# ZhenlongYuan/DVP-MVS

Measured on AMD Instinct MI355X. Metric: Mpixels/sec/PatchMatch-iteration, higher is better.
Workload: dtype f32

## Files before the change

__graft_entry__.py:

```python
import importlib
import os
import subprocess
import sys

ROOT = os.path.dirname(os.path.abspath(__file__))
if ROOT not in sys.path:
    sys.path.insert(0, ROOT)


def build() -> None:
    subprocess.check_call(["make", "-s", "-C", os.path.join(ROOT, "dvp-mvs_amd", "csrc")])
    host = os.path.join(ROOT, "dvp-mvs_amd", "host")
    if os.path.exists(os.path.join(host, "Makefile")):
        subprocess.check_call(["make", "-s", "-C", host])
    subprocess.check_call(["make", "-s", "-C", os.path.join(ROOT, "oracle")])
    subprocess.check_call(["make", "-s", "-C", os.path.join(ROOT, "tests", "emul")])
    subprocess.check_call(["make", "-s", "-C", os.path.join(ROOT, "tests", "host")])
    subprocess.check_call(["make", "-s", "-C", os.path.join(ROOT, "tests", "half16")])
    subprocess.check_call(["make", "-s", "-C", os.path.join(ROOT, "tests", "jpeg_host")])
    subprocess.check_call(["make", "-s", "-C", os.path.join(ROOT, "tests", "edges_host")])
    subprocess.check_call(["make", "-s", "-C", os.path.join(ROOT, "tests", "viewclean_host")])
    subprocess.check_call(["make", "-s", "-C", os.path.join(ROOT, "tests", "labels_host")])
    pkg = importlib.import_module("dvp-mvs_amd")
    lib = pkg.get_capi().lib()
    missing = [s for s in pkg.get_capi().EXPORTS if not hasattr(lib, s)]
    if missing:
        raise RuntimeError("libdvp_mvs_hip.so lacks symbols: %s" % missing)


def smoke() -> None:
    import numpy as np
    pkg = importlib.import_module("dvp-mvs_amd")
    synth, capi = pkg.synth, pkg.get_capi()
    from oracle import oracle as O
    W, H, S = 96, 64, 3
    sc = synth.make_scene(W, H, S)
    p = synth.default_params(S + 1, max_iterations=1, state=synth.FIRST_INIT, use_APD=0)
    p["depth_min"] = np.float32(2.5) * np.float32(0.6)
    p["depth_max"] = np.float32(6.5) * np.float32(1.2)
    state = dict(planes=np.zeros((H * W, 4), np.float32), edge=sc["edge"], label=sc["label"],
                 radius=np.full(H * W, 5, np.int32))
    g = capi.from_scene(sc, p, device=0)
    g.upload_state(**state)
    g.run_patchmatch()
    o = O.from_scene(sc, p)
    o.upload_state(**state)
    o.run_patchmatch()
    pg, po = g.get("planes"), o.get("planes")
    same = (pg.view(np.uint32) == po.view(np.uint32)) | (np.isnan(pg) & np.isnan(po))
    if not same.all():
        raise AssertionError("smoke: HIP planes differ from the oracle in %d values" % int((~same).sum()))
    for n in ("selected_views", "weak_info", "radius"):
        if not (g.get(n) == o.get(n)).all():
            raise AssertionError("smoke: %s differs from the oracle" % n)
    print("smoke ok: %dx%d S=%d bit-exact vs oracle; total %.2f ms" % (W, H, S, g.timings()["total_ms"]))


if __name__ == "__main__":
    build()
    if os.path.exists("/dev/kfd"):
        smoke()
```

dvp-mvs_amd/csrc/dvp_dev.hpp:

```cpp
#ifndef DVP_DEV_HPP_
#define DVP_DEV_HPP_

#include <stdint.h>
#include <math.h>
#include <float.h>
#include <string.h>
#include "../../include/dvp_mvs.h"

#if defined(__HIPCC__)
#include <hip/hip_runtime.h>
#define DVP_HD __host__ __device__ __forceinline__
#define DVP_HD_NOINLINE __host__ __device__ __noinline__
#else
#define DVP_HD inline
#define DVP_HD_NOINLINE inline
#endif
#ifndef DVP_STREAM_HINTS
#define DVP_STREAM_HINTS 3
#endif
#if defined(__HIP_DEVICE_COMPILE__)
#define DVP_NT_STORE(bit, p, v) do { if ((DVP_STREAM_HINTS) & (bit)) __builtin_nontemporal_store((v), (p)); else *(p) = (v); } while (0)
#define DVP_NT_LOAD(bit, p) (((DVP_STREAM_HINTS) & (bit)) ? __builtin_nontemporal_load(p) : *(p))
#else
#define DVP_NT_STORE(bit, p, v) (*(p) = (v))
#define DVP_NT_LOAD(bit, p) (*(p))
#endif

namespace dvp {

struct f4 { float x, y, z, w; };
struct f3 { float x, y, z; };
struct f2 { float x, y; };
struct i2 { int x, y; };
struct s2 { short x, y; };

DVP_HD f4 mk4(float x, float y, float z, float w) { f4 r; r.x = x; r.y = y; r.z = z; r.w = w; return r; }
DVP_HD f3 mk3(float x, float y, float z) { f3 r; r.x = x; r.y = y; r.z = z; return r; }
DVP_HD f2 mk2(float x, float y) { f2 r; r.x = x; r.y = y; return r; }
DVP_HD i2 mki2(int x, int y) { i2 r; r.x = x; r.y = y; return r; }
DVP_HD s2 mks2(int x, int y) { s2 r; r.x = (short)x; r.y = (short)y; return r; }

struct ViewConst {
	float Rrel[9];
	float trel[3];
	float sK0, sK2, sK4, sK5, sK8;
	float rK2, rK5;
	float inv_k0, inv_k4;
	float fw, fh;
	float pad;
};

struct AnchorRec;
struct WeakRec;
struct Dev {
	int width, height, num_images;
	int pitch;
	int org;
	size_t plane_stride;
	int sampler;
	int weak_count;
	uint64_t seed;
	DvpParams params;
	float nb_cos, nb_sin, nb_thresh;
	int nb_shift_range;
	const float* images;
	const uint8_t* images8;
	int img8_tiles_x;
	size_t img8_plane_bytes;
	const uint32_t* images16;
	int img16_tiles_x;
	size_t img16_plane_bytes;
	const float* depths;
	const DvpCamera* cameras;
	const ViewConst* views;
	const int* sector_taps;
	const int* sector_start;
	f4* planes;
	const f4* planes_snap;
	float* costs;
	const float* costs_snap;
	uint32_t* selected_views;
	uint8_t* view_weight;
	uint8_t* weak_info;
	uint8_t* weak_reliable;
	s2* weak_nearest_strong;
	const int* neighbours_map;
	s2* neighbours;
	s2* gn_points;
	int* gn_count;
	f4* fit_planes;
	s2* candidate;
	AnchorRec* anchor_tab;
	WeakRec* weak_rec;
	f2* weak_ctab;
	float* weak_ev;
	const uint8_t* edge;
	int* search_pos;
	float* slot_costs;
	float* strong_rec;
	f4* sweep_rec;
	float* sweep_cost;
	float* sweep_pc;
	int sweep_px0;
	int sweep_row0, sweep_row1;
	int half_w;
	uint32_t* edge_bits;
	int edge_tiles_x;
	uint32_t* strong_bits;
	uint32_t* strong_bits_t;
	int* edge_sat;
	int sat_cells_x, sat_cells_y;
	s2* edge_neigh;
	const int* label;
	s2* label_boundary;
	s2* label_stop;
	float* complex_;
	int* radius;
	const int* weak_list;
	int weak_black, weak_red;
	unsigned long long* eval_counter;
};

#define DVP_MIN(a, b) ((a) > (b) ? (b) : (a))
#define DVP_MAX(a, b) ((a) < (b) ? (b) : (a))

DVP_HD float dvp_expf(float x) {
	if (!(x > -103.0f)) return (x != x) ? x : 0.0f;
	if (x > 88.72f) return INFINITY;
	const float n = rintf(x * 1.44269504088896341f);
	float r = fmaf(n, -0.693359375f, x);
	r = fmaf(n, 2.12194440e-4f, r);
	float p = 1.9875691500e-4f;
	p = fmaf(p, r, 1.3981999507e-3f);
	p = fmaf(p, r, 8.3334519073e-3f);
	p = fmaf(p, r, 4.1665795894e-2f);
	p = fmaf(p, r, 1.6666665459e-1f);
	p = fmaf(p, r, 5.0000001201e-1f);
	const float r2 = r * r;
	const float y = fmaf(p, r2, r) + 1.0f;
	const int ni = (int)n;
	const int n1 = ni / 2, n2 = ni - n1;
	union { uint32_t u; float f; } s1, s2;
	s1.u = (uint32_t)(n1 + 127) << 23;
	s2.u = (uint32_t)(n2 + 127) << 23;
	return (y * s1.f) * s2.f;
}

DVP_HD uint32_t rand_u32(uint64_t seed, uint32_t pixel, uint32_t site, uint32_t k) {
	uint64_t z = seed + 0x9E3779B97F4A7C15ull * ((uint64_t)pixel + ((uint64_t)site << 32));
	z += 0xD1B54A32D192ED03ull * (uint64_t)(k + 1u);
	z ^= z >> 30; z *= 0xBF58476D1CE4E5B9ull;
	z ^= z >> 27; z *= 0x94D049BB133111EBull;
	z ^= z >> 31;
	return (uint32_t)(z >> 32);
}
DVP_HD float rand_uniform(uint64_t seed, uint32_t pixel, uint32_t site, uint32_t k) {
	return (float)((rand_u32(seed, pixel, site, k) >> 8) + 1u) * (1.0f / 16777216.0f);
}
enum { PH_RANDOM_INIT = 1, PH_STRONG = 2, PH_RANSAC = 3, PH_WEAK = 4, PH_NEIGHBOURS = 5 };
enum { SUB_VIEW = 0, SUB_DEPTH_RAND = 1, SUB_NORMAL = 2, SUB_DEPTH_PERT = 3, SUB_LIMIT = 4, SUB_SEARCH = 5, SUB_RANSAC = 6 };
DVP_HD uint32_t rng_site(int phase, int iter, int sub) {
	return ((uint32_t)phase << 16) | ((uint32_t)(iter & 0xff) << 8) | (uint32_t)sub;
}
struct Rng {
	uint64_t seed;
	uint32_t pixel, site, k;
	DVP_HD Rng(uint64_t s, uint32_t p, uint32_t st) : seed(s), pixel(p), site(st), k(0) {}
	DVP_HD uint32_t next() { return rand_u32(seed, pixel, site, k++); }
	DVP_HD float uniform() { return rand_uniform(seed, pixel, site, k++); }
};

constexpr int kImgPad = 2;

DVP_HD size_t cand_index(const Dev& d, int pixel, int v) { return ((size_t)v * ((size_t)d.width * d.height) + (size_t)pixel) * 8; }

DVP_HD int clampi(int v, int lo, int hi) { return v < lo ? lo : (v > hi ? hi : v); }

DVP_HD float tex_texel(const float* img, int org, int pitch, int W, int H, int ix, int iy) {
	return img[org + clampi(iy, 0, H - 1) * pitch + clampi(ix, 0, W - 1)];
}

DVP_HD float img_texel(const float* img, int org, int pitch, int W, int H, int ix, int iy) {
	return img[(size_t)(org + clampi(iy, 0, H - 1) * pitch + clampi(ix, 0, W - 1)) * 2];
}

DVP_HD void load_quad(const float* base, unsigned byte_off, float* a, float* b, float* c, float* e) {
#if defined(__HIPCC__)
	typedef float f4u __attribute__((ext_vector_type(4), aligned(8)));
	const f4u t = *reinterpret_cast<const f4u*>(reinterpret_cast<const char*>(base) + byte_off);
	*a = t.x; *b = t.y; *c = t.z; *e = t.w;
#else
	const float* p = reinterpret_cast<const float*>(reinterpret_cast<const char*>(base) + byte_off);
	*a = p[0]; *b = p[1]; *c = p[2]; *e = p[3];
#endif
}
#ifndef DVP_IMG8_TW
#define DVP_IMG8_TW 7
#endif
constexpr bool kT8Quad = DVP_IMG8_TW == 8;
constexpr int kT8W = DVP_IMG8_TW;
constexpr int kT8E = kT8Quad ? 8 : kT8W + 1;
constexpr int kT8B = kT8Quad ? 4 : 2;
constexpr int kT8H = 128 / (kT8E * kT8B);
constexpr unsigned kT8Mul = kT8W == 7 ? 74899u : (kT8W == 15 ? 34953u : 65536u);
DVP_HD int img8_tiles_x(int W) { return (W + 2 * kImgPad + kT8W - 1) / kT8W; }
DVP_HD int img8_tiles_y(int H) { return (H + 2 * kImgPad + kT8H - 1) / kT8H; }
DVP_HD unsigned img8_offset(int tiles_x, int i0, int j0) {
	const unsigned px = (unsigned)(i0 + kImgPad), py = (unsigned)(j0 + kImgPad);
#if defined(__HIP_DEVICE_COMPILE__)
	const unsigned tx = __umul24(px, kT8Mul) >> 19;
	const unsigned ex = px - __umul24((unsigned)kT8W, tx);
	const unsigned ty = py / (unsigned)kT8H, ey = py % (unsigned)kT8H;
	const unsigned tile = __umul24(ty, (unsigned)tiles_x) + tx;
#else
	const unsigned tx = (px * kT8Mul) >> 19;
	const unsigned ex = px - (unsigned)kT8W * tx;
	const unsigned ty = py / (unsigned)kT8H, ey = py % (unsigned)kT8H;
	const unsigned tile = ty * (unsigned)tiles_x + tx;
#endif
	return (tile << 7) + ey * (unsigned)(kT8B * kT8E) + ex * (unsigned)kT8B;
}
constexpr int kT16W = 7;
constexpr int kT16E = kT16W + 1;
constexpr int kT16B = 4;
constexpr int kT16H = 128 / (kT16E * kT16B);
DVP_HD int img16_tiles_x(int W) { return (W + 2 * kImgPad + kT16W - 1) / kT16W; }
DVP_HD int img16_tiles_y(int H) { return (H + 2 * kImgPad + kT16H - 1) / kT16H; }
DVP_HD unsigned img16_offset(int tiles_x, int i0, int j0) {
	const unsigned px = (unsigned)(i0 + kImgPad), py = (unsigned)(j0 + kImgPad);
	constexpr unsigned kMul = 74899u;
#if defined(__HIP_DEVICE_COMPILE__)
	const unsigned tx = __umul24(px, kMul) >> 19;
	const unsigned ex = px - __umul24((unsigned)kT16W, tx);
	const unsigned tile = __umul24(py / (unsigned)kT16H, (unsigned)tiles_x) + tx;
#else
	const unsigned tx = (px * kMul) >> 19;
	const unsigned ex = px - (unsigned)kT16W * tx;
	const unsigned tile = (py / (unsigned)kT16H) * (unsigned)tiles_x + tx;
#endif
	return (tile << 7) + (py % (unsigned)kT16H) * (unsigned)(kT16B * kT16E) + ex * (unsigned)kT16B;
}
DVP_HD float half_bits_to_float(uint32_t h) {
	const uint32_t s = (h & 0x8000u) << 16, e = (h >> 10) & 31u, m = h & 1023u;
	uint32_t b;
	if (e == 31u) b = s | 0x7F800000u | (m << 13);
	else if (e != 0u) b = s | ((e + 112u) << 23) | (m << 13);
	else if (m == 0u) b = s;
	else {
		int k = 0;
		uint32_t mm = m;
		while (!(mm & 1024u)) { mm <<= 1; ++k; }
		b = s | ((uint32_t)(113 - k) << 23) | ((mm & 1023u) << 13);
// ... 428 lines not shown
```

dvp-mvs_amd/csrc/dvp_engine.hip:

```cpp
#include "dvp_stages.hpp"
#include "dvp_jpeg_enc.h"
#include "dvp_edges_run.h"
#include "dvp_viewclean_run.h"
#include <hip/hip_runtime.h>
#include <cstdlib>
#include <string>
#include <vector>
#include <cstdio>
#include <cstring>
#include <mutex>
#include <condition_variable>
#include <thread>
#include <chrono>
#include <algorithm>
#include <cmath>

using namespace dvp;

struct LaunchArgs {
	int tiles_x, tiles, rows, half, colour, iter;
};

template <int STAGE, int SMP, int MV = 32>
__device__ __forceinline__ void stage_body(const Dev& d, const LaunchArgs& a) {
	const int lane = threadIdx.x & 63;
	const int wave = threadIdx.x >> 6;
	int px, py;
	unsigned long long n = 0;
	__shared__ f2 lds_tab[stage_uses_tab(STAGE) ? kTaps * kTaps * 256 : 1];
	const PatchTab tab{&lds_tab[stage_uses_tab(STAGE) ? threadIdx.x : 0], 256};
	if (block_to_pixel(blockIdx.x, lane, wave, a.tiles_x, a.tiles, a.rows, a.half, a.colour, d.width, d.height, &px, &py))
		run_pixel<STAGE, SMP, MV>(d, px, py, a.iter, d.eval_counter ? &n : nullptr, tab);
	if (d.eval_counter && n) atomicAdd(d.eval_counter, n);
}

struct ListArgs { int base, count, iter, covered_rows, group, run; };
#ifndef DVP_LIST_RUN
#define DVP_LIST_RUN 16
#endif
constexpr int kListRun = DVP_LIST_RUN;
#ifndef DVP_WAVE_RUN
#define DVP_WAVE_RUN 16
#endif
constexpr int kWaveRun = DVP_WAVE_RUN;
__device__ __forceinline__ int list_block(int b, int nblocks, int run) {
	const int group = 8 * run;
	if (b >= nblocks / group * group) return b;
	const int g = b / group, r = b - g * group;
	const int xcd = r & 7, i = r >> 3;
	return g * group + xcd * run + i;
}
template <int STAGE, int SMP, int MV = 32>
__device__ __forceinline__ void stage_body_list(const Dev& d, const ListArgs& a) {
	__shared__ f2 lds_tab[stage_uses_tab(STAGE) ? kTaps * kTaps * 256 : 1];
	const PatchTab tab{&lds_tab[stage_uses_tab(STAGE) ? threadIdx.x : 0], 256};
	const int t = list_block(blockIdx.x, gridDim.x, kListRun) * 256 + threadIdx.x;
	unsigned long long n = 0;
	if (t < a.count) {
		const int center = d.weak_list[a.base + t];
		const int py = center / d.width, px = center - py * d.width;
		if (!stage_is_half_c(STAGE) || py < a.covered_rows)
			run_pixel<STAGE, SMP, MV>(d, px, py, a.iter, d.eval_counter ? &n : nullptr, tab);
	}
	if (d.eval_counter && n) atomicAdd(d.eval_counter, n);
}
template <int STAGE, int SMP, int MV = 32>
__device__ __forceinline__ void stage_body64(const Dev& d, const LaunchArgs& a) {
	const int lane = threadIdx.x;
	const int b = blockIdx.x;
	const int tile = (b >> 5) * 8 + (b & 7), wave = (b >> 3) & 3;
	int px, py;
	unsigned long long n = 0;
	__shared__ f2 lds_tab[kTaps * kTaps * 64];
	const PatchTab tab{&lds_tab[lane], 64};
	if (block_to_pixel(tile, lane, wave, a.tiles_x, a.tiles, a.rows, a.half, a.colour, d.width, d.height, &px, &py))
		run_pixel<STAGE, SMP, MV>(d, px, py, a.iter, d.eval_counter ? &n : nullptr, tab);
	if (d.eval_counter && n) atomicAdd(d.eval_counter, n);
}
#define DVP_KERNEL64(NAME, STAGE, MINW)                                                                    \
	extern "C" __global__ void __launch_bounds__(64, MINW) NAME(const Dev d, const LaunchArgs a) {          \
		stage_body64<STAGE, 0>(d, a);                                                                       \
	}                                                                                                       \
	extern "C" __global__ void __launch_bounds__(64, MINW) NAME##_exact(const Dev d, const LaunchArgs a) {  \
		stage_body64<STAGE, 1>(d, a);                                                                       \
	}
#define DVP_KERNEL_LIST_MV(NAME, STAGE, MINW, MV)                                                         \
	extern "C" __global__ void __launch_bounds__(256, MINW) NAME(const Dev d, const ListArgs a) {         \
		stage_body_list<STAGE, 0, MV>(d, a);                                                               \
	}                                                                                                      \
	extern "C" __global__ void __launch_bounds__(256, MINW) NAME##_exact(const Dev d, const ListArgs a) { \
		stage_body_list<STAGE, 1, MV>(d, a);                                                               \
	}
#define DVP_KERNEL_LIST(NAME, STAGE, MINW)                                                                \
	extern "C" __global__ void __launch_bounds__(256, MINW) NAME(const Dev d, const ListArgs a) {         \
		stage_body_list<STAGE, 0>(d, a);                                                                   \
	}                                                                                                      \
	extern "C" __global__ void __launch_bounds__(256, MINW) NAME##_exact(const Dev d, const ListArgs a) { \
		stage_body_list<STAGE, 1>(d, a);                                                                   \
	}

#define DVP_KERNEL(NAME, STAGE, MINW)                                                                      \
	extern "C" __global__ void __launch_bounds__(256, MINW) NAME(const Dev d, const LaunchArgs a) {         \
		stage_body<STAGE, 0>(d, a);                                                                         \
	}                                                                                                       \
	extern "C" __global__ void __launch_bounds__(256, MINW) NAME##_exact(const Dev d, const LaunchArgs a) { \
		stage_body<STAGE, 1>(d, a);                                                                         \
	}

#define DVP_KERNEL_MV(NAME, STAGE, MINW, MV)                                                               \
	extern "C" __global__ void __launch_bounds__(256, MINW) NAME(const Dev d, const LaunchArgs a) {         \
		stage_body<STAGE, 0, MV>(d, a);                                                                     \
	}                                                                                                       \
	extern "C" __global__ void __launch_bounds__(256, MINW) NAME##_exact(const Dev d, const LaunchArgs a) { \
		stage_body<STAGE, 1, MV>(d, a);                                                                     \
	}

DVP_KERNEL(dvp_gen_edge_inform, DVP_ST_GEN_EDGE_INFORM, 1)
#ifndef DVP_LB_HEAVY
#define DVP_LB_HEAVY 2
#endif
DVP_KERNEL(dvp_random_init, DVP_ST_RANDOM_INIT, DVP_LB_HEAVY)
DVP_KERNEL(dvp_strong_update, DVP_ST_STRONG_UPDATE, DVP_LB_HEAVY)
DVP_KERNEL_MV(dvp_strong_update_v8, DVP_ST_STRONG_UPDATE, DVP_LB_HEAVY, kNarrowViews)
DVP_KERNEL_MV(dvp_strong_update_v16, DVP_ST_STRONG_UPDATE, DVP_LB_HEAVY, 16)
DVP_KERNEL64(dvp_strong_eval, kStageStrongEval, DVP_LB_HEAVY)
template <int SMP>
__device__ __forceinline__ void strong_eval_items_body(const Dev& d, const LaunchArgs& a) {
	const int lane = threadIdx.x;
	const int b = blockIdx.x;
	const int tile = (b >> 5) * 8 + (b & 7), wave = (b >> 3) & 3;
	__shared__ f2 lds_tab[kTaps * kTaps * 64];
	__shared__ uint8_t items[64 * kSlotCount];
	int px = 0, py = 0;
	bool active = block_to_pixel(tile, lane, wave, a.tiles_x, a.tiles, a.rows, a.half, a.colour, d.width, d.height, &px, &py);
	if (active && d.weak_info[px + py * d.width] == DVP_WEAK) active = false;
	PatchCtx c;
	c.tab = PatchTab{&lds_tab[lane], 64};
	c.sum_ref = c.sum_ref_ref = c.wsum = 0.0f;
	c.radius = c.inc = c.fast = 0;
	uint32_t uniq = 0;
	if (active) {
		const int center = px + py * d.width;
		int radius, inc;
		patch_geometry(d, center, &radius, &inc);
		build_patch_ctx(d, px, py, radius, inc, 0, c.tab, &c);
		uint32_t w[3];
		uniq = strong_slot_sources(d, center, w);
		const size_t Lh = (size_t)d.half_w * (size_t)d.height;
		uint32_t* dup = reinterpret_cast<uint32_t*>(d.strong_rec) + half_index(d, px, py);
		dup[SR_DUP * Lh] = w[0]; dup[(SR_DUP + 1) * Lh] = w[1]; dup[(SR_DUP + 2) * Lh] = w[2];
	}
	const int n = __popc(uniq);
	int incl = n;
#pragma unroll
	for (int o = 1; o < 64; o <<= 1) {
		const int t = __shfl_up(incl, o, 64);
		if (lane >= o) incl += t;
	}
	const int off = incl - n;
	const int total = __shfl(incl, 63, 64);
	{
		int k = 0;
		for (uint32_t m = uniq; m; m &= m - 1, ++k) items[off + k] = (uint8_t)lane;
	}
	__syncthreads();
	unsigned long long cnt = 0;
	for (int i0 = 0; i0 < total; i0 += 64) {
		const bool valid = i0 + lane < total;
		const int i = valid ? i0 + lane : total - 1;
		const int pl = items[i];
		const int k = i - __shfl(off, pl, 64);
		uint32_t m = (uint32_t)__shfl((int)uniq, pl, 64);
		for (int j = 0; j < k; ++j) m &= m - 1;
		const int slot = dvp_ctz(m);
		PatchCtx ci;
		ci.tab = PatchTab{&lds_tab[pl], 64};
		ci.sum_ref = __shfl(c.sum_ref, pl, 64);
		ci.sum_ref_ref = __shfl(c.sum_ref_ref, pl, 64);
		ci.wsum = __shfl(c.wsum, pl, 64);
		ci.radius = __shfl(c.radius, pl, 64);
		ci.inc = __shfl(c.inc, pl, 64);
		ci.fast = __shfl(c.fast, pl, 64);
		const int ipx = __shfl(px, pl, 64), ipy = __shfl(py, pl, 64);
		strong_eval_item<SMP>(d, ci, ipx, ipy, slot, valid, d.eval_counter ? &cnt : nullptr);
	}
	if (d.eval_counter && cnt) atomicAdd(d.eval_counter, cnt);
}
extern "C" __global__ void __launch_bounds__(64, DVP_LB_HEAVY) dvp_strong_eval_items(const Dev d, const LaunchArgs a) { strong_eval_items_body<0>(d, a); }
extern "C" __global__ void __launch_bounds__(64, DVP_LB_HEAVY) dvp_strong_eval_items_exact(const Dev d, const LaunchArgs a) { strong_eval_items_body<1>(d, a); }
DVP_KERNEL64(dvp_strong_refine, kStageStrongRefine, DVP_LB_HEAVY)
DVP_KERNEL64(dvp_strong_refine_lanes, kStageStrongRefineLanes, DVP_LB_HEAVY)
template <int MV>
__device__ __forceinline__ void strong_decide_body(const Dev& d, const LaunchArgs& a) {
	int px, py;
	if (!block_to_pixel(blockIdx.x, threadIdx.x & 63, threadIdx.x >> 6, a.tiles_x, a.tiles, a.rows, a.half, a.colour, d.width, d.height, &px, &py)) return;
	if (d.weak_info[px + py * d.width] != DVP_WEAK) strong_decide_px<MV>(d, px, py, a.iter);
}
#ifndef DVP_LB_DECIDE
#define DVP_LB_DECIDE 4
#endif
#define DVP_DECIDE_KERNEL(MV) extern "C" __global__ void __launch_bounds__(256, DVP_LB_DECIDE) dvp_strong_decide_v##MV(const Dev d, const LaunchArgs a) { strong_decide_body<MV>(d, a); }
DVP_DECIDE_KERNEL(4)
DVP_DECIDE_KERNEL(6)
DVP_DECIDE_KERNEL(8)
DVP_DECIDE_KERNEL(10)
DVP_DECIDE_KERNEL(12)
DVP_DECIDE_KERNEL(16)
DVP_KERNEL(dvp_get_depth_normal, DVP_ST_GET_DEPTH_NORMAL, 1)
DVP_KERNEL(dvp_filter_strong, DVP_ST_FILTER_STRONG, 1)
DVP_KERNEL(dvp_depth_to_weak, DVP_ST_DEPTH_TO_WEAK, DVP_LB_HEAVY)
DVP_KERNEL(dvp_local_refine, DVP_ST_LOCAL_REFINE, DVP_LB_HEAVY)
DVP_KERNEL(dvp_depth_to_weak_refine, kStageSweeps, DVP_LB_HEAVY)
template <int WHAT>
__device__ __forceinline__ void sweep_light_body(const Dev& d, const LaunchArgs& a) {
	int px, py;
	if (!block_to_pixel(blockIdx.x, threadIdx.x & 63, threadIdx.x >> 6, a.tiles_x, a.tiles, a.rows, 0, 0, d.width, d.height, &px, &py)) return;
	if (WHAT != 0 && d.sweep_row1 > 0 && (py < d.sweep_row0 || py >= d.sweep_row1)) return;
	if (WHAT == 0) sweep_prepare_px(d, px, py);
	else if (WHAT == 1) sweep_decide1_px(d, px, py);
	else sweep_decide2_px(d, px, py);
}
extern "C" __global__ void __launch_bounds__(256) dvp_sweep_prepare(const Dev d, const LaunchArgs a) { sweep_light_body<0>(d, a); }
extern "C" __global__ void __launch_bounds__(256) dvp_sweep_decide1(const Dev d, const LaunchArgs a) { sweep_light_body<1>(d, a); }
extern "C" __global__ void __launch_bounds__(256) dvp_sweep_decide2(const Dev d, const LaunchArgs a) { sweep_light_body<2>(d, a); }
#ifndef DVP_SWEEP_ROWS
#define DVP_SWEEP_ROWS 14
#endif
constexpr int kSweepRows = DVP_SWEEP_ROWS;
template <int SMP>
__device__ __forceinline__ void sweep_eval_body(const Dev& d, const LaunchArgs& a) {
	const int lane = threadIdx.x;
	const int v = blockIdx.y;
	__shared__ f2 lds_tab[kTaps * kTaps * 64];
	__shared__ uint16_t list[64 * kSweepRows];
	__shared__ DvpCamera cams[2];
	const PatchTab tab{&lds_tab[lane], 64};
	static_assert(sizeof(DvpCamera) == 112, "28 dwords");
	if (lane < 56) {
		const int which = lane >= 28 ? 1 : 0;
		reinterpret_cast<uint32_t*>(&cams[which])[lane - 28 * which] = reinterpret_cast<const uint32_t*>(d.cameras + (which ? v + 1 : 0))[lane - 28 * which];
	}
	const int tiles_y = a.tiles / a.tiles_x;
	int tx, ty;
	{
		const int per_strip = 8 * tiles_y;
		const int st = (int)blockIdx.x / per_strip, rem = (int)blockIdx.x - st * per_strip;
		const int w_last = a.tiles_x - st * 8;
		if (w_last >= 8) { ty = rem >> 3; tx = st * 8 + (rem & 7); }
		else { ty = rem / w_last; tx = st * 8 + (rem - ty * w_last); }
	}
	ty += a.rows;
	const int x = tx * 64 + lane;
	int n = 0;
	for (int r = 0; r < kSweepRows; ++r) {
		const int y = ty * kSweepRows + r;
		const bool go = x < d.width && y < d.height && sweep_go(d, x + y * d.width, v, a.iter);
		const unsigned long long m = __ballot(go);
		if (go) list[n + __popcll(m & ((1ull << lane) - 1ull))] = (uint16_t)(r * 64 + lane);
		n += __popcll(m);
	}
	__syncthreads();
	unsigned long long cnt = 0;
	for (int i0 = 0; i0 < n; i0 += 64) {
		if (i0 + lane < n) {
			const int e = list[i0 + lane];
			sweep_eval_px<SMP>(d, tx * 64 + (e & 63), ty * kSweepRows + (e >> 6), v, a.iter, tab, d.eval_counter ? &cnt : nullptr, cams);
		}
	}
	if (d.eval_counter && cnt) atomicAdd(d.eval_counter, cnt);
}
template <int SMP>
__device__ __forceinline__ void sweep_border_body(const Dev& d, const LaunchArgs& a) {
	__shared__ f2 lds_tab[kTaps * kTaps * 64];
	const PatchTab tab{&lds_tab[threadIdx.x], 64};
	const int W = d.width, H = d.height;
	const long long t = (long long)blockIdx.x * 64 + threadIdx.x;
	int px, py;
	if (t < 12ll * W) {
		const int r = (int)(t / W);
		px = (int)(t - (long long)r * W);
		py = r < 6 ? r : H - 12 + r;
	} else {
		const long long u = t - 12ll * W;
		const int r = (int)(u / 12), cidx = (int)(u - 12ll * r);
		if (r >= H - 12) return;
		py = 6 + r;
		px = cidx < 6 ? cidx : W - 12 + cidx;
	}
	unsigned long long n = 0;
	run_pixel<kStageSweeps, SMP>(d, px, py, kSweepBorderOnly, d.eval_counter ? &n : nullptr, tab);
	if (d.eval_counter && n) atomicAdd(d.eval_counter, n);
}
extern "C" __global__ void __launch_bounds__(64, DVP_LB_HEAVY) dvp_sweep_border(const Dev d, const LaunchArgs a) { sweep_border_body<0>(d, a); }
extern "C" __global__ void __launch_bounds__(64, DVP_LB_HEAVY) dvp_sweep_border_exact(const Dev d, const LaunchArgs a) { sweep_border_body<1>(d, a); }
extern "C" __global__ void __launch_bounds__(64, DVP_LB_HEAVY) dvp_sweep_eval(const Dev d, const LaunchArgs a) { sweep_eval_body<0>(d, a); }
extern "C" __global__ void __launch_bounds__(64, DVP_LB_HEAVY) dvp_sweep_eval_exact(const Dev d, const LaunchArgs a) { sweep_eval_body<1>(d, a); }

DVP_KERNEL_LIST(dvp_find_nearest_strong_list, DVP_ST_FIND_NEAREST_STRONG, 1)
extern "C" __global__ void __launch_bounds__(256) dvp_gen_neighbours_list(const Dev d, const ListArgs a) {
	__shared__ s2 pts[kGnDirSlots * 256];
	const int t = list_block(blockIdx.x, gridDim.x, kListRun) * 256 + threadIdx.x;
	if (t >= a.count) return;
	const int center = d.weak_list[a.base + t];
// ... 162 lines not shown
		y = kImgPad + k / (2 * kImgPad);
		x = k % (2 * kImgPad);
		if (x >= kImgPad) x += W;
	}
	float* p = planes + (size_t)pl * plane_stride;
	const int sx = clampi(x - kImgPad, 0, W - 1) + kImgPad, sy = clampi(y - kImgPad, 0, H - 1) + kImgPad;
	p[(size_t)y * pitch + x] = p[(size_t)sy * pitch + sx];
}

extern "C" __global__ void dvp_interleave_rows(const float* __restrict__ in, float* __restrict__ out, int PH, int pitch, size_t plane_stride, int n_planes) {
	const int x = blockIdx.x * blockDim.x + threadIdx.x;
	const int y = blockIdx.y;
	const int pl = blockIdx.z;
	if (x >= pitch) return;
	const float* p = in + (size_t)pl * plane_stride;
	const int y1 = y + 1 < PH ? y + 1 : y;
	const float2 v = make_float2(p[(size_t)y * pitch + x], p[(size_t)y1 * pitch + x]);
	reinterpret_cast<float2*>(out + (size_t)pl * plane_stride * 2)[(size_t)y * pitch + x] = v;
}

extern "C" __global__ void dvp_pairs_to_tiles(const float* __restrict__ pairs, uint8_t* __restrict__ out, int PW, int PH, int pitch, size_t plane_stride,
                                              int tiles_x, int tiles_y, int n_planes, int* inexact) {
	const size_t per_plane = (size_t)tiles_x * tiles_y * 64;
	const size_t i = (size_t)blockIdx.x * blockDim.x + threadIdx.x;
	if (i >= per_plane * n_planes) return;
	const int pl = (int)(i / per_plane);
	const size_t r = i - (size_t)pl * per_plane;
	const int tile = (int)(r >> 6), e = (int)(r & 63);
	const int ty = tile / tiles_x, tx = tile - ty * tiles_x;
	const int sx = min(tx * kT8W + (e % kT8E), PW - 1), sy = min(ty * kT8H + (e / kT8E), PH - 1);
	if (e >= kT8E * kT8H) return;
	const float* plane = pairs + (size_t)pl * plane_stride * 2;
	const float2 v = reinterpret_cast<const float2*>(plane)[(size_t)sy * pitch + sx];
	const float2 u = reinterpret_cast<const float2*>(plane)[(size_t)sy * pitch + min(sx + 1, PW - 1)];
	uint32_t h;
	const unsigned bad = tile_pair_rule(v.x, v.y, &h);
	if (bad) {
		if ((*inexact & bad) != bad) atomicOr(inexact, (int)bad);
		if (bad & 1u) return;
	}
	uint8_t* dst = out + ((size_t)pl * tiles_x * tiles_y + tile) * 128 + (size_t)e * kT8B;
	dst[0] = (uint8_t)v.x;
	dst[1] = (uint8_t)v.y;
	if (kT8Quad) { dst[2] = (uint8_t)u.x; dst[3] = (uint8_t)u.y; }
}

extern "C" __global__ void dvp_pairs_to_tiles16(const float* __restrict__ pairs, uint32_t* __restrict__ out, int PW, int PH, int pitch, size_t plane_stride,
                                                int tiles_x, int tiles_y, int n_planes) {
	constexpr int kPer = kT16E * kT16H;
	const size_t per_plane = (size_t)tiles_x * tiles_y * kPer;
	const size_t i = (size_t)blockIdx.x * blockDim.x + threadIdx.x;
	if (i >= per_plane * n_planes) return;
	const int pl = (int)(i / per_plane);
	const size_t r = i - (size_t)pl * per_plane;
	const int tile = (int)(r / kPer), e = (int)(r % kPer);
	const int ty = tile / tiles_x, tx = tile - ty * tiles_x;
	const int sx = min(tx * kT16W + (e % kT16E), PW - 1), sy = min(ty * kT16H + (e / kT16E), PH - 1);
	const float2 v = reinterpret_cast<const float2*>(pairs + (size_t)pl * plane_stride * 2)[(size_t)sy * pitch + sx];
	uint32_t h;
	(void)tile_pair_rule(v.x, v.y, &h);
	out[((size_t)pl * tiles_x * tiles_y + tile) * (128 / 4) + e] = h;
}

extern "C" __global__ void dvp_pack_edge_bits(const uint8_t* __restrict__ edge, uint32_t* __restrict__ bits, int W, int H, int tiles_x, size_t words, int equals) {
	const size_t w = (size_t)blockIdx.x * blockDim.x + threadIdx.x;
	if (w < words) bits[w] = pack_edge_word(edge, W, H, tiles_x, w, equals);
}

extern "C" __global__ void __launch_bounds__(256) dvp_gen_candidates(const Dev d, const LaunchArgs a) {
	int px, py;
	if (block_to_pixel(blockIdx.x, threadIdx.x & 63, threadIdx.x >> 6, a.tiles_x, a.tiles, a.rows, 0, 0, d.width, d.height, &px, &py))
		gen_candidates_px(d, px, py, (int)blockIdx.y);
}

extern "C" __global__ void __launch_bounds__(256) dvp_gen_candidates_views(const Dev d, const LaunchArgs a) {
	int px, py;
	if (block_to_pixel(blockIdx.x, threadIdx.x & 63, threadIdx.x >> 6, a.tiles_x, a.tiles, a.rows, 0, 0, d.width, d.height, &px, &py))
		gen_candidates_views_px<kCandGroup>(d, px, py, (int)blockIdx.y * kCandGroup);
}
extern "C" __global__ void __launch_bounds__(256) dvp_gen_candidates_views_list(const Dev d, const unsigned* list, const unsigned* n_list) {
	const unsigned t = blockIdx.x * 256 + threadIdx.x;
	if (t >= *n_list) return;
	const int center = (int)list[t];
	const int py = center / d.width, px = center - py * d.width;
	gen_candidates_views_px<kCandGroup>(d, px, py, (int)blockIdx.y * kCandGroup);
}

extern "C" __global__ void __launch_bounds__(256) dvp_anchor_mask(const Dev d, const ListArgs a, uint8_t* mask) {
	const int t = blockIdx.x * 256 + threadIdx.x;
	if (t >= a.count) return;
	const int center = d.weak_list[a.base + t];
	const s2* nb = d.neighbours + (size_t)d.neighbours_map[center] * DVP_NEIGHBOUR_NUM;
	for (int k = 1; k < DVP_NEIGHBOUR_NUM; ++k) {
		const s2 q = nb[k];
		if (q.x >= 0 && q.y >= 0 && q.x < d.width && q.y < d.height) mask[(size_t)q.y * d.width + q.x] = 1;
	}
}
extern "C" __global__ void __launch_bounds__(256) dvp_mask_compact(const uint8_t* mask, size_t L, unsigned* list, unsigned* n_list) {
	const size_t p = (size_t)blockIdx.x * 256 + threadIdx.x;
	const bool go = p < L && mask[p] != 0;
	const unsigned long long m = __ballot(go);
	if (!m) return;
	const int lane = threadIdx.x & 63;
	unsigned base = 0;
	if (lane == __builtin_ctzll(m)) base = atomicAdd(n_list, (unsigned)__popcll(m));
	base = __shfl(base, __builtin_ctzll(m), 64);
	if (go) list[base + __popcll(m & ((1ull << lane) - 1ull))] = (unsigned)p;
}
extern "C" __global__ void __launch_bounds__(256) dvp_gen_candidates_list(const Dev d, const unsigned* list, const unsigned* n_list) {
	const unsigned t = blockIdx.x * 256 + threadIdx.x;
	if (t >= *n_list) return;
	const int center = (int)list[t];
	const int py = center / d.width, px = center - py * d.width;
	gen_candidates_px(d, px, py, (int)blockIdx.y);
}

extern "C" __global__ void dvp_pack_bits_transposed(const uint8_t* __restrict__ map, uint32_t* __restrict__ bits, int W, int H, int tiles_x, size_t words, int equals) {
	const size_t w = (size_t)blockIdx.x * blockDim.x + threadIdx.x;
	if (w < words) bits[w] = pack_edge_word_t(map, W, H, tiles_x, w, equals);
}

extern "C" __global__ void dvp_edge_cell_counts(const Dev d) {
	const int c = blockIdx.x * blockDim.x + threadIdx.x;
	if (c >= d.sat_cells_x * d.sat_cells_y) return;
	const int cy = c / d.sat_cells_x, cx = c - cy * d.sat_cells_x;
	int n = 0;
	for (int r = 0; r < 8; ++r) {
		const int y = cy * 8 + r;
		if (y >= d.height) break;
		const unsigned w = d.edge_bits[(size_t)(((y >> 5) * d.edge_tiles_x + (cx >> 2)) * 32 + (y & 31))];
		n += __popc((w >> ((cx & 3) * 8)) & 255u);
	}
	d.edge_sat[(cy + 1) * (d.sat_cells_x + 1) + cx + 1] = n;
}
extern "C" __global__ void dvp_edge_sat_rows(const Dev d) {
	const int r = blockIdx.x * blockDim.x + threadIdx.x;
	if (r > d.sat_cells_y) return;
	int* row = d.edge_sat + (size_t)r * (d.sat_cells_x + 1);
	int acc = 0;
	for (int x = 0; x <= d.sat_cells_x; ++x) { acc += (r == 0 || x == 0) ? 0 : row[x]; row[x] = acc; }
}
extern "C" __global__ void dvp_edge_sat_cols(const Dev d) {
	const int x = blockIdx.x * blockDim.x + threadIdx.x;
	if (x > d.sat_cells_x) return;
	const int P = d.sat_cells_x + 1;
	int acc = 0;
	for (int r = 0; r <= d.sat_cells_y; ++r) { acc += d.edge_sat[(size_t)r * P + x]; d.edge_sat[(size_t)r * P + x] = acc; }
}

extern "C" __global__ void __launch_bounds__(256) dvp_strong_search(const Dev d, const LaunchArgs a) {
	int px, py;
	if (block_to_pixel(blockIdx.x, threadIdx.x & 63, threadIdx.x >> 6, a.tiles_x, a.tiles, a.rows, a.half, a.colour, d.width, d.height, &px, &py))
		strong_search_px(d, px, py);
}

extern "C" __global__ void __launch_bounds__(256) dvp_edge_rays(const Dev d, int what) {
	edge_ray_line(d, blockIdx.y, blockIdx.x * blockDim.x + threadIdx.x, what);
}

constexpr int kWeakTile = 16, kWeakSuper = 64, kWeakChunk = 1024;
DVP_HD void weak_slot_origin(int slot, int supers_x, int* tx, int* ty) {
	const int super = slot >> 4, t = slot & 15;
	*tx = (super % supers_x) * kWeakSuper + (t & 3) * kWeakTile;
	*ty = (super / supers_x) * kWeakSuper + (t >> 2) * kWeakTile;
}
extern "C" __global__ void __launch_bounds__(256) dvp_weak_counts(const uint8_t* __restrict__ weak, int W, int H, int supers_x, int n_slots, int n_chunks, int* __restrict__ counts) {
	const int lane = threadIdx.x & 63;
	const int unit = blockIdx.x * 4 + (threadIdx.x >> 6);
	if (unit < n_slots) {
		int tx, ty;
		weak_slot_origin(unit, supers_x, &tx, &ty);
		int nb = 0, nr = 0;
		for (int step = 0; step < 4; ++step) {
			const int x = tx + (lane & 15), y = ty + step * 4 + (lane >> 4);
			const bool wk = x < W && y < H && weak[(size_t)y * W + x] == DVP_WEAK;
			nb += __popcll(__ballot(wk && !((x + y) & 1)));
			nr += __popcll(__ballot(wk && ((x + y) & 1)));
		}
		if (lane == 0) { counts[unit] = nb; counts[n_slots + unit] = nr; }
	} else if (unit < n_slots + n_chunks) {
		const int chunk = unit - n_slots;
		const size_t L = (size_t)W * H;
		int n = 0;
		for (int step = 0; step < kWeakChunk / 64; ++step) {
			const size_t i = (size_t)chunk * kWeakChunk + step * 64 + lane;
			n += __popcll(__ballot(i < L && weak[i] == DVP_WEAK));
		}
		if (lane == 0) counts[2 * n_slots + chunk] = n;
	}
}
extern "C" __global__ void __launch_bounds__(1024) dvp_scan3(int* __restrict__ data, int s0, int s1, int s2, int s3, int* __restrict__ totals) {
	__shared__ int part[1024];
	__shared__ int carry;
	const int starts[4] = { s0, s1, s2, s3 };
	const int lo = starts[blockIdx.x], hi = starts[blockIdx.x + 1];
	if (threadIdx.x == 0) carry = 0;
	__syncthreads();
	for (int base = lo; base < hi; base += 1024) {
		const int i = base + (int)threadIdx.x;
		const int v = i < hi ? data[i] : 0;
		part[threadIdx.x] = v;
		__syncthreads();
		for (int off = 1; off < 1024; off <<= 1) {
			const int add = threadIdx.x >= (unsigned)off ? part[threadIdx.x - off] : 0;
			__syncthreads();
			part[threadIdx.x] += add;
			__syncthreads();
		}
		if (i < hi) data[i] = carry + part[threadIdx.x] - v;
		__syncthreads();
		if (threadIdx.x == 1023) carry += part[1023];
		__syncthreads();
	}
	if (threadIdx.x == 0) totals[blockIdx.x] = carry;
}
extern "C" __global__ void __launch_bounds__(256) dvp_weak_fill(const uint8_t* __restrict__ weak, int W, int H, int supers_x, int n_slots, int n_chunks,
                                                               const int* __restrict__ offs, const int* __restrict__ totals, int* __restrict__ list, int* __restrict__ map) {
	const int lane = threadIdx.x & 63;
	const int unit = blockIdx.x * 4 + (threadIdx.x >> 6);
	const unsigned long long below = (1ull << lane) - 1ull;
	if (unit < n_slots) {
		int tx, ty;
		weak_slot_origin(unit, supers_x, &tx, &ty);
		int ob = offs[unit], orr = totals[0] + offs[n_slots + unit];
		for (int step = 0; step < 4; ++step) {
			const int x = tx + (lane & 15), y = ty + step * 4 + (lane >> 4);
			const bool wk = x < W && y < H && weak[(size_t)y * W + x] == DVP_WEAK;
			const bool red = (x + y) & 1;
			const unsigned long long mb = __ballot(wk && !red), mr = __ballot(wk && red);
			if (wk) list[red ? orr + __popcll(mr & below) : ob + __popcll(mb & below)] = y * W + x;
			ob += __popcll(mb);
			orr += __popcll(mr);
		}
	} else if (unit < n_slots + n_chunks) {
		const int chunk = unit - n_slots;
		const size_t L = (size_t)W * H;
		int o = offs[2 * n_slots + chunk];
		for (int step = 0; step < kWeakChunk / 64; ++step) {
			const size_t i = (size_t)chunk * kWeakChunk + step * 64 + lane;
			const bool wk = i < L && weak[i] == DVP_WEAK;
			const unsigned long long m = __ballot(wk);
			if (i < L) map[i] = wk ? o + __popcll(m & below) : 0;
			o += __popcll(m);
		}
	}
}

struct RescaleArgs {
	int W, H, sw, sh;
	float scale_x, scale_y;
	const float* depth; const float* normal; const uint32_t* views; const uint8_t* weak; const int* radius;
	f4* planes; uint32_t* out_views; uint8_t* out_weak; int* out_radius;
	int radius_fallback;
};
extern "C" __global__ void __launch_bounds__(256) dvp_rescale_state(const RescaleArgs a) {
	const int c = blockIdx.x * blockDim.x + threadIdx.x, r = blockIdx.y;
	if (c >= a.W) return;
	const int o_r = static_cast<int>(r / a.scale_x);
	const int o_c = static_cast<int>(c / a.scale_y);
	const bool in = o_r >= 0 && o_c >= 0 && o_r < a.sh && o_c < a.sw;
	const size_t o = (size_t)r * a.W + c, i = in ? (size_t)o_r * a.sw + o_c : 0;
	a.planes[o] = in ? mk4(a.normal[3 * i], a.normal[3 * i + 1], a.normal[3 * i + 2], a.depth[i]) : mk4(0.0f, 0.0f, 0.0f, 0.0f);
	a.out_views[o] = in ? a.views[i] : 0u;
	const uint8_t st = a.weak ? (in ? a.weak[i] : (uint8_t)0) : (uint8_t)DVP_STRONG;
	a.out_weak[o] = st;
	if (a.radius) a.out_radius[o] = st == DVP_UNKNOWN ? a.radius_fallback : (in ? a.radius[i] : 0);
}

extern "C" __global__ void __launch_bounds__(256) dvp_unpack_maps(const f4* __restrict__ planes, const uint8_t* __restrict__ weak, size_t L, float dmin, float dmax,
                                                                 float* __restrict__ depth, float* __restrict__ normal, uint8_t* __restrict__ state) {
	const size_t i = (size_t)blockIdx.x * blockDim.x + threadIdx.x;
	if (i >= L) return;
	const f4 ph = planes[i];
	const bool usable = !(ph.w < dmin || ph.w > dmax);
	depth[i] = usable ? ph.w : 0.0f;
	normal[3 * i] = ph.x; normal[3 * i + 1] = ph.y; normal[3 * i + 2] = ph.z;
	state[i] = usable ? weak[i] : (uint8_t)DVP_UNKNOWN;
}

extern "C" __global__ void dvp_prepare_views(const DvpCamera* cams, ViewConst* views, int n) {
	const int v = blockIdx.x * blockDim.x + threadIdx.x;
	if (v >= 1 && v < n) compute_view_const(cams[0], cams[v], &views[v]);
}

extern "C" __global__ void __launch_bounds__(256) dvp_cost_vectors(const Dev d, const int* px, const f4* planes, int n, float* out) {
	const int i = blockIdx.x * blockDim.x + threadIdx.x;
	if (i >= n) return;
	const int x = px[2 * i], y = px[2 * i + 1];
	const int S = d.num_images - 1;
	PatchCtx c;
	__shared__ f2 lds_tab[kTaps * kTaps * 256];
	int radius, inc;
	patch_geometry(d, x + y * d.width, &radius, &inc);
	build_patch_ctx(d, x, y, radius, inc, 0, PatchTab{&lds_tab[threadIdx.x], 256}, &c);
	const f4 pl = planes[i];
	for (int v = 0; v < S; ++v) out[(size_t)i * S + v] = d.sampler ? ncc_old<1>(d, c, x, y, v + 1, pl) : ncc_old<0>(d, c, x, y, v + 1, pl);
}

extern "C" __global__ void __launch_bounds__(256) dvp_cost_all_pixels(const Dev d, const LaunchArgs a, float* out) {
	const int lane = threadIdx.x & 63, wave = threadIdx.x >> 6;
	int px, py;
	if (!block_to_pixel(blockIdx.x, lane, wave, a.tiles_x, a.tiles, a.rows, 0, 0, d.width, d.height, &px, &py)) return;
	const int center = px + py * d.width;
	const int S = d.num_images - 1;
	PatchCtx c;
	__shared__ f2 lds_tab[kTaps * kTaps * 256];
// ... 74 lines not shown
	const ViewConst vc = d.views[v + 1];
	const unsigned plane_off = (unsigned)((size_t)(v + 1) * d.plane_stride * 2 * sizeof(float));
	const int center = px + py * d.width;
	float acc = 0.0f;
	for (int k = 0; k < K; ++k) {
		int q = center + (k - K / 2) * stride;
		q = q < 0 ? 0 : (q >= L ? L - 1 : q);
		const f4 pl = d.planes[q];
		float H[9];
		homography(vc, pl, H);
		const f2 pt = apply_homography(H, px, py);
		if (pt.x >= vc.fw || pt.x < 0.0f || pt.y >= vc.fh || pt.y < 0.0f) { acc += 2.0f; continue; }
		acc += ncc_patch_fast<0>(d, c, H, d.images, px, py, plane_off);
	}
	atomicAdd(&out[center], acc);
}
__device__ __forceinline__ float probe_slot_plane(const DvpCamera& rc, const f4 origin, float base_line, float disp, int k, int px, int py, const DvpParams& P, bool* in_range) {
	float p_depth = origin.w;
	*in_range = true;
	if (k < 61) {
		p_depth = rc.K[0] * base_line / (disp + (k - 30));
		if (p_depth < P.depth_min || p_depth > P.depth_max) *in_range = false;
	}
	return distance_to_origin(rc, px, py, p_depth, origin);
}
extern "C" __global__ void __launch_bounds__(256, 2) dvp_probe_c(const Dev d, const LaunchArgs a, float* out, unsigned vmask) {
	const int lane = threadIdx.x & 63, wave = threadIdx.x >> 6;
	int px, py;
	if (!block_to_pixel(blockIdx.x, lane, wave, a.tiles_x, a.tiles, a.rows, 0, 0, d.width, d.height, &px, &py)) return;
	const int center = px + py * d.width;
	const int S = d.num_images - 1;
	PatchCtx c;
	__shared__ f2 lds_tab[kTaps * kTaps * 256];
	int radius, inc;
	patch_geometry(d, center, &radius, &inc);
	build_patch_ctx(d, px, py, radius, inc, 0, PatchTab{&lds_tab[threadIdx.x], 256}, &c);
	const DvpCamera rc = load_camera(d, 0);
	const f4 origin = normal_world_to_cam(rc, d.planes[center]);
	const float base_line = 0.4f, disp = rc.K[0] * base_line / origin.w;
	float acc = 0.0f;
	for (int k = 0; k < 62; ++k) {
		bool ok;
		f4 pl = origin;
		pl.w = probe_slot_plane(rc, origin, base_line, disp, k, px, py, d.params, &ok);
		float t = 0.0f;
		if (ok) for (int v = 0; v < S; ++v) if ((vmask >> v) & 1) t += ncc_old<0>(d, c, px, py, v + 1, pl);
		acc += t;
	}
	out[center] = acc;
}
#ifndef DVP_PROBE_NPX
#define DVP_PROBE_NPX 16
#endif
extern "C" __global__ void __launch_bounds__(64, DVP_PROBE_LB) dvp_probe_d(const Dev d, float* out, unsigned vmask) {
	const int lane = threadIdx.x;
	const int S = d.num_images - 1;
	__shared__ f2 ctab[kTaps * kTaps];
	__shared__ float caa[kTaps * kTaps];
	__shared__ float tot[64];
	const int runs = 64 / DVP_PROBE_NPX;
	const int tiles_x = (d.width + 63) / 64;
	const int per_strip = 8 * d.height * runs;
	const int st = (int)blockIdx.x / per_strip, rem = (int)blockIdx.x - st * per_strip;
	const int w_last = tiles_x - st * 8 >= 8 ? 8 : tiles_x - st * 8;
	const int col = rem % w_last, k2 = rem / w_last;
	const int py = k2 / runs, x0 = (st * 8 + col) * 64 + (k2 - py * runs) * DVP_PROBE_NPX;
	if (py >= d.height) return;
	const DvpCamera rc = load_camera(d, 0);
	for (int i = 0; i < DVP_PROBE_NPX; ++i) {
		const int px = x0 + i;
		if (px >= d.width) break;
		const int center = px + py * d.width;
		int radius, inc;
		patch_geometry(d, center, &radius, &inc);
		PatchCtx c;
		c.radius = radius; c.inc = inc; c.fast = 1;
		c.tab = PatchTab{ctab, 1};
		if (lane < kTaps * kTaps) {
			const int ty = lane / kTaps, tx = lane - ty * kTaps;
			const float cpix = img_texel(d.images, d.org, d.pitch, d.width, d.height, px, py);
			const float av = img_texel(d.images, d.org, d.pitch, d.width, d.height, px - radius + tx * inc, py - radius + ty * inc);
			const float w = bilateral_weight((float)(-radius + tx * inc), (float)(-radius + ty * inc), av, cpix, d.params.sigma_spatial, d.params.sigma_color, 0);
			const float wa = w * av;
			ctab[lane] = mk2(w, wa);
			caa[lane] = wa * av;
		}
		__builtin_amdgcn_fence(__ATOMIC_RELEASE, "wavefront"); __builtin_amdgcn_wave_barrier(); __builtin_amdgcn_fence(__ATOMIC_ACQUIRE, "wavefront");
		{
			float sr = 0.0f, srr = 0.0f, ws = 0.0f;
			for (int ty = 0; ty < kTaps; ++ty) {
				float a0 = 0.0f, a1 = 0.0f, a2 = 0.0f;
				for (int tx = 0; tx < kTaps; ++tx) { const f2 t = ctab[ty * kTaps + tx]; a0 += t.y; a1 += caa[ty * kTaps + tx]; a2 += t.x; }
				sr += a0; srr += a1; ws += a2;
			}
			c.sum_ref = sr; c.sum_ref_ref = srr; c.wsum = ws;
		}
		f4 origin = normal_world_to_cam(rc, d.planes[center]);
		origin.x = uniform_f(origin.x); origin.y = uniform_f(origin.y); origin.z = uniform_f(origin.z); origin.w = uniform_f(origin.w);
		const float base_line = 0.4f, disp = rc.K[0] * base_line / origin.w;
		bool ok;
		f4 pl = origin;
		pl.w = probe_slot_plane(rc, origin, base_line, disp, lane, px, py, d.params, &ok);
		float t = 0.0f;
		if (lane < 62 && ok) for (int v = 0; v < S; ++v) if ((vmask >> v) & 1) t += ncc_old<0>(d, c, px, py, v + 1, pl);
		tot[lane] = t;
		__builtin_amdgcn_fence(__ATOMIC_RELEASE, "wavefront"); __builtin_amdgcn_wave_barrier(); __builtin_amdgcn_fence(__ATOMIC_ACQUIRE, "wavefront");
		if (lane == 0) {
			float acc = 0.0f;
			for (int k = 0; k < 62; ++k) acc += tot[k];
			out[center] = acc;
		}
		__builtin_amdgcn_wave_barrier();
	}
}
extern "C" int dvp_probe(dvp_ctx* c, int mode, int K, int stride, int repeat, float* mean_ms, float* checksum);
#endif

struct EventPair { int stage; hipEvent_t a, b; };
enum { EV_TOTAL = -1, EV_ITER_LOOP = -2 };

struct dvp_ctx {
	int device = 0;
	int W = 0, H = 0, NI = 0, pitch = 0;
	size_t L = 0;
	hipStream_t stream = nullptr;
	int cand_mask_mode = -1;
	bool cand_mask_on = true;
	uint8_t* cand_mask = nullptr;
	unsigned *cand_list = nullptr, *cand_n = nullptr;
	uint32_t* sel_snap = nullptr;
	hipStream_t side = nullptr;
	hipEvent_t side_fork = nullptr, side_join = nullptr;
	Dev d{};
	std::vector<void*> allocs;
	float* images = nullptr;
	uint8_t* images8 = nullptr;
	int* images8_flag = nullptr;
	bool images8_ok = false;
	bool no_images8 = false;
	uint32_t* images16 = nullptr;
	bool images16_ok = false;
	bool no_images16 = false;
	float* image_stage = nullptr;
	float* depths = nullptr;
	uint32_t* edge_bits = nullptr;
	uint32_t* strong_bits = nullptr;
	uint32_t* strong_bits_t = nullptr;
	int* edge_sat = nullptr;
	DvpCamera* cameras = nullptr; ViewConst* views = nullptr; int* sector_taps = nullptr; int* sector_start = nullptr;
	f4* planes = nullptr; f4* planes_snap = nullptr; f4* fit_planes = nullptr;
	int* search_pos = nullptr;
	float* slot_costs = nullptr;
	float* strong_rec = nullptr;
	bool strong_split = true;
	bool eval_items = true;
	bool refine_lanes = true;
	f4* sweep_rec = nullptr; float* sweep_cost = nullptr; float* sweep_pc = nullptr;
	bool ransac_wave = false;
	bool sweep_split = true;
	bool sweep_force = false;
	double sweep_band_gb = 0.0;
	int sweep_band_rows = 0;
	bool gn_wave = false;
	float* costs = nullptr; float* costs_snap = nullptr; float* complex_ = nullptr;
	uint32_t* selected_views = nullptr;
	uint8_t* view_weight = nullptr; uint8_t* weak_info = nullptr; uint8_t* weak_reliable = nullptr; uint8_t* edge = nullptr;
	s2* label_stop = nullptr; s2* weak_nearest_strong = nullptr; s2* neighbours = nullptr; s2* gn_points = nullptr; int* gn_count = nullptr; s2* candidate = nullptr; s2* edge_neigh = nullptr; s2* label_boundary = nullptr;
	int* neighbours_map = nullptr; int* label = nullptr; int* radius = nullptr;
	unsigned long long* eval_counter = nullptr;
	float* scratch_out = nullptr;
	size_t weak_alloc = 0;
	AnchorRec* anchor_tab = nullptr;
	size_t anchor_tab_alloc = 0;
	bool anchor_tab_valid = false;
	bool anchor_tab_off = false;
	WeakRec* weak_rec = nullptr; f2* weak_ctab = nullptr; float* weak_ev = nullptr;
	size_t weak_phase_alloc = 0;
	bool weak_phased = true;
	int weak_phased_min = 8192;
	int weak_run[4] = { 64, 256, 1024, 1024 };
	int weak_group[4] = { 1, 4, 4, 2 };
	int* weak_list = nullptr;
	size_t weak_list_alloc = 0;
	int* weak_counts = nullptr;
	int* weak_totals_host = nullptr;
	uint8_t* coarse = nullptr;
	uint8_t* maps_out = nullptr;
	hipStream_t copy = nullptr;
	uint8_t* maps_host = nullptr;
	std::mutex dl_m;
	std::condition_variable dl_cv;
	bool dl_busy = false;
	bool dl_fetching = false;
	size_t coarse_alloc = 0;
	uint8_t* pv_bgr[3] = { nullptr, nullptr, nullptr };
	dvpjpeg::Encoder pv_enc[3];
	unsigned long long* pv_total = nullptr;
	hipEvent_t pv_done = nullptr;
	hipStream_t pv_copy = nullptr;
	int pv_kinds = 0;
	dvpedge::Scratch eg;
	struct EdgeSlot { uint8_t* map = nullptr; hipEvent_t done = nullptr; unsigned long long seq = 0; bool pending = false, fetching = false; };
	EdgeSlot eg_slot[2];
	unsigned long long eg_seq = 0;
	hipStream_t eg_copy = nullptr;
	std::mutex eg_m;
	std::condition_variable eg_cv;
	bool have_images = false;
	dvpvc::Scratch vc;
	bool vc_on = false;
	int vc_num_src = 0, vc_min_region = 0;
	f4* saved_planes = nullptr; uint32_t* saved_views = nullptr; uint8_t* saved_weak = nullptr; int* saved_radius = nullptr;
	bool have_saved = false;
	int lut_radius = -1;
	bool have_depths = false;
	bool profiling = false;
	std::vector<EventPair> events;
	DvpTimings timings{};
	std::string error;
};

static std::string g_create_error;

#define HIP_TRY(ctx, expr)                                                                          \
	do {                                                                                            \
		hipError_t e_ = (expr);                                                                     \
		if (e_ != hipSuccess) {                                                                     \
			char buf_[512];                                                                         \
			snprintf(buf_, sizeof(buf_), "%s failed: %s (%s:%d)", #expr, hipGetErrorString(e_), __FILE__, __LINE__); \
			(ctx)->error = buf_;                                                                    \
			return 1;                                                                               \
		}                                                                                           \
	} while (0)

template <class T>
static int dalloc(dvp_ctx* c, T** p, size_t count, bool zero = true) {
	void* q = nullptr;
	const size_t bytes = (count ? count : 1) * sizeof(T);
	HIP_TRY(c, hipMalloc(&q, bytes));
	c->allocs.push_back(q);
	if (zero) HIP_TRY(c, hipMemsetAsync(q, 0, bytes, c->stream));
	*p = (T*)q;
	return 0;
}

template <class T>
static void dfree(dvp_ctx* c, T** p) {
	if (!*p) return;
	for (size_t i = 0; i < c->allocs.size(); ++i)
		if (c->allocs[i] == (void*)*p) { c->allocs[i] = c->allocs.back(); c->allocs.pop_back(); break; }
	(void)hipFree((void*)*p);
	*p = nullptr;
}

static size_t img16_plane_bytes(int W, int H) { return (size_t)img16_tiles_x(W) * img16_tiles_y(H) * 128; }

static void sync_dev_struct(dvp_ctx* c) {
	Dev& d = c->d;
	d.width = c->W; d.height = c->H; d.num_images = c->NI; d.pitch = c->pitch;
	d.org = kImgPad * c->pitch + kImgPad;
	d.plane_stride = (size_t)c->pitch * (c->H + 2 * kImgPad);
	d.images = c->images; d.images8 = c->images8_ok ? c->images8 : nullptr; d.img8_tiles_x = img8_tiles_x(c->W); d.img8_plane_bytes = (size_t)img8_tiles_x(c->W) * img8_tiles_y(c->H) * 128;
	d.images16 = c->images16_ok ? c->images16 : nullptr; d.img16_tiles_x = img16_tiles_x(c->W); d.img16_plane_bytes = img16_plane_bytes(c->W, c->H);
	d.depths = c->depths; d.cameras = c->cameras; d.views = c->views; d.sector_taps = c->sector_taps; d.sector_start = c->sector_start;
	d.search_pos = c->search_pos;
	d.sweep_px0 = 0; d.sweep_row0 = 0; d.sweep_row1 = 0;
	d.sweep_rec = c->sweep_rec; d.sweep_cost = c->sweep_cost; d.sweep_pc = c->sweep_pc; d.slot_costs = c->slot_costs; d.strong_rec = c->strong_rec; d.half_w = (c->W + 1) / 2;
	d.planes = c->planes; d.planes_snap = c->planes_snap; d.costs = c->costs; d.costs_snap = c->costs_snap;
	d.selected_views = c->selected_views; d.view_weight = c->view_weight; d.weak_info = c->weak_info;
	d.weak_reliable = c->weak_reliable; d.weak_nearest_strong = c->weak_nearest_strong;
	d.anchor_tab = (c->anchor_tab_off || !c->anchor_tab_valid) ? nullptr : c->anchor_tab; d.neighbours_map = c->neighbours_map; d.neighbours = c->neighbours; d.gn_points = c->gn_points; d.gn_count = c->gn_count; d.fit_planes = c->fit_planes;
	d.candidate = c->candidate; d.edge = c->edge; d.edge_bits = c->edge_bits; d.strong_bits = c->strong_bits; d.strong_bits_t = c->strong_bits_t; d.edge_sat = c->edge_sat; d.sat_cells_x = sat_cells(c->W); d.sat_cells_y = sat_cells(c->H); d.edge_tiles_x = edge_tiles_x(c->W); d.edge_neigh = c->edge_neigh; d.label = c->label;
	d.label_boundary = c->label_boundary; d.label_stop = c->label_stop; d.complex_ = c->complex_; d.radius = c->radius;
	d.weak_list = c->weak_list;
	d.weak_rec = c->weak_rec; d.weak_ctab = c->weak_ctab; d.weak_ev = c->weak_ev;
	d.eval_counter = c->profiling ? c->eval_counter : nullptr;
}

static int ensure_images16(dvp_ctx* c) {
	if (c->images16) return 0;
	return dalloc(c, &c->images16, img16_plane_bytes(c->W, c->H) / 4 * c->NI, false);
}

static int set_device(dvp_ctx* c) {
	HIP_TRY(c, hipSetDevice(c->device));
	return 0;
}

extern "C" {

int dvp_ctx_create(int device, int width, int height, int num_images, dvp_ctx** out) {
	if (!out) return 1;
	*out = nullptr;
	if (width <= 0 || height <= 0 || num_images < 2 || num_images > DVP_MAX_IMAGES || width > 32767 || height > 32767) {
		g_create_error = "dvp_ctx_create: bad dimensions (2 <= num_images <= 32, sizes <= 32767: short2 pixel coordinates)";
		return 1;
	}
	{
		const unsigned long long pitch = ((unsigned long long)width + 2 * kImgPad + 63) / 64 * 64;
		if (pitch * ((unsigned long long)height + 2 * kImgPad) * 8ull >= (1ull << 32)) {
			g_create_error = "dvp_ctx_create: image too large (a padded row-pair plane must stay below 4 GiB)";
			return 1;
		}
	}
	dvp_ctx* c = new dvp_ctx();
	c->device = device; c->W = width; c->H = height; c->NI = num_images;
	c->no_images8 = getenv("DVP_NO_IMAGES8") != nullptr;
	c->no_images16 = getenv("DVP_NO_IMAGES16") != nullptr;
	if (const char* e = getenv("DVP_STRONG_SPLIT")) c->strong_split = atoi(e) != 0;
	if (const char* e = getenv("DVP_REFINE_LANES")) c->refine_lanes = atoi(e) != 0;
	if (const char* e = getenv("DVP_EVAL_ITEMS")) c->eval_items = atoi(e) != 0;
	if (const char* e = getenv("DVP_SWEEP_SPLIT")) { c->sweep_split = atoi(e) != 0; c->sweep_force = atoi(e) == 2; }
	if (const char* e = getenv("DVP_SWEEP_BAND_GB")) c->sweep_band_gb = atof(e);
	if (const char* e = getenv("DVP_WEAK_ANCHOR_TAB")) c->anchor_tab_off = atoi(e) == 0;
	if (const char* e = getenv("DVP_GN_WAVE")) c->gn_wave = atoi(e) != 0;
	if (const char* e = getenv("DVP_RANSAC_WAVE")) c->ransac_wave = atoi(e) != 0;
	if (const char* e = getenv("DVP_CAND_MASK")) c->cand_mask_mode = atoi(e) != 0 ? 1 : 0;
	if (const char* e = getenv("DVP_WEAK_PHASED")) c->weak_phased = atoi(e) != 0;
	if (const char* e = getenv("DVP_WEAK_PHASED_MIN")) c->weak_phased_min = atoi(e);
	if (const char* e = getenv("DVP_WEAK_RUNS")) {
		int g[4];
		if (sscanf(e, "%d,%d,%d,%d", &g[0], &g[1], &g[2], &g[3]) == 4)
			for (int i = 0; i < 4; ++i) c->weak_run[i] = g[i] < 1 ? 1 : g[i];
	}
	if (const char* e = getenv("DVP_WEAK_GROUPS")) {
		int g[4];
		if (sscanf(e, "%d,%d,%d,%d", &g[0], &g[1], &g[2], &g[3]) == 4)
			for (int i = 0; i < 4; ++i) c->weak_group[i] = g[i] < 1 ? 1 : (g[i] > kGrp ? kGrp : g[i]);
	}
	c->pitch = (width + 2 * kImgPad + 63) / 64 * 64;
	c->L = (size_t)width * height;
	auto fail = [&](int) { g_create_error = c->error; dvp_ctx_destroy(c); return 1; };
	if (set_device(c)) return fail(0);
	if (hipStreamCreateWithFlags(&c->stream, hipStreamNonBlocking) != hipSuccess) { c->error = "hipStreamCreate failed"; return fail(0); }
	if (hipStreamCreateWithFlags(&c->side, hipStreamNonBlocking) != hipSuccess || hipEventCreateWithFlags(&c->side_fork, hipEventDisableTiming) != hipSuccess ||
	    hipEventCreateWithFlags(&c->side_join, hipEventDisableTiming) != hipSuccess) { c->error = "hipStreamCreate failed"; return fail(0); }
	const size_t L = c->L, S = (size_t)num_images - 1, plane = (size_t)c->pitch * (height + 2 * kImgPad);
	int r = 0;
	r |= dalloc(c, &c->images, plane * num_images * 2);
	r |= dalloc(c, &c->images8, (size_t)img8_tiles_x(width) * img8_tiles_y(height) * 128 * num_images);
	r |= dalloc(c, &c->images8_flag, (size_t)1);
	r |= dalloc(c, &c->image_stage, plane * num_images);
	r |= dalloc(c, &c->cameras, (size_t)num_images);
	r |= dalloc(c, &c->views, (size_t)num_images);
	r |= dalloc(c, &c->planes, L);
	r |= dalloc(c, &c->planes_snap, L);
	r |= dalloc(c, &c->search_pos, L * 16);
	r |= dalloc(c, &c->fit_planes, L);
	r |= dalloc(c, &c->costs, L);
	r |= dalloc(c, &c->costs_snap, L);
	r |= dalloc(c, &c->selected_views, L + (size_t)width);
	r |= dalloc(c, &c->view_weight, L * 32);
	r |= dalloc(c, &c->weak_info, L);
	r |= dalloc(c, &c->weak_reliable, L);
	r |= dalloc(c, &c->weak_nearest_strong, L);
	r |= dalloc(c, &c->neighbours_map, L);
	r |= dalloc(c, &c->candidate, L * S * 8);
	r |= dalloc(c, &c->edge, L);
	r |= dalloc(c, &c->edge_bits, edge_bits_words(width, height));
	r |= dalloc(c, &c->strong_bits, edge_bits_words(width, height));
	r |= dalloc(c, &c->strong_bits_t, edge_bits_words(width, height));
	r |= dalloc(c, &c->edge_sat, (size_t)(sat_cells(width) + 1) * (sat_cells(height) + 1));
	r |= dalloc(c, &c->edge_neigh, L * 8);
	r |= dalloc(c, &c->label, L);
	r |= dalloc(c, &c->radius, L);
	r |= dalloc(c, &c->eval_counter, (size_t)1);
	r |= dalloc(c, &c->scratch_out, L);
	if (r) return fail(0);
	{
		std::vector<uint8_t> st(L, (uint8_t)DVP_STRONG);
		std::vector<int> rad(L, 5);
		std::vector<s2> m1(L * 8, mks2(-1, -1));
		if (hipMemcpyAsync(c->weak_info, st.data(), L, hipMemcpyHostToDevice, c->stream) != hipSuccess ||
			hipMemcpyAsync(c->radius, rad.data(), L * 4, hipMemcpyHostToDevice, c->stream) != hipSuccess ||
			hipMemcpyAsync(c->edge_neigh, m1.data(), L * 8 * 4, hipMemcpyHostToDevice, c->stream) != hipSuccess ||
			hipMemcpyAsync(c->weak_nearest_strong, m1.data(), L * 4, hipMemcpyHostToDevice, c->stream) != hipSuccess ||
			hipStreamSynchronize(c->stream) != hipSuccess) { c->error = "default state upload failed"; return fail(0); }
	}
	std::memset(&c->d.params, 0, sizeof(DvpParams));
	c->d.params.num_images = num_images;
	c->d.params.strong_radius = 5; c->d.params.strong_increment = 2; c->d.params.weak_radius = 5; c->d.params.weak_increment = 5;
	c->d.params.rotate_time = 4;
	sync_dev_struct(c);
	*out = c;
	return 0;
}

int dvp_ctx_destroy(dvp_ctx* c) {
	if (!c) return 0;
	(void)hipSetDevice(c->device);
	{
		int limit_s = 120;
		if (const char* e = getenv("DVP_DOWNLOAD_WAIT_S")) limit_s = atoi(e);
		std::unique_lock<std::mutex> lk(c->dl_m);
		c->dl_cv.wait_for(lk, std::chrono::seconds(limit_s > 0 ? limit_s : 1), [c] { return !c->dl_busy; });
		c->dl_cv.wait(lk, [c] { return !c->dl_fetching; });
	}
	if (c->copy) { (void)hipStreamSynchronize(c->copy); (void)hipStreamDestroy(c->copy); }
	if (c->pv_copy) { (void)hipStreamSynchronize(c->pv_copy); (void)hipStreamDestroy(c->pv_copy); }
	{
		std::unique_lock<std::mutex> lk(c->eg_m);
		c->eg_cv.wait(lk, [c] { return !c->eg_slot[0].fetching && !c->eg_slot[1].fetching; });
	}
	if (c->eg_copy) { (void)hipStreamSynchronize(c->eg_copy); (void)hipStreamDestroy(c->eg_copy); }
	if (c->stream) (void)hipStreamSynchronize(c->stream);
	for (auto& e : c->pv_enc) dvpjpeg::encoder_free(e);
	dvpedge::scratch_free(c->eg);
	dvpvc::scratch_free(c->vc);
	for (auto& sl : c->eg_slot) { if (sl.map) (void)hipFree(sl.map); if (sl.done) (void)hipEventDestroy(sl.done); }
	if (c->pv_total) (void)hipHostFree(c->pv_total);
	if (c->pv_done) (void)hipEventDestroy(c->pv_done);
	if (c->maps_host) (void)hipHostFree(c->maps_host);
	if (c->stream) (void)hipStreamSynchronize(c->stream);
	for (auto& e : c->events) { (void)hipEventDestroy(e.a); (void)hipEventDestroy(e.b); }
	for (void* p : c->allocs) (void)hipFree(p);
	if (c->weak_totals_host) (void)hipHostFree(c->weak_totals_host);
	if (c->side) { (void)hipStreamSynchronize(c->side); (void)hipStreamDestroy(c->side); }
	if (c->side_fork) (void)hipEventDestroy(c->side_fork);
	if (c->side_join) (void)hipEventDestroy(c->side_join);
	if (c->stream) (void)hipStreamDestroy(c->stream);
	delete c;
	return 0;
}

#ifndef DVP_BUILD_ID
#define DVP_BUILD_ID "unknown"
#endif
const char* dvp_build_id(void) { return DVP_BUILD_ID; }

struct FinishError { const dvp_ctx* c = nullptr; std::string msg; };
static thread_local FinishError t_finish_error;
const char* dvp_last_error(const dvp_ctx* c) {
	if (c && t_finish_error.c == c && !t_finish_error.msg.empty()) return t_finish_error.msg.c_str();
	return c ? c->error.c_str() : g_create_error.c_str();
}

static int upload_planes(dvp_ctx* c, float* dst, const float* const* src, int pitch_floats, hipMemcpyKind kind, float* pairs = nullptr) {
	if (set_device(c)) return 1;
	if (pitch_floats < c->W) { c->error = "pitch_floats < width"; return 1; }
	const size_t stride = (size_t)c->pitch * (c->H + 2 * kImgPad);
	for (int i = 0; i < c->NI; ++i) {
		if (!src[i]) { c->error = "null image pointer"; return 1; }
		HIP_TRY(c, hipMemcpy2DAsync(dst + (size_t)i * stride + (size_t)kImgPad * c->pitch + kImgPad, (size_t)c->pitch * 4, src[i],
		                            (size_t)pitch_floats * 4, (size_t)c->W * 4, (size_t)c->H, kind, c->stream));
	}
	{
		const long long cells = (long long)(2 * kImgPad * (c->W + 2 * kImgPad) + 2 * kImgPad * c->H) * c->NI;
		hipLaunchKernelGGL(dvp_pad_replicate, dim3((unsigned)((cells + 255) / 256)), dim3(256), 0, c->stream, dst, c->W, c->H, c->pitch, stride, c->NI);
		HIP_TRY(c, hipGetLastError());
	}
	if (pairs) {
		const int PH = c->H + 2 * kImgPad;
		hipLaunchKernelGGL(dvp_interleave_rows, dim3((unsigned)((c->pitch + 255) / 256), (unsigned)PH, (unsigned)c->NI), dim3(256), 0, c->stream,
		                   dst, pairs, PH, c->pitch, stride, c->NI);
		HIP_TRY(c, hipGetLastError());
		HIP_TRY(c, hipMemsetAsync(c->images8_flag, 0, sizeof(int), c->stream));
		const int t8x = img8_tiles_x(c->W), t8y = img8_tiles_y(c->H);
		const size_t n = (size_t)t8x * t8y * 64 * c->NI;
		hipLaunchKernelGGL(dvp_pairs_to_tiles, dim3((unsigned)((n + 255) / 256)), dim3(256), 0, c->stream, pairs, c->images8, c->W + 2 * kImgPad, PH, c->pitch, stride,
		                   t8x, t8y, c->NI, c->images8_flag);
		HIP_TRY(c, hipGetLastError());
		int inexact = 3;
		HIP_TRY(c, hipMemcpyAsync(&inexact, c->images8_flag, sizeof(int), hipMemcpyDeviceToHost, c->stream));
		HIP_TRY(c, hipStreamSynchronize(c->stream));
		c->images8_ok = inexact == 0 && !c->no_images8;
		c->images16_ok = inexact == 1 && !c->no_images8 && !c->no_images16;
		if (c->images16_ok) {
			if (ensure_images16(c)) { c->images16_ok = false; sync_dev_struct(c); return 1; }
			const int t16x = img16_tiles_x(c->W), t16y = img16_tiles_y(c->H);
			const size_t n16 = (size_t)t16x * t16y * (kT16E * kT16H) * c->NI;
			hipLaunchKernelGGL(dvp_pairs_to_tiles16, dim3((unsigned)((n16 + 255) / 256)), dim3(256), 0, c->stream, pairs, c->images16, c->W + 2 * kImgPad, PH, c->pitch, stride,
			                   t16x, t16y, c->NI);
			HIP_TRY(c, hipGetLastError());
		}
		sync_dev_struct(c);
	}
	HIP_TRY(c, hipStreamSynchronize(c->stream));
	return 0;
}
int dvp_upload_images(dvp_ctx* c, const float* const* images, int pitch_floats) {
	c->anchor_tab_valid = false;
	if (upload_planes(c, c->image_stage, images, pitch_floats, hipMemcpyHostToDevice, c->images)) return 1;
	c->have_images = true;
	return 0;
}
int dvp_upload_images_device(dvp_ctx* c, const float* const* images, int pitch_floats) {
	c->anchor_tab_valid = false;
	if (upload_planes(c, c->image_stage, images, pitch_floats, hipMemcpyDeviceToDevice, c->images)) return 1;
	c->have_images = true;
	return 0;
}
static int ensure_depths(dvp_ctx* c) {
	if (!c->depths) {
		if (dalloc(c, &c->depths, (size_t)c->pitch * (c->H + 2 * kImgPad) * c->NI)) return 1;
		sync_dev_struct(c);
	}
	c->have_depths = true;
	return 0;
}
int dvp_upload_depths(dvp_ctx* c, const float* const* depths, int pitch_floats) {
	if (set_device(c) || ensure_depths(c)) return 1;
	return upload_planes(c, c->depths, depths, pitch_floats, hipMemcpyHostToDevice);
}
int dvp_upload_depths_device(dvp_ctx* c, const float* const* depths, int pitch_floats) {
	if (set_device(c) || ensure_depths(c)) return 1;
	return upload_planes(c, c->depths, depths, pitch_floats, hipMemcpyDeviceToDevice);
}

int dvp_upload_cameras(dvp_ctx* c, const DvpCamera* cams, int n) {
	if (set_device(c)) return 1;
	if (n != c->NI) { c->error = "dvp_upload_cameras: n != num_images"; return 1; }
	HIP_TRY(c, hipMemcpyAsync(c->cameras, cams, sizeof(DvpCamera) * n, hipMemcpyHostToDevice, c->stream));
	hipLaunchKernelGGL(dvp_prepare_views, dim3(1), dim3(64), 0, c->stream, c->cameras, c->views, n);
	HIP_TRY(c, hipGetLastError());
	HIP_TRY(c, hipStreamSynchronize(c->stream));
	return 0;
}

static int ensure_weak_buffers(dvp_ctx* c, size_t weak_count) {
	const size_t need = weak_count ? weak_count : 1;
	if (need > c->weak_alloc) {
		HIP_TRY(c, hipStreamSynchronize(c->stream));
		if (c->side) HIP_TRY(c, hipStreamSynchronize(c->side));
		dfree(c, &c->neighbours); dfree(c, &c->gn_points); dfree(c, &c->gn_count); dfree(c, &c->complex_); dfree(c, &c->label_boundary);
		const size_t cap = std::min<size_t>(c->L, std::max(need, c->weak_alloc + c->weak_alloc / 2));
		if (dalloc(c, &c->neighbours, cap * DVP_NEIGHBOUR_NUM, false)) return 1;
		if (dalloc(c, &c->gn_points, cap * kGnDirSlots, false) || dalloc(c, &c->gn_count, cap)) return 1;
		if (dalloc(c, &c->complex_, cap)) return 1;
		if (dalloc(c, &c->label_boundary, cap * 8, false)) return 1;
		c->weak_alloc = cap;
	}
	HIP_TRY(c, hipMemsetAsync(c->neighbours, 0xFF, need * DVP_NEIGHBOUR_NUM * sizeof(s2), c->stream));
	HIP_TRY(c, hipMemsetAsync(c->label_boundary, 0xFF, need * 8 * sizeof(s2), c->stream));
	HIP_TRY(c, hipMemsetAsync(c->complex_, 0, need * 4, c->stream));
	return 0;
}

static int rebuild_weak_lists(dvp_ctx* c) {
	const size_t L = c->L;
	const int supers_x = (c->W + kWeakSuper - 1) / kWeakSuper, supers_y = (c->H + kWeakSuper - 1) / kWeakSuper;
	const int n_slots = supers_x * supers_y * 16, n_chunks = (int)((L + kWeakChunk - 1) / kWeakChunk);
	const int n_units = n_slots + n_chunks;
	if (!c->weak_counts) {
		if (dalloc(c, &c->weak_counts, (size_t)2 * n_slots + n_chunks + 4)) return 1;
		HIP_TRY(c, hipHostMalloc((void**)&c->weak_totals_host, 4 * sizeof(int)));
	}
	int* totals = c->weak_counts + 2 * (size_t)n_slots + n_chunks;
	hipLaunchKernelGGL(dvp_weak_counts, dim3((n_units + 3) / 4), dim3(256), 0, c->stream, c->weak_info, c->W, c->H, supers_x, n_slots, n_chunks, c->weak_counts);
	hipLaunchKernelGGL(dvp_scan3, dim3(3), dim3(1024), 0, c->stream, c->weak_counts, 0, n_slots, 2 * n_slots, 2 * n_slots + n_chunks, totals);
	HIP_TRY(c, hipMemcpyAsync(c->weak_totals_host, totals, 3 * sizeof(int), hipMemcpyDeviceToHost, c->stream));
	HIP_TRY(c, hipStreamSynchronize(c->stream));
	const int nb = c->weak_totals_host[0], nr = c->weak_totals_host[1], wc = c->weak_totals_host[2];
	if (nb + nr != wc) { c->error = "dvp_upload_state: WEAK list / map counts disagree"; return 1; }
	c->d.weak_count = wc;
	c->d.weak_black = nb;
	c->d.weak_red = nr;
	if ((size_t)wc > c->weak_list_alloc) {
		dfree(c, &c->weak_list);
		const size_t cap = std::min<size_t>(L, std::max<size_t>((size_t)wc, c->weak_list_alloc + c->weak_list_alloc / 2));
		if (dalloc(c, &c->weak_list, cap, false)) return 1;
		c->weak_list_alloc = cap;
	}
	if (wc > 0) {
		hipLaunchKernelGGL(dvp_weak_fill, dim3((n_units + 3) / 4), dim3(256), 0, c->stream, c->weak_info, c->W, c->H, supers_x, n_slots, n_chunks,
		                   c->weak_counts, totals, c->weak_list, c->neighbours_map);
		HIP_TRY(c, hipGetLastError());
	} else {
		HIP_TRY(c, hipMemsetAsync(c->neighbours_map, 0, L * 4, c->stream));
	}
	if (ensure_weak_buffers(c, (size_t)wc)) return 1;
	HIP_TRY(c, hipStreamSynchronize(c->stream));
	sync_dev_struct(c);
	return 0;
}

int dvp_upload_state(dvp_ctx* c, const float* planes, const uint32_t* views, const uint8_t* weak,
                     const uint8_t* edge, const int32_t* label, const int32_t* radius) {
	c->anchor_tab_valid = false;
	if (set_device(c)) return 1;
	const size_t L = c->L;
	if (planes) HIP_TRY(c, hipMemcpyAsync(c->planes, planes, L * 16, hipMemcpyHostToDevice, c->stream));
	if (views) HIP_TRY(c, hipMemcpyAsync(c->selected_views, views, L * 4, hipMemcpyHostToDevice, c->stream));
	if (edge) HIP_TRY(c, hipMemcpyAsync(c->edge, edge, L, hipMemcpyHostToDevice, c->stream));
	if (label) HIP_TRY(c, hipMemcpyAsync(c->label, label, L * 4, hipMemcpyHostToDevice, c->stream));
	if (radius) HIP_TRY(c, hipMemcpyAsync(c->radius, radius, L * 4, hipMemcpyHostToDevice, c->stream));
	if (weak) HIP_TRY(c, hipMemcpyAsync(c->weak_info, weak, L, hipMemcpyHostToDevice, c->stream));
	return rebuild_weak_lists(c);
}

int dvp_upload_state_rescaled(dvp_ctx* c, int src_w, int src_h, const float* depth, const float* normal_xyz, const uint32_t* views,
                              const uint8_t* weak, const int32_t* radius, int radius_fallback, const uint8_t* edge, const int32_t* label) {
	c->anchor_tab_valid = false;
	if (set_device(c)) return 1;
	if (src_w <= 0 || src_h <= 0 || !depth || !normal_xyz || !views) { c->error = "dvp_upload_state_rescaled: depth, normal and selected_views are required"; return 1; }
	const size_t L = c->L, n = (size_t)src_w * src_h;
	const size_t off_normal = n * 4, off_views = off_normal + n * 12, off_radius = off_views + n * 4, off_weak = off_radius + n * 4, bytes = off_weak + n;
	if (bytes > c->coarse_alloc) {
		HIP_TRY(c, hipStreamSynchronize(c->stream));
		dfree(c, &c->coarse);
		if (dalloc(c, &c->coarse, bytes, false)) return 1;
		c->coarse_alloc = bytes;
	}
	HIP_TRY(c, hipMemcpyAsync(c->coarse, depth, n * 4, hipMemcpyHostToDevice, c->stream));
	HIP_TRY(c, hipMemcpyAsync(c->coarse + off_normal, normal_xyz, n * 12, hipMemcpyHostToDevice, c->stream));
	HIP_TRY(c, hipMemcpyAsync(c->coarse + off_views, views, n * 4, hipMemcpyHostToDevice, c->stream));
	if (radius) HIP_TRY(c, hipMemcpyAsync(c->coarse + off_radius, radius, n * 4, hipMemcpyHostToDevice, c->stream));
	if (weak) HIP_TRY(c, hipMemcpyAsync(c->coarse + off_weak, weak, n, hipMemcpyHostToDevice, c->stream));
	if (edge) HIP_TRY(c, hipMemcpyAsync(c->edge, edge, L, hipMemcpyHostToDevice, c->stream));
	if (label) HIP_TRY(c, hipMemcpyAsync(c->label, label, L * 4, hipMemcpyHostToDevice, c->stream));
	RescaleArgs a;
	a.W = c->W; a.H = c->H; a.sw = src_w; a.sh = src_h;
	a.scale_x = c->W / static_cast<float>(src_w);
	a.scale_y = c->H / static_cast<float>(src_h);
	a.depth = reinterpret_cast<const float*>(c->coarse); a.normal = reinterpret_cast<const float*>(c->coarse + off_normal);
	a.views = reinterpret_cast<const uint32_t*>(c->coarse + off_views);
	a.radius = radius ? reinterpret_cast<const int*>(c->coarse + off_radius) : nullptr;
	a.weak = weak ? c->coarse + off_weak : nullptr;
	a.planes = c->planes; a.out_views = c->selected_views; a.out_weak = c->weak_info; a.out_radius = c->radius;
	a.radius_fallback = radius_fallback;
	hipLaunchKernelGGL(dvp_rescale_state, dim3((unsigned)((c->W + 255) / 256), (unsigned)c->H), dim3(256), 0, c->stream, a);
	HIP_TRY(c, hipGetLastError());
	return rebuild_weak_lists(c);
}

int dvp_reset_state(dvp_ctx* c) {
	c->anchor_tab_valid = false;
	if (set_device(c)) return 1;
	const size_t L = c->L;
	HIP_TRY(c, hipMemsetAsync(c->planes, 0, L * 16, c->stream));
	HIP_TRY(c, hipMemsetAsync(c->fit_planes, 0, L * 16, c->stream));
	HIP_TRY(c, hipMemsetAsync(c->costs, 0, L * 4, c->stream));
	HIP_TRY(c, hipMemsetAsync(c->selected_views, 0, (L + c->W) * 4, c->stream));
	HIP_TRY(c, hipMemsetAsync(c->view_weight, 0, L * 32, c->stream));
	HIP_TRY(c, hipMemsetAsync(c->weak_info, DVP_STRONG, L, c->stream));
	HIP_TRY(c, hipMemsetAsync(c->edge, 0, L, c->stream));
	HIP_TRY(c, hipMemsetAsync(c->label, 0, L * 4, c->stream));
	HIP_TRY(c, hipMemsetAsync(c->neighbours_map, 0, L * 4, c->stream));
	HIP_TRY(c, hipMemsetD32Async((hipDeviceptr_t)c->radius, c->d.params.strong_radius, L, c->stream));
	c->d.weak_count = 0;
	c->d.weak_black = c->d.weak_red = 0;
	if (ensure_weak_buffers(c, 0)) return 1;
	sync_dev_struct(c);
	return 0;
}

int dvp_image_format(const dvp_ctx* c) { return !c ? 0 : (c->images8_ok ? 1 : (c->images16_ok ? 2 : 0)); }
int dvp_save_state(dvp_ctx* c) {
	if (set_device(c)) return 1;
	const size_t L = c->L;
	if (!c->saved_planes) {
		if (dalloc(c, &c->saved_planes, L, false) || dalloc(c, &c->saved_views, L, false) ||
			dalloc(c, &c->saved_weak, L, false) || dalloc(c, &c->saved_radius, L, false)) return 1;
	}
	HIP_TRY(c, hipMemcpyAsync(c->saved_planes, c->planes, L * 16, hipMemcpyDeviceToDevice, c->stream));
	HIP_TRY(c, hipMemcpyAsync(c->saved_views, c->selected_views, L * 4, hipMemcpyDeviceToDevice, c->stream));
	HIP_TRY(c, hipMemcpyAsync(c->saved_weak, c->weak_info, L, hipMemcpyDeviceToDevice, c->stream));
	HIP_TRY(c, hipMemcpyAsync(c->saved_radius, c->radius, L * 4, hipMemcpyDeviceToDevice, c->stream));
	c->have_saved = true;
	return 0;
}
int dvp_restore_state(dvp_ctx* c) {
	c->anchor_tab_valid = false;
	if (set_device(c)) return 1;
	if (!c->have_saved) { c->error = "dvp_restore_state: no saved state"; return 1; }
	const size_t L = c->L;
	HIP_TRY(c, hipMemcpyAsync(c->planes, c->saved_planes, L * 16, hipMemcpyDeviceToDevice, c->stream));
	HIP_TRY(c, hipMemcpyAsync(c->selected_views, c->saved_views, L * 4, hipMemcpyDeviceToDevice, c->stream));
	HIP_TRY(c, hipMemcpyAsync(c->weak_info, c->saved_weak, L, hipMemcpyDeviceToDevice, c->stream));
	HIP_TRY(c, hipMemcpyAsync(c->radius, c->saved_radius, L * 4, hipMemcpyDeviceToDevice, c->stream));
	HIP_TRY(c, hipMemsetAsync(c->fit_planes, 0, L * 16, c->stream));
	HIP_TRY(c, hipMemsetAsync(c->costs, 0, L * 4, c->stream));
	HIP_TRY(c, hipMemsetAsync(c->view_weight, 0, L * 32, c->stream));
	HIP_TRY(c, hipMemsetAsync(c->weak_reliable, 0, L, c->stream));
	if (ensure_weak_buffers(c, (size_t)c->d.weak_count)) return 1;
	return 0;
}

int dvp_set_params(dvp_ctx* c, const DvpParams* p) {
	c->anchor_tab_valid = false;
	if (set_device(c)) return 1;
	if (p->num_images != c->NI) { c->error = "dvp_set_params: params.num_images != context num_images"; return 1; }
	if (p->use_edge == 0) { c->error = "dvp_set_params: use_edge=false is rejected: the reference's legacy ACMH branch (APD.cu:2142-2460) adopts planes through positions[], which only the use_edge branch assigns (APD.cu:2036, 2084, 2133 vs 2559-2563) - it has no defined result to reproduce"; return 1; }
	if (p->weak_radius < 0 || p->weak_radius > 15) { c->error = "dvp_set_params: weak_radius out of range [0,15]"; return 1; }
	c->d.params = *p;
	set_neighbour_consts(&c->d);
	if (c->lut_radius != p->weak_radius) {
		std::vector<int> taps, start;
		make_sector_taps(p->weak_radius, &taps, &start);
		if (dalloc(c, &c->sector_taps, taps.size(), false) || dalloc(c, &c->sector_start, start.size(), false)) return 1;
		HIP_TRY(c, hipMemcpyAsync(c->sector_taps, taps.data(), taps.size() * 4, hipMemcpyHostToDevice, c->stream));
		HIP_TRY(c, hipMemcpyAsync(c->sector_start, start.data(), start.size() * 4, hipMemcpyHostToDevice, c->stream));
		HIP_TRY(c, hipStreamSynchronize(c->stream));
		c->lut_radius = p->weak_radius;
	}
	sync_dev_struct(c);
	return 0;
}
int dvp_set_seed(dvp_ctx* c, uint64_t seed) { c->d.seed = seed; return 0; }
int dvp_set_sampler(dvp_ctx* c, int s) { c->d.sampler = s ? 1 : 0; return 0; }
int dvp_set_profiling(dvp_ctx* c, int on) { c->profiling = on != 0; sync_dev_struct(c); return 0; }

static int grow_anchor_table(dvp_ctx* c, size_t wc) {
	const size_t need = wc * (size_t)(c->NI - 1) * kAnchors;
	if (c->anchor_tab_off || need <= c->anchor_tab_alloc) return 0;
	{
		HIP_TRY(c, hipStreamSynchronize(c->stream));
		dfree(c, &c->anchor_tab);
		c->anchor_tab_alloc = 0;
		const size_t cap = need + need / 2;
		void* q = nullptr;
		size_t got = cap;
		if (hipMalloc(&q, cap * sizeof(AnchorRec)) != hipSuccess) {
			(void)hipGetLastError();
			got = need;
			if (hipMalloc(&q, need * sizeof(AnchorRec)) != hipSuccess) q = nullptr;
		}
		if (!q) {
			(void)hipGetLastError();
			c->anchor_tab_off = true;
			sync_dev_struct(c);
			fprintf(stderr, "dvp: no room for the weak update's anchor table (%.1f GB); forming the reference side per item\n", (double)need * sizeof(AnchorRec) / 1e9);
			return 0;
		}
		c->allocs.push_back(q);
		c->anchor_tab = (AnchorRec*)q;
		c->anchor_tab_alloc = got;
		sync_dev_struct(c);
	}
	return 0;
}
static int ensure_anchor_table(dvp_ctx* c, int covered_rows) {
	if (c->anchor_tab_off) return 0;
	if (c->anchor_tab_valid) return 0;
	const int wc = c->d.weak_black + c->d.weak_red;
	const size_t need = (size_t)wc * (size_t)(c->NI - 1) * kAnchors;
	if (grow_anchor_table(c, (size_t)wc)) return 1;
	if (c->anchor_tab_off) return 0;
	c->anchor_tab_valid = true;
	sync_dev_struct(c);
	ListArgs la;
	la.base = 0; la.count = wc; la.iter = 0; la.covered_rows = covered_rows;
	const long long n = (long long)need;
	if (n > 0) {
		hipLaunchKernelGGL(dvp_weak_anchor_table, dim3((unsigned)((n + 255) / 256)), dim3(256), 0, c->stream, c->d, la);
		HIP_TRY(c, hipGetLastError());
	}
	return 0;
}

static int grow_weak_phase_buffers(dvp_ctx* c, size_t wc);
static int ensure_weak_phase_buffers(dvp_ctx* c) { return grow_weak_phase_buffers(c, (size_t)(c->d.weak_black + c->d.weak_red)); }
static int grow_weak_phase_buffers(dvp_ctx* c, size_t wc) {
	if (!c->weak_phased) return 0;
	if (wc <= c->weak_phase_alloc) return 0;
	HIP_TRY(c, hipStreamSynchronize(c->stream));
	dfree(c, &c->weak_rec); dfree(c, &c->weak_ctab); dfree(c, &c->weak_ev);
	c->weak_phase_alloc = 0;
	const size_t cap = std::min<size_t>(c->L, wc + wc / 2), S = (size_t)c->NI - 1;
	void *r = nullptr, *t = nullptr, *e = nullptr;
	if (getenv("DVP_TEST_WEAK_PHASE_ALLOC_FAIL")  || hipMalloc(&r, cap * sizeof(WeakRec)) != hipSuccess ||
	    hipMalloc(&t, cap * kTaps * kTaps * sizeof(f2)) != hipSuccess || hipMalloc(&e, cap * 8 * S * sizeof(float)) != hipSuccess) {
		(void)hipGetLastError();
		if (r) (void)hipFree(r);
		if (t) (void)hipFree(t);
		c->weak_phased = false;
		fprintf(stderr, "dvp: no room for the phased weak update's hand-over buffers (%.2f GB); using the one-wave kernel\n", (double)cap * (sizeof(WeakRec) + 288 + 32 * S) / 1e9);
		sync_dev_struct(c);
		return 0;
	}
	c->allocs.push_back(r); c->allocs.push_back(t); c->allocs.push_back(e);
	c->weak_rec = (WeakRec*)r; c->weak_ctab = (f2*)t; c->weak_ev = (float*)e;
	c->weak_phase_alloc = cap;
	sync_dev_struct(c);
	return 0;
}

static void ensure_strong_split_buffers(dvp_ctx* c) {
	if (c->slot_costs || !c->strong_split || c->NI - 1 > 16) return;
	const size_t Lh = (size_t)((c->W + 1) / 2) * c->H;
	void *sc = nullptr, *sr = nullptr;
	if (getenv("DVP_TEST_SPLIT_ALLOC_FAIL")  || hipMalloc(&sc, (size_t)kSlotCount * (c->NI - 1) * Lh * sizeof(*c->slot_costs) + 64 ) != hipSuccess || hipMalloc(&sr, (size_t)SR_FIELDS * Lh * sizeof(*c->strong_rec)) != hipSuccess) {
		(void)hipGetLastError();
		if (sc) (void)hipFree(sc);
		c->strong_split = false;
		fprintf(stderr, "dvp: no room for the split strong update's cost buffer (%.1f GB); using the monolithic kernel\n", (double)kSlotCount * (c->NI - 1) * Lh * 4 / 1e9);
	} else {
		c->allocs.push_back(sc); c->allocs.push_back(sr);
		c->slot_costs = (decltype(c->slot_costs))sc; c->strong_rec = (decltype(c->strong_rec))sr;
		sync_dev_struct(c);
	}
}
static void ensure_sweep_buffers(dvp_ctx* c) {
	if (c->sweep_cost || !c->sweep_split) return;
	const size_t L = c->L;
	void *r = nullptr, *sc = nullptr, *pc = nullptr;
	size_t band_px = L;
	c->sweep_band_rows = 0;
	if (c->sweep_band_gb > 0.0) {
		const double whole = (double)sweep_cost_floats(L, c->NI - 1) * sizeof(float);
		const int bands = (int)std::ceil(whole / (c->sweep_band_gb * 1e9));
		if (bands > 1) {
			int rows = (c->H + bands - 1) / bands;
			rows = (rows + kSweepRows - 1) / kSweepRows * kSweepRows;
			if (rows < c->H) { c->sweep_band_rows = rows; band_px = (size_t)rows * c->W; }
		}
	}
	if (getenv("DVP_TEST_SWEEP_ALLOC_FAIL") || hipMalloc(&r, 2 * L * sizeof(f4)) != hipSuccess || hipMalloc(&pc, 61 * L * sizeof(float)) != hipSuccess ||
	    hipMalloc(&sc, sweep_cost_floats(band_px, c->NI - 1) * sizeof(float)) != hipSuccess) {
		(void)hipGetLastError();
		if (r) (void)hipFree(r);
		if (pc) (void)hipFree(pc);
		c->sweep_split = false;
		fprintf(stderr, "dvp: no room for the view-compacted DepthToWeak's cost buffer (%.1f GB); using the fused kernel\n", (double)(c->NI - 1) * kSweepFields * L * 4 / 1e9);
	} else {
		c->allocs.push_back(r); c->allocs.push_back(sc); c->allocs.push_back(pc);
		c->sweep_rec = (f4*)r; c->sweep_cost = (float*)sc; c->sweep_pc = (float*)pc;
		sync_dev_struct(c);
	}
}

static int launch_stage(dvp_ctx* c, int stage, int iter, int colour, bool fused = false) {
	if (stage < 0 || stage >= DVP_ST_LAUNCHABLE) { c->error = "bad stage id"; return 1; }
	if (!c->sector_taps) { c->error = "dvp_set_params must be called before running kernels"; return 1; }
	if (c->d.params.geom_consistency && !c->have_depths) { c->error = "geom_consistency is on but no depth maps were uploaded"; return 1; }
	const LaunchGeom g = make_geom(c->W, c->H, stage_is_half(stage));
	LaunchArgs a;
	a.tiles_x = g.tiles_x; a.tiles = g.tiles; a.rows = g.rows; a.half = g.half ? 1 : 0;
	a.colour = colour; a.iter = iter;
	if (c->events.size() >= 2048 && dvp_get_timings(c, nullptr)) return 1;
	if (stage != DVP_ST_STRONG_UPDATE && stage != DVP_ST_RANSAC_FIT && stage != DVP_ST_WEAK_UPDATE) c->anchor_tab_valid = false;
	if (stage == DVP_ST_STRONG_UPDATE) {
		EventPair prep;
		prep.stage = DVP_ST_STRONG_PREP;
		HIP_TRY(c, hipEventCreate(&prep.a));
		HIP_TRY(c, hipEventCreate(&prep.b));
		HIP_TRY(c, hipEventRecord(prep.a, c->stream));
		HIP_TRY(c, hipMemcpyAsync(c->planes_snap, c->planes, c->L * 16, hipMemcpyDeviceToDevice, c->stream));
		HIP_TRY(c, hipMemcpyAsync(c->costs_snap, c->costs, c->L * 4, hipMemcpyDeviceToDevice, c->stream));
		hipLaunchKernelGGL(dvp_strong_search, dim3(g.grid()), dim3(256), 0, c->stream, c->d, a);
		HIP_TRY(c, hipGetLastError());
		HIP_TRY(c, hipEventRecord(prep.b, c->stream));
		c->events.push_back(prep);
	}
	EventPair ep;
	ep.stage = stage;
	HIP_TRY(c, hipEventCreate(&ep.a));
	HIP_TRY(c, hipEventCreate(&ep.b));
	if (c->profiling) HIP_TRY(c, hipMemsetAsync(c->eval_counter, 0, 8, c->stream));
	HIP_TRY(c, hipEventRecord(ep.a, c->stream));
	const dim3 grid(g.grid()), block(256);
	const dim3 wave_grid((unsigned)((g.grid() + 7) / 8 * 32)), wave_block(64);
	const bool list_stage = stage == DVP_ST_FIND_NEAREST_STRONG || stage == DVP_ST_GEN_NEIGHBOURS || stage == DVP_ST_NEIGHBOUR_UPDATE ||
	                        stage == DVP_ST_RANSAC_FIT || stage == DVP_ST_WEAK_UPDATE;
	if (stage == DVP_ST_FIND_NEAREST_STRONG && c->d.weak_black + c->d.weak_red > 0) {
		const size_t words = edge_bits_words(c->W, c->H);
		hipLaunchKernelGGL(dvp_pack_edge_bits, dim3((unsigned)((words + 255) / 256)), dim3(256), 0, c->stream, c->weak_info, c->strong_bits, c->W, c->H, edge_tiles_x(c->W), words, (int)DVP_STRONG);
		hipLaunchKernelGGL(dvp_pack_bits_transposed, dim3((unsigned)((words + 255) / 256)), dim3(256), 0, c->stream, c->weak_info, c->strong_bits_t, c->W, c->H, edge_tiles_x(c->W), words, (int)DVP_STRONG);
		HIP_TRY(c, hipGetLastError());
	}
	if (stage == DVP_ST_GEN_NEIGHBOURS || stage == DVP_ST_RANSAC_FIT) {
		const size_t words = edge_bits_words(c->W, c->H);
		hipLaunchKernelGGL(dvp_pack_edge_bits, dim3((unsigned)((words + 255) / 256)), dim3(256), 0, c->stream, c->edge, c->edge_bits, c->W, c->H, edge_tiles_x(c->W), words, -1);
		HIP_TRY(c, hipGetLastError());
		const int cells = c->d.sat_cells_x * c->d.sat_cells_y;
		hipLaunchKernelGGL(dvp_edge_cell_counts, dim3((cells + 255) / 256), dim3(256), 0, c->stream, c->d);
		hipLaunchKernelGGL(dvp_edge_sat_rows, dim3((c->d.sat_cells_y + 1 + 63) / 64), dim3(64), 0, c->stream, c->d);
		hipLaunchKernelGGL(dvp_edge_sat_cols, dim3((c->d.sat_cells_x + 1 + 63) / 64), dim3(64), 0, c->stream, c->d);
		HIP_TRY(c, hipGetLastError());
		if (stage == DVP_ST_GEN_NEIGHBOURS) {
			hipLaunchKernelGGL(dvp_pack_edge_bits, dim3((unsigned)((words + 255) / 256)), dim3(256), 0, c->stream, c->weak_info, c->strong_bits, c->W, c->H, edge_tiles_x(c->W), words, (int)DVP_STRONG);
			HIP_TRY(c, hipGetLastError());
		}
	}
	if (list_stage) {
		if (stage == DVP_ST_FIND_NEAREST_STRONG) HIP_TRY(c, hipMemsetAsync(c->weak_nearest_strong, 0xFF, c->L * sizeof(s2), c->stream));
		if (stage == DVP_ST_RANSAC_FIT) HIP_TRY(c, hipMemcpyAsync(c->fit_planes, c->planes, c->L * 16, hipMemcpyDeviceToDevice, c->stream));
		ListArgs la;
		la.iter = iter;
		la.covered_rows = 2 * make_geom(c->W, c->H, true).rows;
		la.base = (stage == DVP_ST_WEAK_UPDATE && colour == 1) ? c->d.weak_black : 0;
		la.count = (stage == DVP_ST_WEAK_UPDATE) ? (colour == 0 ? c->d.weak_black : (colour == 1 ? c->d.weak_red : c->d.weak_black + c->d.weak_red)) : c->d.weak_black + c->d.weak_red;
		if (la.count > 0) {
			const dim3 lg((la.count + 255) / 256);
			const bool ex = c->d.sampler != 0;
			switch (stage) {
			case DVP_ST_FIND_NEAREST_STRONG: hipLaunchKernelGGL(ex ? dvp_find_nearest_strong_list_exact : dvp_find_nearest_strong_list, lg, block, 0, c->stream, c->d, la); break;
			case DVP_ST_GEN_NEIGHBOURS:
				if (c->gn_wave) hipLaunchKernelGGL(dvp_gen_neighbours_search, dim3((la.count + 3) / 4), block, 0, c->stream, c->d, la);
				else hipLaunchKernelGGL(dvp_gen_neighbours_list, lg, block, 0, c->stream, c->d, la);
				hipLaunchKernelGGL(dvp_gen_neighbours_fit, dim3(la.count), dim3(64), 0, c->stream, c->d, la);
				break;
			case DVP_ST_NEIGHBOUR_UPDATE: hipLaunchKernelGGL(ex ? dvp_neighbour_update_list_exact : dvp_neighbour_update_list, lg, block, 0, c->stream, c->d, la); break;
			case DVP_ST_RANSAC_FIT:
				if (c->ransac_wave) hipLaunchKernelGGL(dvp_ransac_fit_plane_wave, dim3(la.count), dim3(64), 0, c->stream, c->d, la);
				else hipLaunchKernelGGL(ex ? dvp_ransac_fit_plane_list_exact : dvp_ransac_fit_plane_list, lg, block, 0, c->stream, c->d, la);
				break;
			case DVP_ST_WEAK_UPDATE:
				if (ensure_anchor_table(c, la.covered_rows)) return 1;
				if (c->d.anchor_tab && ensure_weak_phase_buffers(c)) return 1;
				if (c->d.anchor_tab && c->weak_phased && (la.count >= c->weak_phased_min || c->weak_phased_min <= 0)) {
					const int fmt = dvp_image_format(c);
					const dim3 w64(64), lg64((la.count + 63) / 64);
#define DVP_PICK(NAME) (ex ? (fmt == 1 ? NAME##_exact_u8 : (fmt == 2 ? NAME##_exact_f16 : NAME##_exact)) : (fmt == 1 ? NAME##_u8 : (fmt == 2 ? NAME##_f16 : NAME)))
#define DVP_GROUP_LAUNCH(NAME, PHASE) { la.group = std::min(c->weak_group[PHASE], PHASE == 0 ? kGrpWide : kGrp); la.run = c->weak_run[PHASE]; hipLaunchKernelGGL(DVP_PICK(NAME), dim3((la.count + la.group - 1) / la.group), w64, 0, c->stream, c->d, la); }
					DVP_GROUP_LAUNCH(dvp_weak_eval_candidates, 0)
					hipLaunchKernelGGL(dvp_weak_select_views, lg, block, 0, c->stream, c->d, la);
					DVP_GROUP_LAUNCH(dvp_weak_eval_planes, 1)
					hipLaunchKernelGGL(dvp_weak_make_hypotheses, lg, block, 0, c->stream, c->d, la);
					DVP_GROUP_LAUNCH(dvp_weak_eval_first_view, 2)
					DVP_GROUP_LAUNCH(dvp_weak_eval_survivors, 3)
#undef DVP_GROUP_LAUNCH
					hipLaunchKernelGGL(dvp_weak_adopt, lg, block, 0, c->stream, c->d, la);
					hipLaunchKernelGGL(ex ? dvp_weak_final_cost_exact : dvp_weak_final_cost, lg64, w64, 0, c->stream, c->d, la);
#undef DVP_PICK
				} else if (c->d.anchor_tab) {
					if (c->images8_ok) hipLaunchKernelGGL(ex ? dvp_weak_update_wave_exact_u8 : dvp_weak_update_wave_u8, dim3(la.count), dim3(64), 0, c->stream, c->d, la);
					else if (c->images16_ok) hipLaunchKernelGGL(ex ? dvp_weak_update_wave_exact_f16 : dvp_weak_update_wave_f16, dim3(la.count), dim3(64), 0, c->stream, c->d, la);
					else hipLaunchKernelGGL(ex ? dvp_weak_update_wave_exact : dvp_weak_update_wave, dim3(la.count), dim3(64), 0, c->stream, c->d, la);
				} else {
					if (c->images8_ok) hipLaunchKernelGGL(ex ? dvp_weak_update_wave_exact_u8_notab : dvp_weak_update_wave_u8_notab, dim3(la.count), dim3(64), 0, c->stream, c->d, la);
					else if (c->images16_ok) hipLaunchKernelGGL(ex ? dvp_weak_update_wave_exact_f16_notab : dvp_weak_update_wave_f16_notab, dim3(la.count), dim3(64), 0, c->stream, c->d, la);
					else hipLaunchKernelGGL(ex ? dvp_weak_update_wave_exact_notab : dvp_weak_update_wave_notab, dim3(la.count), dim3(64), 0, c->stream, c->d, la);
				}
				break;
			}
			HIP_TRY(c, hipGetLastError());
		}
	} else {
	if (stage == DVP_ST_GEN_EDGE_INFORM && c->d.params.use_edge) {
		hipLaunchKernelGGL(dvp_edge_rays, dim3((c->W + c->H + 255) / 256, 8), dim3(256), 0, c->stream, c->d, 0);
		HIP_TRY(c, hipGetLastError());
	}
	if (stage == DVP_ST_GEN_EDGE_INFORM && c->d.params.use_label && c->d.weak_count > 0) {
		if (!c->label_stop) {
			if (dalloc(c, &c->label_stop, c->L * 8, false)) return 1;
			sync_dev_struct(c);
		}
		hipLaunchKernelGGL(dvp_edge_rays, dim3((c->W + c->H + 255) / 256, 8), dim3(256), 0, c->stream, c->d, 1);
		HIP_TRY(c, hipGetLastError());
	}
	switch (stage) {
	case DVP_ST_GEN_EDGE_INFORM:
		if (!fused) {
			if (gen_candidates_all_views(c->d)) hipLaunchKernelGGL(dvp_gen_candidates_views, dim3(g.grid(), (unsigned)((c->NI - 1 + kCandGroup - 1) / kCandGroup)), block, 0, c->stream, c->d, a);
			else hipLaunchKernelGGL(dvp_gen_candidates, dim3(g.grid(), (unsigned)(c->NI - 1)), block, 0, c->stream, c->d, a);
		}
		hipLaunchKernelGGL(c->d.sampler ? dvp_gen_edge_inform_exact : dvp_gen_edge_inform, grid, block, 0, c->stream, c->d, a);
		break;
	case DVP_ST_RANDOM_INIT: hipLaunchKernelGGL(c->d.sampler ? dvp_random_init_exact : dvp_random_init, grid, block, 0, c->stream, c->d, a); break;
	case DVP_ST_STRONG_UPDATE:
		if (c->strong_split && c->NI - 1 <= 16) {
			ensure_strong_split_buffers(c);
		}
		if (c->strong_split && c->NI - 1 <= 16) {
			const int S = c->NI - 1;
			if (c->eval_items) hipLaunchKernelGGL(c->d.sampler ? dvp_strong_eval_items_exact : dvp_strong_eval_items, wave_grid, wave_block, 0, c->stream, c->d, a);
			else hipLaunchKernelGGL(c->d.sampler ? dvp_strong_eval_exact : dvp_strong_eval, wave_grid, wave_block, 0, c->stream, c->d, a);
			if (S <= 4) hipLaunchKernelGGL(dvp_strong_decide_v4, grid, block, 0, c->stream, c->d, a);
			else if (S <= 6) hipLaunchKernelGGL(dvp_strong_decide_v6, grid, block, 0, c->stream, c->d, a);
			else if (S <= 8) hipLaunchKernelGGL(dvp_strong_decide_v8, grid, block, 0, c->stream, c->d, a);
			else if (S <= 10) hipLaunchKernelGGL(dvp_strong_decide_v10, grid, block, 0, c->stream, c->d, a);
			else if (S <= 12) hipLaunchKernelGGL(dvp_strong_decide_v12, grid, block, 0, c->stream, c->d, a);
			else hipLaunchKernelGGL(dvp_strong_decide_v16, grid, block, 0, c->stream, c->d, a);
			if (c->refine_lanes && (size_t)c->pitch * (c->H + 2 * kImgPad) * 8 * c->NI < ((size_t)1 << 32))
				hipLaunchKernelGGL(c->d.sampler ? dvp_strong_refine_lanes_exact : dvp_strong_refine_lanes, wave_grid, wave_block, 0, c->stream, c->d, a);
			else hipLaunchKernelGGL(c->d.sampler ? dvp_strong_refine_exact : dvp_strong_refine, wave_grid, wave_block, 0, c->stream, c->d, a);
		}
		else if (c->NI - 1 <= kNarrowViews) hipLaunchKernelGGL(c->d.sampler ? dvp_strong_update_v8_exact : dvp_strong_update_v8, grid, block, 0, c->stream, c->d, a);
		else if (c->NI - 1 <= 16) hipLaunchKernelGGL(c->d.sampler ? dvp_strong_update_v16_exact : dvp_strong_update_v16, grid, block, 0, c->stream, c->d, a);
		else hipLaunchKernelGGL(c->d.sampler ? dvp_strong_update_exact : dvp_strong_update, grid, block, 0, c->stream, c->d, a);
		break;
	case DVP_ST_GET_DEPTH_NORMAL: hipLaunchKernelGGL(c->d.sampler ? dvp_get_depth_normal_exact : dvp_get_depth_normal, grid, block, 0, c->stream, c->d, a); break;
	case DVP_ST_FILTER_STRONG: hipLaunchKernelGGL(c->d.sampler ? dvp_filter_strong_exact : dvp_filter_strong, grid, block, 0, c->stream, c->d, a); break;
	case DVP_ST_DEPTH_TO_WEAK: {
		const bool sweep_passes = fused && c->sweep_split && (c->d.params.geom_consistency || c->sweep_force);
		if (sweep_passes) ensure_sweep_buffers(c);
		if (sweep_passes && c->sweep_split) {
			const bool ex = c->d.sampler != 0;
			LaunchArgs s0 = a, s1 = a, sb = a;
			s0.iter = 0; s1.iter = 1; sb.iter = kSweepBorderOnly;
			const int etx = (c->W + 63) / 64, ety = (c->H + kSweepRows - 1) / kSweepRows;
			s0.tiles_x = s1.tiles_x = etx; s0.tiles = s1.tiles = etx * ety;
			const dim3 egrid((unsigned)(etx * ety), (unsigned)(c->NI - 1));
			hipLaunchKernelGGL(dvp_sweep_prepare, grid, block, 0, c->stream, c->d, a);
			const int band_rows = c->sweep_band_rows > 0 ? c->sweep_band_rows : c->H;
			for (int row0 = 0; row0 < c->H; row0 += band_rows) {
				Dev db = c->d;
				LaunchArgs b0 = s0, b1 = s1;
				dim3 bgrid = egrid;
				b0.rows = b1.rows = 0;
				if (c->sweep_band_rows > 0) {
					const int row1 = std::min(c->H, row0 + band_rows);
					db.sweep_px0 = row0 * c->W; db.sweep_row0 = row0; db.sweep_row1 = row1;
					const int bty = (row1 - row0 + kSweepRows - 1) / kSweepRows;
					b0.rows = b1.rows = row0 / kSweepRows;
					b0.tiles = b1.tiles = etx * bty;
					bgrid = dim3((unsigned)(etx * bty), (unsigned)(c->NI - 1));
				}
				hipLaunchKernelGGL(ex ? dvp_sweep_eval_exact : dvp_sweep_eval, bgrid, dim3(64), 0, c->stream, db, b0);
				hipLaunchKernelGGL(dvp_sweep_decide1, grid, block, 0, c->stream, db, a);
				if (sweep_window(c->d.params) < 30) {
					hipLaunchKernelGGL(ex ? dvp_sweep_eval_exact : dvp_sweep_eval, bgrid, dim3(64), 0, c->stream, db, b1);
				}
				hipLaunchKernelGGL(dvp_sweep_decide2, grid, block, 0, c->stream, db, a);
			}
			if (c->W >= 12 && c->H >= 12) {
				const long long frame = 12ll * c->W + 12ll * (c->H - 12);
				hipLaunchKernelGGL(ex ? dvp_sweep_border_exact : dvp_sweep_border, dim3((unsigned)((frame + 63) / 64)), dim3(64), 0, c->stream, c->d, sb);
			}
			else hipLaunchKernelGGL(ex ? dvp_depth_to_weak_refine_exact : dvp_depth_to_weak_refine, grid, block, 0, c->stream, c->d, sb);
		}
		else if (fused) hipLaunchKernelGGL(c->d.sampler ? dvp_depth_to_weak_refine_exact : dvp_depth_to_weak_refine, grid, block, 0, c->stream, c->d, a);
		else hipLaunchKernelGGL(c->d.sampler ? dvp_depth_to_weak_exact : dvp_depth_to_weak, grid, block, 0, c->stream, c->d, a);
		break;
	}
	case DVP_ST_LOCAL_REFINE: hipLaunchKernelGGL(c->d.sampler ? dvp_local_refine_exact : dvp_local_refine, grid, block, 0, c->stream, c->d, a); break;
	}
	HIP_TRY(c, hipGetLastError());
	}
	HIP_TRY(c, hipEventRecord(ep.b, c->stream));
	c->events.push_back(ep);
	if (c->profiling) {
		unsigned long long n = 0;
		HIP_TRY(c, hipMemcpyAsync(&n, c->eval_counter, 8, hipMemcpyDeviceToHost, c->stream));
		HIP_TRY(c, hipStreamSynchronize(c->stream));
		c->timings.ncc_evals[stage] += n;
	}
	return 0;
}

int dvp_run_stage(dvp_ctx* c, int stage, int iter, int colour) {
	if (set_device(c)) return 1;
	return launch_stage(c, stage, iter, colour);
}

static int ensure_edge_buffers(dvp_ctx* c, int slots) {
	if (dvpedge::scratch_reserve(c->eg, c->L)) { c->error = "dvp_edge_map: out of device memory"; return 1; }
	for (int k = 0; k < slots; ++k) {
		dvp_ctx::EdgeSlot& sl = c->eg_slot[k];
		if (!sl.map && hipMalloc(reinterpret_cast<void**>(&sl.map), c->L) != hipSuccess) { (void)hipGetLastError(); sl.map = nullptr; c->error = "dvp_edge_map: out of device memory"; return 1; }
		if (!sl.done && hipEventCreateWithFlags(&sl.done, hipEventDisableTiming) != hipSuccess) { (void)hipGetLastError(); sl.done = nullptr; c->error = "dvp_edge_map: hipEventCreate failed"; return 1; }
	}
	return 0;
}

int dvp_ctx_reserve(dvp_ctx* c, int weak_pixels, int flags) {
	if (set_device(c)) return 1;
	if (flags & 1) ensure_strong_split_buffers(c);
	if (flags & 2) ensure_sweep_buffers(c);
	if ((flags & 4) && !c->no_images8 && !c->no_images16 && ensure_images16(c)) return 1;
	if ((flags & 8) && ensure_edge_buffers(c, 2)) return 1;
	if ((flags & 16) && dvpvc::scratch_reserve(c->vc, c->L, c->NI - 1)) { c->error = "dvp_ctx_reserve: out of device memory (view clean-up)"; return 1; }
	if (weak_pixels > 0) {
		const size_t wc = std::min<size_t>((size_t)weak_pixels, c->L);
		if (grow_anchor_table(c, wc)) return 1;
		if (c->anchor_tab && grow_weak_phase_buffers(c, wc)) return 1;
		c->anchor_tab_valid = false;
	}
	return 0;
}

int dvp_synchronize(dvp_ctx* c) {
	if (set_device(c)) return 1;
	HIP_TRY(c, hipStreamSynchronize(c->stream));
	return 0;
}

int dvp_run_patchmatch(dvp_ctx* c) {
	c->anchor_tab_valid = false;
	if (set_device(c)) return 1;
	EventPair tot, itl;
	tot.stage = EV_TOTAL; itl.stage = EV_ITER_LOOP;
	HIP_TRY(c, hipEventCreate(&tot.a)); HIP_TRY(c, hipEventCreate(&tot.b));
	HIP_TRY(c, hipEventCreate(&itl.a)); HIP_TRY(c, hipEventCreate(&itl.b));
	HIP_TRY(c, hipEventRecord(tot.a, c->stream));
	const bool side_work = c->d.weak_count > 0;
	bool masked = side_work && c->cand_mask_on && (c->cand_mask_mode == 1 || (c->cand_mask_mode < 0 && (size_t)c->d.weak_count * 25 < c->L));
	if (masked && !c->cand_mask) {
		void *m = nullptr, *l = nullptr, *n = nullptr, *sv = nullptr;
		if (hipMalloc(&m, c->L) != hipSuccess || hipMalloc(&l, c->L * 4) != hipSuccess || hipMalloc(&n, 4) != hipSuccess || hipMalloc(&sv, (c->L + c->W) * 4) != hipSuccess) {
			(void)hipGetLastError();
			for (void* p : { m, l, n, sv }) if (p) (void)hipFree(p);
			c->cand_mask_on = masked = false;
		} else {
			for (void* p : { m, l, n, sv }) c->allocs.push_back(p);
			c->cand_mask = (uint8_t*)m; c->cand_list = (unsigned*)l; c->cand_n = (unsigned*)n; c->sel_snap = (uint32_t*)sv;
		}
	}
	if (side_work && !masked) {
		if (!c->sector_taps) { c->error = "dvp_set_params must be called before running kernels"; return 1; }
		HIP_TRY(c, hipEventRecord(c->side_fork, c->stream));
		HIP_TRY(c, hipStreamWaitEvent(c->side, c->side_fork, 0));
		const LaunchGeom g = make_geom(c->W, c->H, false);
		LaunchArgs a;
		a.tiles_x = g.tiles_x; a.tiles = g.tiles; a.rows = g.rows; a.half = 0; a.colour = 0; a.iter = 0;
		if (gen_candidates_all_views(c->d)) hipLaunchKernelGGL(dvp_gen_candidates_views, dim3(g.grid(), (unsigned)((c->NI - 1 + kCandGroup - 1) / kCandGroup)), dim3(256), 0, c->side, c->d, a);
		else hipLaunchKernelGGL(dvp_gen_candidates, dim3(g.grid(), (unsigned)(c->NI - 1)), dim3(256), 0, c->side, c->d, a);
		HIP_TRY(c, hipGetLastError());
		HIP_TRY(c, hipEventRecord(c->side_join, c->side));
	}
	if (launch_stage(c, DVP_ST_GEN_EDGE_INFORM, 0, 0, true)) return 1;
	if (launch_stage(c, DVP_ST_FIND_NEAREST_STRONG, 0, 0)) return 1;
	if (launch_stage(c, DVP_ST_GEN_NEIGHBOURS, 0, 0)) return 1;
	if (launch_stage(c, DVP_ST_NEIGHBOUR_UPDATE, 0, 0)) return 1;
	if (side_work && !masked) HIP_TRY(c, hipStreamWaitEvent(c->stream, c->side_join, 0));
	if (masked) {
		if (!c->sector_taps) { c->error = "dvp_set_params must be called before running kernels"; return 1; }
		HIP_TRY(c, hipMemcpyAsync(c->sel_snap, c->selected_views, (c->L + c->W) * 4, hipMemcpyDeviceToDevice, c->stream));
		HIP_TRY(c, hipEventRecord(c->side_fork, c->stream));
		HIP_TRY(c, hipStreamWaitEvent(c->side, c->side_fork, 0));
		HIP_TRY(c, hipMemsetAsync(c->cand_mask, 0, c->L, c->side));
		HIP_TRY(c, hipMemsetAsync(c->cand_n, 0, 4, c->side));
		ListArgs la;
		la.base = 0; la.count = c->d.weak_black + c->d.weak_red; la.iter = 0; la.covered_rows = 0; la.group = 1; la.run = 1;
		if (la.count > 0) hipLaunchKernelGGL(dvp_anchor_mask, dim3((la.count + 255) / 256), dim3(256), 0, c->side, c->d, la, c->cand_mask);
		hipLaunchKernelGGL(dvp_mask_compact, dim3((unsigned)((c->L + 255) / 256)), dim3(256), 0, c->side, c->cand_mask, c->L, c->cand_list, c->cand_n);
		const size_t most = std::min(c->L, (size_t)la.count * (DVP_NEIGHBOUR_NUM - 1));
		Dev dsnap = c->d;
		dsnap.selected_views = c->sel_snap;
		if (most > 0 && gen_candidates_all_views(dsnap)) hipLaunchKernelGGL(dvp_gen_candidates_views_list, dim3((unsigned)((most + 255) / 256), (unsigned)((c->NI - 1 + kCandGroup - 1) / kCandGroup)), dim3(256), 0, c->side, dsnap, c->cand_list, c->cand_n);
		else if (most > 0) hipLaunchKernelGGL(dvp_gen_candidates_list, dim3((unsigned)((most + 255) / 256), (unsigned)(c->NI - 1)), dim3(256), 0, c->side, dsnap, c->cand_list, c->cand_n);
		HIP_TRY(c, hipGetLastError());
		HIP_TRY(c, hipEventRecord(c->side_join, c->side));
	}
	if (launch_stage(c, DVP_ST_RANDOM_INIT, 0, 0)) return 1;
	HIP_TRY(c, hipEventRecord(itl.a, c->stream));
	for (int i = 0; i < c->d.params.max_iterations; ++i) {
		if (launch_stage(c, DVP_ST_STRONG_UPDATE, i, 0)) return 1;
		if (launch_stage(c, DVP_ST_STRONG_UPDATE, i, 1)) return 1;
		if (c->d.weak_count == 0 && i == c->d.params.max_iterations - 1)
			HIP_TRY(c, hipMemcpyAsync(c->fit_planes, c->planes, c->L * 16, hipMemcpyDeviceToDevice, c->stream));
		if (c->d.weak_count > 0) {
			if (masked && i == 0) HIP_TRY(c, hipStreamWaitEvent(c->stream, c->side_join, 0));
			if (launch_stage(c, DVP_ST_RANSAC_FIT, i, 0)) return 1;
			if (c->weak_phased && !c->anchor_tab_off && !getenv("DVP_WEAK_SPLIT_COLOURS")) {
				if (launch_stage(c, DVP_ST_WEAK_UPDATE, i, 2)) return 1;
			} else {
				if (launch_stage(c, DVP_ST_WEAK_UPDATE, i, 0)) return 1;
				if (launch_stage(c, DVP_ST_WEAK_UPDATE, i, 1)) return 1;
			}
		}
	}
	if (masked && c->d.params.max_iterations <= 0) HIP_TRY(c, hipStreamWaitEvent(c->stream, c->side_join, 0));
	HIP_TRY(c, hipEventRecord(itl.b, c->stream));
	if (launch_stage(c, DVP_ST_GET_DEPTH_NORMAL, 0, 0)) return 1;
	if (launch_stage(c, DVP_ST_FILTER_STRONG, 0, 0)) return 1;
	if (launch_stage(c, DVP_ST_FILTER_STRONG, 0, 1)) return 1;
	if (launch_stage(c, DVP_ST_DEPTH_TO_WEAK, 0, 0, true)) return 1;
	HIP_TRY(c, hipEventRecord(tot.b, c->stream));
	c->events.push_back(tot);
	c->events.push_back(itl);
	return 0;
}

int dvp_download_state(dvp_ctx* c, float* planes, uint32_t* views, uint8_t* weak, int32_t* radius) {
	if (set_device(c)) return 1;
	const size_t L = c->L;
	if (planes) HIP_TRY(c, hipMemcpyAsync(planes, c->planes, L * 16, hipMemcpyDeviceToHost, c->stream));
	if (views) HIP_TRY(c, hipMemcpyAsync(views, c->selected_views, L * 4, hipMemcpyDeviceToHost, c->stream));
	if (weak) HIP_TRY(c, hipMemcpyAsync(weak, c->weak_info, L, hipMemcpyDeviceToHost, c->stream));
	if (radius) HIP_TRY(c, hipMemcpyAsync(radius, c->radius, L * 4, hipMemcpyDeviceToHost, c->stream));
	HIP_TRY(c, hipStreamSynchronize(c->stream));
	return 0;
}

static void download_done(dvp_ctx* c) {
	{ std::lock_guard<std::mutex> lk(c->dl_m); c->dl_busy = false; c->dl_fetching = false; }
	c->dl_cv.notify_all();
}
int dvp_download_maps_begin(dvp_ctx* c, float* depth_device_copy) {
	if (set_device(c)) return 1;
	{
		int limit_s = 120;
		if (const char* e = getenv("DVP_DOWNLOAD_WAIT_S")) limit_s = atoi(e);
		std::unique_lock<std::mutex> lk(c->dl_m);
		if (!c->dl_cv.wait_for(lk, std::chrono::seconds(limit_s > 0 ? limit_s : 1), [c] { return !c->dl_busy; })) {
			c->error = "dvp_download_maps_begin: the maps staged by the previous dvp_download_maps_begin were never fetched (dvp_download_maps_finish)";
			return 1;
		}
		c->dl_busy = true;
	}
	const size_t L = c->L;
	auto fail = [c]() { download_done(c); return 1; };
	if (!c->maps_out && dalloc(c, &c->maps_out, L * 25, false)) return fail();
	float* d_depth = reinterpret_cast<float*>(c->maps_out);
	float* d_normal = d_depth + L;
	uint8_t* d_state = c->maps_out + L * 24;
	uint32_t* d_views = reinterpret_cast<uint32_t*>(c->maps_out + L * 16);
	hipLaunchKernelGGL(dvp_unpack_maps, dim3((unsigned)((L + 255) / 256)), dim3(256), 0, c->stream, c->planes, c->weak_info, L, c->d.params.depth_min, c->d.params.depth_max,
	                   d_depth, d_normal, d_state);
	if (hipGetLastError() != hipSuccess) { c->error = "dvp_download_maps_begin: launch failed"; return fail(); }
	if (c->vc_on) {
		if (dvpvc::scratch_reserve(c->vc, L, c->vc_num_src)) { c->error = "dvp_download_maps_begin: out of device memory (view clean-up)"; return fail(); }
		if (dvpvc::launch_clean(c->stream, c->vc, c->selected_views, c->W, c->H, c->vc_num_src, c->vc_min_region, d_views)) { c->error = "dvp_download_maps_begin: launch failed (view clean-up)"; return fail(); }
	}
	if ((!c->vc_on && hipMemcpyAsync(d_views, c->selected_views, L * 4, hipMemcpyDeviceToDevice, c->stream) != hipSuccess) ||
	    hipMemcpyAsync(c->maps_out + L * 20, c->radius, L * 4, hipMemcpyDeviceToDevice, c->stream) != hipSuccess ||
	    (depth_device_copy && hipMemcpyAsync(depth_device_copy, d_depth, L * 4, hipMemcpyDeviceToDevice, c->stream) != hipSuccess) ||
	    hipStreamSynchronize(c->stream) != hipSuccess) { c->error = "dvp_download_maps_begin: device copies failed"; return fail(); }
	return 0;
}
int dvp_download_maps_finish(dvp_ctx* c, float* depth, float* normal_xyz, uint32_t* views, uint8_t* weak, int32_t* radius) {
	t_finish_error.c = c;
	t_finish_error.msg.clear();
	{
		std::lock_guard<std::mutex> lk(c->dl_m);
		if (!c->dl_busy || c->dl_fetching) { t_finish_error.msg = "dvp_download_maps_finish without dvp_download_maps_begin"; return 1; }
		c->dl_fetching = true;
	}
	auto fail = [c](const char* what) { t_finish_error.msg = what; download_done(c); return 1; };
	if (hipSetDevice(c->device) != hipSuccess) return fail("hipSetDevice failed");
	if (!depth || !normal_xyz || !weak) return fail("dvp_download_maps: depth, normal and weak_info are required");
	if (!c->copy && hipStreamCreateWithFlags(&c->copy, hipStreamNonBlocking) != hipSuccess) return fail("hipStreamCreate failed");
	const size_t L = c->L;
	if (!c->maps_host && hipHostMalloc(reinterpret_cast<void**>(&c->maps_host), L * 25, hipHostMallocDefault) != hipSuccess) { (void)hipGetLastError(); c->maps_host = nullptr; }
	if (c->maps_host) {
		if (hipMemcpyAsync(c->maps_host, c->maps_out, L * 25, hipMemcpyDeviceToHost, c->copy) != hipSuccess || hipStreamSynchronize(c->copy) != hipSuccess)
			return fail("dvp_download_maps_finish: copy to the host failed");
		struct Part { void* dst; size_t off, bytes; };
		const Part parts[5] = { { depth, 0, L * 4 }, { normal_xyz, L * 4, L * 12 }, { weak, L * 24, L }, { views, L * 16, L * 4 }, { radius, L * 20, L * 4 } };
		std::vector<std::thread> team;
		const uint8_t* src = c->maps_host;
// ... 48 lines not shown
		c->error = "dvp_edge_map_begin: launch failed"; return 1;
	}
	HIP_TRY(c, hipEventRecord(sl.done, c->stream));
	std::lock_guard<std::mutex> lk(c->eg_m);
	sl.seq = ++c->eg_seq;
	sl.pending = true;
	return 0;
}

int dvp_edge_map_finish(dvp_ctx* c, uint8_t* edge) {
	t_finish_error.c = c;
	t_finish_error.msg.clear();
	auto fail = [](const char* what) { t_finish_error.msg = what; return 1; };
	if (!edge) return fail("dvp_edge_map_finish: edge is required");
	if (hipSetDevice(c->device) != hipSuccess) { (void)hipGetLastError(); return fail("dvp_edge_map_finish: hipSetDevice failed"); }
	int k = -1;
	{
		std::lock_guard<std::mutex> lk(c->eg_m);
		for (int i = 0; i < 2; ++i)
			if (c->eg_slot[i].pending && !c->eg_slot[i].fetching && (k < 0 || c->eg_slot[i].seq < c->eg_slot[k].seq)) k = i;
		if (k < 0) return fail("dvp_edge_map_finish: no edge map was begun (dvp_edge_map_begin)");
		c->eg_slot[k].fetching = true;
		if (!c->eg_copy && hipStreamCreateWithFlags(&c->eg_copy, hipStreamNonBlocking) != hipSuccess) { (void)hipGetLastError(); c->eg_copy = nullptr; c->eg_slot[k].fetching = false; return fail("dvp_edge_map_finish: hipStreamCreate failed"); }
	}
	dvp_ctx::EdgeSlot& sl = c->eg_slot[k];
	const bool ok = hipEventSynchronize(sl.done) == hipSuccess && hipMemcpyAsync(edge, sl.map, c->L, hipMemcpyDeviceToHost, c->eg_copy) == hipSuccess &&
	                hipStreamSynchronize(c->eg_copy) == hipSuccess;
	{
		std::lock_guard<std::mutex> lk(c->eg_m);
		sl.fetching = false;
		sl.pending = false;
	}
	c->eg_cv.notify_all();
	if (!ok) { (void)hipGetLastError(); return fail("dvp_edge_map_finish: copy to the host failed"); }
	return 0;
}

int dvp_preview_begin(dvp_ctx* c, int kinds, int quality) {
	if (set_device(c)) return 1;
	if (kinds < 1 || kinds > 7) { c->error = "dvp_preview_begin: kinds must be a non-empty set of DVP_PREVIEW_DEPTH | NORMAL | WEAK"; return 1; }
	if (quality < 1 || quality > 100) { c->error = "dvp_preview_begin: quality must be 1..100"; return 1; }
	c->pv_kinds = 0;
	const size_t L = c->L;
	for (int k = 0; k < 3; ++k)
		if ((kinds >> k & 1) && !c->pv_bgr[k] && dalloc(c, &c->pv_bgr[k], L * 3, false)) return 1;
	if (!c->pv_total) HIP_TRY(c, hipHostMalloc(reinterpret_cast<void**>(&c->pv_total), 3 * sizeof(unsigned long long), hipHostMallocDefault));
	if (!c->pv_done) HIP_TRY(c, hipEventCreateWithFlags(&c->pv_done, hipEventDisableTiming));
	if (!c->pv_copy) HIP_TRY(c, hipStreamCreateWithFlags(&c->pv_copy, hipStreamNonBlocking));
	auto bgr = [&](int k) { return (kinds >> k & 1) ? c->pv_bgr[k] : nullptr; };
	if (dvpjpeg::launch_render(c->stream, reinterpret_cast<const float*>(c->planes), c->weak_info, L, c->d.params.depth_min, c->d.params.depth_max,
	                           bgr(0), bgr(1), bgr(2))) { c->error = "dvp_preview_begin: render launch failed"; return 1; }
	for (int k = 0; k < 3; ++k)
		if ((kinds >> k & 1) && dvpjpeg::encode_begin(c->pv_enc[k], c->stream, c->pv_bgr[k], (long long)c->W * 3, c->W, c->H, 3, quality, 0, &c->pv_total[k])) {
			c->error = std::string("dvp_preview_begin: ") + c->pv_enc[k].error; return 1;
		}
	HIP_TRY(c, hipStreamSynchronize(c->stream));
	for (int k = 0; k < 3; ++k)
		if ((kinds >> k & 1) && dvpjpeg::encode_write(c->pv_enc[k], c->stream, c->pv_total[k])) {
			c->error = std::string("dvp_preview_begin: ") + c->pv_enc[k].error; return 1;
		}
	HIP_TRY(c, hipEventRecord(c->pv_done, c->stream));
	c->pv_kinds = kinds;
	return 0;
}
static int preview_slot(dvp_ctx* c, int kind, const char* who) {
	t_finish_error.c = c;
	t_finish_error.msg.clear();
	const int k = kind == DVP_PREVIEW_DEPTH ? 0 : kind == DVP_PREVIEW_NORMAL ? 1 : kind == DVP_PREVIEW_WEAK ? 2 : -1;
	if (k < 0 || !(c->pv_kinds >> k & 1)) { t_finish_error.msg = std::string(who) + ": that preview was not begun (dvp_preview_begin)"; return -1; }
	if (hipSetDevice(c->device) != hipSuccess || hipEventSynchronize(c->pv_done) != hipSuccess) { t_finish_error.msg = std::string(who) + ": device error"; return -1; }
	return k;
}
int dvp_preview_finish(dvp_ctx* c, int kind, uint8_t* dst, long long capacity, long long* bytes) {
	const int k = preview_slot(c, kind, "dvp_preview_finish");
	if (k < 0) return 1;
	const dvpjpeg::Encoder& e = c->pv_enc[k];
	const long long n = (long long)dvpjpeg::file_bytes(e);
	if (bytes) *bytes = n;
	if (!dst || capacity < n) { t_finish_error.msg = "dvp_preview_finish: capacity below the encoded size (*bytes)"; return 1; }
	memcpy(dst, e.header, e.header_len);
	if (hipMemcpyAsync(dst + e.header_len, e.out, e.data_bytes, hipMemcpyDeviceToHost, c->pv_copy) != hipSuccess || hipStreamSynchronize(c->pv_copy) != hipSuccess) {
		t_finish_error.msg = "dvp_preview_finish: copy to the host failed"; return 1;
	}
	dst[n - 2] = 0xFF;
	dst[n - 1] = 0xD9;
	return 0;
}
int dvp_preview_pixels(dvp_ctx* c, int kind, uint8_t* bgr) {
	const int k = preview_slot(c, kind, "dvp_preview_pixels");
	if (k < 0) return 1;
	if (!bgr || hipMemcpyAsync(bgr, c->pv_bgr[k], c->L * 3, hipMemcpyDeviceToHost, c->pv_copy) != hipSuccess || hipStreamSynchronize(c->pv_copy) != hipSuccess) {
		t_finish_error.msg = "dvp_preview_pixels: copy to the host failed"; return 1;
	}
	return 0;
}

int dvp_download_maps(dvp_ctx* c, float* depth, float* normal_xyz, uint32_t* views, uint8_t* weak, int32_t* radius) {
	if (!depth || !normal_xyz || !weak) { c->error = "dvp_download_maps: depth, normal and weak_info are required"; return 1; }
	if (dvp_download_maps_begin(c, nullptr)) return 1;
	return dvp_download_maps_finish(c, depth, normal_xyz, views, weak, radius);
}

static void* buffer_ptr(dvp_ctx* c, int id, size_t* bytes) {
	const size_t L = c->L, S = (size_t)c->NI - 1;
	const size_t wc = c->d.weak_count > 0 ? (size_t)c->d.weak_count : 1;
	switch (id) {
	case DVP_BUF_PLANES: *bytes = L * 16; return c->planes;
	case DVP_BUF_COSTS: *bytes = L * 4; return c->costs;
	case DVP_BUF_SELECTED_VIEWS: *bytes = L * 4; return c->selected_views;
	case DVP_BUF_VIEW_WEIGHT: *bytes = L * 32; return c->view_weight;
	case DVP_BUF_WEAK_INFO: *bytes = L; return c->weak_info;
	case DVP_BUF_WEAK_RELIABLE: *bytes = L; return c->weak_reliable;
	case DVP_BUF_WEAK_NEAREST_STRONG: *bytes = L * 4; return c->weak_nearest_strong;
	case DVP_BUF_NEIGHBOURS_MAP: *bytes = L * 4; return c->neighbours_map;
	case DVP_BUF_NEIGHBOURS: *bytes = wc * DVP_NEIGHBOUR_NUM * 4; return c->neighbours;
	case DVP_BUF_FIT_PLANES: *bytes = L * 16; return c->fit_planes;
	case DVP_BUF_CANDIDATE: *bytes = L * S * 8 * 4; return c->candidate;
	case DVP_BUF_EDGE: *bytes = L; return c->edge;
	case DVP_BUF_EDGE_NEIGH: *bytes = L * 8 * 4; return c->edge_neigh;
	case DVP_BUF_LABEL: *bytes = L * 4; return c->label;
	case DVP_BUF_LABEL_BOUNDARY: *bytes = wc * 8 * 4; return c->label_boundary;
	case DVP_BUF_COMPLEX: *bytes = wc * 4; return c->complex_;
	case DVP_BUF_RADIUS: *bytes = L * 4; return c->radius;
	}
	*bytes = 0;
	return nullptr;
}
long long dvp_buffer_bytes(dvp_ctx* c, int id) { size_t b; buffer_ptr(c, id, &b); return (long long)b; }
static void candidate_transpose(const dvp_ctx* c, const s2* src, s2* dst, bool to_device) {
	const size_t L = c->L, S = (size_t)c->NI - 1;
	for (size_t v = 0; v < S; ++v)
		for (size_t p = 0; p < L; ++p) {
			const size_t dev = (v * L + p) * 8, host = (p * S + v) * 8;
			std::memcpy(to_device ? dst + dev : dst + host, to_device ? src + host : src + dev, 8 * sizeof(s2));
		}
}
int dvp_download_buffer(dvp_ctx* c, int id, void* dst) {
	if (set_device(c)) return 1;
	size_t b; void* p = buffer_ptr(c, id, &b);
	if (!p) { c->error = "bad or unallocated buffer id"; return 1; }
	if (id == DVP_BUF_CANDIDATE) {
		std::vector<s2> tmp(b / sizeof(s2));
		HIP_TRY(c, hipMemcpyAsync(tmp.data(), p, b, hipMemcpyDeviceToHost, c->stream));
		HIP_TRY(c, hipStreamSynchronize(c->stream));
		candidate_transpose(c, tmp.data(), (s2*)dst, false);
		return 0;
	}
	HIP_TRY(c, hipMemcpyAsync(dst, p, b, hipMemcpyDeviceToHost, c->stream));
	HIP_TRY(c, hipStreamSynchronize(c->stream));
	return 0;
}
int dvp_upload_buffer(dvp_ctx* c, int id, const void* src) {
	c->anchor_tab_valid = false;
	if (set_device(c)) return 1;
	size_t b; void* p = buffer_ptr(c, id, &b);
	if (!p) { c->error = "bad or unallocated buffer id"; return 1; }
	std::vector<s2> tmp;
	if (id == DVP_BUF_CANDIDATE) {
		tmp.resize(b / sizeof(s2));
		candidate_transpose(c, (const s2*)src, tmp.data(), true);
		src = tmp.data();
	}
	HIP_TRY(c, hipMemcpyAsync(p, src, b, hipMemcpyHostToDevice, c->stream));
	HIP_TRY(c, hipStreamSynchronize(c->stream));
	return 0;
}
int dvp_weak_count(dvp_ctx* c) { return c->d.weak_count; }

int dvp_get_timings(dvp_ctx* c, DvpTimings* out) {
	if (set_device(c)) return 1;
	HIP_TRY(c, hipStreamSynchronize(c->stream));
	for (auto& e : c->events) {
		float ms = 0.0f;
		HIP_TRY(c, hipEventElapsedTime(&ms, e.a, e.b));
		if (e.stage == EV_TOTAL) c->timings.total_ms += ms;
		else if (e.stage == EV_ITER_LOOP) c->timings.iter_loop_ms += ms;
		else { c->timings.stage_ms[e.stage] += ms; c->timings.stage_launches[e.stage] += 1; }
		(void)hipEventDestroy(e.a);
		(void)hipEventDestroy(e.b);
	}
	c->events.clear();
	if (out) *out = c->timings;
	return 0;
}
int dvp_reset_timings(dvp_ctx* c) {
	if (dvp_get_timings(c, nullptr)) return 1;
	std::memset(&c->timings, 0, sizeof(DvpTimings));
	return 0;
}

namespace {
struct DevBuf {
	void* p = nullptr;
	~DevBuf() { if (p) (void)hipFree(p); }
};
struct EventPairGuard {
	hipEvent_t a = nullptr, b = nullptr;
	~EventPairGuard() { if (a) (void)hipEventDestroy(a); if (b) (void)hipEventDestroy(b); }
};
}

int dvp_eval_cost_vectors(dvp_ctx* c, const int32_t* px, const float* planes, int n, float* out, float* kernel_ms) {
	if (set_device(c)) return 1;
	if (!c->sector_taps) { c->error = "dvp_set_params must be called first"; return 1; }
	if (n <= 0) return 0;
	const size_t S = (size_t)c->NI - 1;
	DevBuf dpx, dpl, dout;
	EventPairGuard ev;
	HIP_TRY(c, hipMalloc(&dpx.p, (size_t)n * 8));
	HIP_TRY(c, hipMalloc(&dpl.p, (size_t)n * 16));
	HIP_TRY(c, hipMalloc(&dout.p, (size_t)n * S * 4));
	HIP_TRY(c, hipMemcpyAsync(dpx.p, px, (size_t)n * 8, hipMemcpyHostToDevice, c->stream));
	HIP_TRY(c, hipMemcpyAsync(dpl.p, planes, (size_t)n * 16, hipMemcpyHostToDevice, c->stream));
	HIP_TRY(c, hipEventCreate(&ev.a));
	HIP_TRY(c, hipEventCreate(&ev.b));
	HIP_TRY(c, hipEventRecord(ev.a, c->stream));
	hipLaunchKernelGGL(dvp_cost_vectors, dim3((n + 255) / 256), dim3(256), 0, c->stream, c->d, (const int*)dpx.p, (const f4*)dpl.p, n, (float*)dout.p);
	HIP_TRY(c, hipGetLastError());
	HIP_TRY(c, hipEventRecord(ev.b, c->stream));
	HIP_TRY(c, hipMemcpyAsync(out, dout.p, (size_t)n * S * 4, hipMemcpyDeviceToHost, c->stream));
	HIP_TRY(c, hipStreamSynchronize(c->stream));
	if (kernel_ms) HIP_TRY(c, hipEventElapsedTime(kernel_ms, ev.a, ev.b));
	return 0;
}

int dvp_bench_cost_kernel(dvp_ctx* c, int repeat, float* mean_kernel_ms, uint64_t* evals_per_launch) {
	if (set_device(c)) return 1;
	if (!c->sector_taps) { c->error = "dvp_set_params must be called first"; return 1; }
	if (repeat < 1) repeat = 1;
	const LaunchGeom g = make_geom(c->W, c->H, false);
	LaunchArgs a;
	a.tiles_x = g.tiles_x; a.tiles = g.tiles; a.rows = g.rows; a.half = 0; a.colour = 0; a.iter = 0;
	EventPairGuard ev;
	HIP_TRY(c, hipEventCreate(&ev.a));
	HIP_TRY(c, hipEventCreate(&ev.b));
	hipLaunchKernelGGL(dvp_cost_all_pixels, dim3(g.grid()), dim3(256), 0, c->stream, c->d, a, c->scratch_out);
	HIP_TRY(c, hipEventRecord(ev.a, c->stream));
	for (int i = 0; i < repeat; ++i)
		hipLaunchKernelGGL(dvp_cost_all_pixels, dim3(g.grid()), dim3(256), 0, c->stream, c->d, a, c->scratch_out);
	HIP_TRY(c, hipEventRecord(ev.b, c->stream));
	HIP_TRY(c, hipGetLastError());
	HIP_TRY(c, hipStreamSynchronize(c->stream));
	float ms = 0.0f;
	HIP_TRY(c, hipEventElapsedTime(&ms, ev.a, ev.b));
	if (mean_kernel_ms) *mean_kernel_ms = ms / repeat;
	if (evals_per_launch) *evals_per_launch = (uint64_t)c->L * (uint64_t)(c->NI - 1);
	return 0;
}

#ifdef DVP_PROBE
int dvp_probe(dvp_ctx* c, int mode, int K, int stride, int repeat, float* mean_ms, float* checksum) {
	if (set_device(c)) return 1;
	const LaunchGeom g = make_geom(c->W, c->H, false);
	LaunchArgs a;
	a.tiles_x = g.tiles_x; a.tiles = g.tiles; a.rows = g.rows; a.half = 0; a.colour = 0; a.iter = 0;
	const int S = c->NI - 1, P = 64 / S;
	const int waves = ((c->W + P - 1) / P) * c->H;
	EventPairGuard ev;
	HIP_TRY(c, hipEventCreate(&ev.a));
	HIP_TRY(c, hipEventCreate(&ev.b));
	for (int i = 0; i <= repeat; ++i) {
		if (i == 1) HIP_TRY(c, hipEventRecord(ev.a, c->stream));
		HIP_TRY(c, hipMemsetAsync(c->scratch_out, 0, c->L * 4, c->stream));
		if (mode == 0) hipLaunchKernelGGL(dvp_probe_a, dim3(g.grid()), dim3(256), 0, c->stream, c->d, a, c->scratch_out, K, stride);
		else if (mode == 1) hipLaunchKernelGGL(dvp_probe_b, dim3((waves + 3) / 4), dim3(256), 0, c->stream, c->d, c->scratch_out, K, stride);
		else if (mode == 2) hipLaunchKernelGGL(dvp_probe_c, dim3(g.grid()), dim3(256), 0, c->stream, c->d, a, c->scratch_out, (unsigned)K);
		else hipLaunchKernelGGL(dvp_probe_d, dim3((unsigned)(g.tiles_x * c->H * (64 / DVP_PROBE_NPX))), dim3(64), 0, c->stream, c->d, c->scratch_out, (unsigned)K);
	}
	HIP_TRY(c, hipEventRecord(ev.b, c->stream));
	HIP_TRY(c, hipGetLastError());
	HIP_TRY(c, hipStreamSynchronize(c->stream));
	float ms = 0.0f;
	HIP_TRY(c, hipEventElapsedTime(&ms, ev.a, ev.b));
	*mean_ms = ms / repeat;
	std::vector<float> h(c->L);
	HIP_TRY(c, hipMemcpy(h.data(), c->scratch_out, c->L * 4, hipMemcpyDeviceToHost));
	double sum = 0;
	for (float v : h) sum += v;
	*checksum = (float)(sum / (double)c->L);
	return 0;
}
#endif

}
```

dvp-mvs_amd/csrc/dvp_strong.hpp:

```cpp
#ifndef DVP_STRONG_HPP_
#define DVP_STRONG_HPP_

#include "dvp_ncc.hpp"

namespace dvp {

DVP_HD void sort_small(float* v, int n) {
	for (int i = 1; i < n; i++) {
		const float tmp = v[i];
		int j = i;
		for (; j >= 1 && tmp < v[j - 1]; j--) v[j] = v[j - 1];
		v[j] = tmp;
	}
}

DVP_HD f4 random_normal_yzl_sel(const Dev& d, int px, int py, Rng& rng, float depth, uint32_t sel) {
	const int W = d.width, H = d.height;
	const DvpCamera rc = load_camera(d, 0);
	f3 vd[20];
	{
		const f4 v0 = view_direction(rc, px, py, depth);
		vd[0] = mk3(v0.x, v0.y, v0.z);
	}
	int index = 1;
// ... 370 lines not shown
					if (vw[j] > 0) fc += vw[j] * cost_array[k * MV + j];
				final_costs[k] = fc / weight_norm;
			}
			min_cost_idx = 0;
			{
				float mc = final_costs[0];
				for (int k = 1; k < 8; ++k)
					if (final_costs[k] <= mc) { mc = final_costs[k]; min_cost_idx = k; }
			}
			plane = d.planes_snap[center];
			mask = sel_mask;
		} else {
			const int i = slot - 17;
			plane = ref_normals[i];
			plane.w = distance_to_origin(rc, px, py, ref_depths[i], plane);
			mask = sel_mask;
		}

		if (mask) {
			for (int v = 0; v < S; ++v) {
				if ((mask >> v) & 1) {
					cv[v] = ncc_old<SMP>(d, c, px, py, v + 1, plane);
					if (nevals) *nevals += 1;
				}
			}
		}

		if (slot < 8) {
			if (pos >= 0) {
				flag |= 1u << slot;
				positions[slot] = pos;
				for (int v = 0; v < S; ++v) cost_array[slot * MV + v] = cv[v];
			}
		} else if (slot < 16) {
			const int k = slot - 8;
			if (pos >= 0) {
				const bool had = (flag >> k) & 1;
				flag |= 1u << k;
				int good0 = 0, good1 = 0, bad0 = 0, bad1 = 0;
				for (int j = 0; j < S; ++j) {
					const float a = cost_array[k * MV + j], b = cv[j];
					if (a < good_thr) good0++;
					if (a > 1.2f) bad0++;
					if (b < good_thr) good1++;
					if (b > 1.2f) bad1++;
				}
				if (!had || good1 > good0 || (good1 == good0 && bad1 < bad0)) {
					positions[k] = pos;
					for (int j = 0; j < S; ++j) cost_array[k * MV + j] = cv[j];
				}
			}
		} else if (slot == 16) {
			float cn = 0.0f;
			for (int v = 0; v < S; ++v)
				if (vw[v] > 0) cn += vw[v] * cv[v];
			cost_now = cn / weight_norm;
			costs_center = cost_now;
			plane_now = d.planes_snap[center];
			depth_now = depth_from_plane(rc, plane_now, px, py);
			if ((flag >> min_cost_idx) & 1) {
				const f4 cand = d.planes_snap[positions[min_cost_idx]];
				const float db = depth_from_plane(rc, cand, px, py);
				if (db >= P.depth_min && db <= P.depth_max && final_costs[min_cost_idx] < cost_now) {
					depth_now = db;
					plane_now = cand;
					cost_now = final_costs[min_cost_idx];
					selected_views_written = true;
				}
			}
			Rng rd(d.seed, (uint32_t)center, rng_site(PH_STRONG, iter, SUB_DEPTH_RAND));
			Rng rn(d.seed, (uint32_t)center, rng_site(PH_STRONG, iter, SUB_NORMAL));
			Rng rp(d.seed, (uint32_t)center, rng_site(PH_STRONG, iter, SUB_DEPTH_PERT));
			const float depth_rand = rd.uniform() * (P.depth_max - P.depth_min) + P.depth_min;
			if (selected_views_written) d.selected_views[center] = sel_mask;
			const f4 n_rand = random_normal_yzl(d, px, py, rn, depth_now);
			const float dmin_p = (1 - 0.02f) * depth_now, dmax_p = (1 + 0.02f) * depth_now;
			const float depth_pert = rp.uniform() * (dmax_p - dmin_p) + dmin_p;
			f4 n_pert = plane_now;
			normalize3(&n_pert);
			ref_depths[0] = depth_rand; ref_normals[0] = plane_now;
			ref_depths[1] = depth_now;  ref_normals[1] = n_rand;
			ref_depths[2] = depth_rand; ref_normals[2] = n_rand;
			ref_depths[3] = depth_now;  ref_normals[3] = n_pert;
			ref_depths[4] = depth_now;  ref_normals[4] = n_pert;
			ref_depths[5] = depth_pert; ref_normals[5] = plane_now;
		} else {
			float tc = 0.0f;
			for (int j = 0; j < S; ++j)
				if (vw[j] > 0) tc += vw[j] * cv[j];
			tc /= weight_norm;
			const float db = depth_from_plane(rc, plane, px, py);
			if (db >= P.depth_min && db <= P.depth_max && tc < cost_now) {
				depth_now = db;
				plane_now = plane;
				cost_now = tc;
			}
		}
	}

	if (P.state == DVP_REFINE_INIT) {
		if (cost_now < costs_center - 0.1) {
			costs_center = cost_now;
			d.planes[center] = plane_now;
		}
	} else {
		costs_center = cost_now;
		d.planes[center] = plane_now;
	}
	d.costs[center] = costs_center;
}

constexpr int kSlotCur = 16;
constexpr int kSlotCount = 17;
enum { SR_PLANE = 0, SR_DEPTH = 4, SR_COST = 5, SR_CENTER = 6, SR_DRAND = 7, SR_DPERT = 8, SR_NRAND = 9, SR_DUP = 12 , SR_FIELDS = 15 };
DVP_HD size_t half_index(const Dev& d, int px, int py) { return (size_t)py * d.half_w + (size_t)(px >> 1); }
#ifndef DVP_SLOT_LAYOUT
#define DVP_SLOT_LAYOUT 1
#endif
DVP_HD int slot_place(int slot) {
#if DVP_SLOT_LAYOUT
	return slot < 8 ? 2 * slot : (slot < 16 ? 2 * (slot - 8) + 1 : slot);
#else
	return slot;
#endif
}
DVP_HD size_t slot_cost_index(const Dev& d, int slot, int v, int px, int py) {
	const size_t Lh = (size_t)d.half_w * (size_t)d.height;
	const int S = d.params.num_images - 1;
#if DVP_SLOT_LAYOUT
	return (half_index(d, px, py) * kSlotCount + (size_t)slot_place(slot)) * (size_t)S + (size_t)v;
#else
	return (size_t)(slot * S + v) * Lh + half_index(d, px, py);
#endif
}
struct SlotCostView { const float* base; size_t slot_stride, view_stride; };
DVP_HD SlotCostView slot_cost_view(const Dev& d, int px, int py) {
	const size_t Lh = (size_t)d.half_w * (size_t)d.height;
	const int S = d.params.num_images - 1;
	SlotCostView r;
#if DVP_SLOT_LAYOUT
	r.base = d.slot_costs + half_index(d, px, py) * kSlotCount * (size_t)S;
	r.slot_stride = (size_t)S;
	r.view_stride = 1;
#else
	r.base = d.slot_costs + half_index(d, px, py);
	r.slot_stride = (size_t)S * Lh;
	r.view_stride = Lh;
#endif
	return r;
}
DVP_HD bool same_plane_bits(const f4 a, const f4 b) {
	return f32_bits(a.x) == f32_bits(b.x) && f32_bits(a.y) == f32_bits(b.y) && f32_bits(a.z) == f32_bits(b.z) && f32_bits(a.w) == f32_bits(b.w);
}
DVP_HD uint32_t strong_slot_sources(const Dev& d, int center, uint32_t w[3]) {
	const size_t L = (size_t)d.width * d.height;
	f4 pl[kSlotCount];
	uint32_t have = 0, uniq = 0;
#pragma unroll
	for (int slot = 0; slot < kSlotCount; ++slot) {
		const int pos = slot < 16 ? d.search_pos[(size_t)slot * L + center] : center;
		pl[slot] = mk4(0.0f, 0.0f, 0.0f, 0.0f);
		if (pos >= 0) { pl[slot] = d.planes_snap[pos]; have |= 1u << slot; }
	}
	w[0] = w[1] = w[2] = 0;
#pragma unroll
	for (int slot = 0; slot < kSlotCount; ++slot) {
		int src = slot;
#pragma unroll
		for (int u = slot - 1; u >= 0; --u)
			if (((have >> u) & 1u) && same_plane_bits(pl[u], pl[slot])) src = u;
		if (!((have >> slot) & 1u)) continue;
		if (src == slot) uniq |= 1u << slot;
		if (slot < 8) w[0] |= (uint32_t)src << (4 * slot);
		else if (slot < 16) w[1] |= (uint32_t)src << (4 * (slot - 8));
		else w[2] = (uint32_t)src;
	}
	return uniq;
}
DVP_HD int strong_slot_source(uint32_t w0, uint32_t w1, uint32_t w2, int slot) {
	return slot < 8 ? (int)((w0 >> (4 * slot)) & 15u) : slot < 16 ? (int)((w1 >> (4 * (slot - 8))) & 15u) : (int)w2;
}
template <int SMP>
DVP_HD void strong_eval_item(const Dev& d, const PatchCtx& c, int px, int py, int slot, bool store, unsigned long long* nevals) {
	const int W = d.width;
	const int center = py * W + px;
	const int S = d.params.num_images - 1;
	const size_t L = (size_t)W * d.height;
	const int pos = slot < 16 ? d.search_pos[(size_t)slot * L + center] : center;
	const f4 plane = d.planes_snap[pos];
	for (int v = 0; v < S; ++v) {
		const float cost = ncc_old<SMP>(d, c, px, py, v + 1, plane);
		if (store) DVP_NT_STORE(4, &d.slot_costs[slot_cost_index(d, slot, v, px, py)], cost);
	}
	if (nevals && store) *nevals += (unsigned long long)S;
}
template <int SMP>
DVP_HD void strong_eval_px(const Dev& d, int px, int py, PatchTab tab, unsigned long long* nevals) {
	const int W = d.width;
	const int center = py * W + px;
	PatchCtx c;
	{
		int radius, inc;
		patch_geometry(d, center, &radius, &inc);
		build_patch_ctx(d, px, py, radius, inc, 0, tab, &c);
	}
	uint32_t w[3];
	const uint32_t uniq = strong_slot_sources(d, center, w);
	const size_t Lh = (size_t)d.half_w * (size_t)d.height, hi = half_index(d, px, py);
	uint32_t* dup = reinterpret_cast<uint32_t*>(d.strong_rec) + hi;
	dup[SR_DUP * Lh] = w[0]; dup[(SR_DUP + 1) * Lh] = w[1]; dup[(SR_DUP + 2) * Lh] = w[2];
	for (uint32_t m = uniq; m; m &= m - 1) strong_eval_item<SMP>(d, c, px, py, dvp_ctz(m), true, nevals);
}

template <int MV>
DVP_HD void load_slot_costs(const float* sc, size_t view_stride, int S, float* out) {
#if defined(__HIP_DEVICE_COMPILE__) && DVP_SLOT_LAYOUT
	typedef float f4v __attribute__((ext_vector_type(4), aligned(4)));
	constexpr int Q = (MV + 3) / 4;
	f4v q[Q];
#pragma unroll
	for (int i = 0; i < Q; ++i) q[i] = DVP_NT_LOAD(8, &reinterpret_cast<const f4v*>(sc)[i]);
#pragma unroll
	for (int v = 0; v < MV; ++v) out[v] = v < S ? q[v >> 2][v & 3] : 0.0f;
#else
#pragma unroll
	for (int v = 0; v < MV; ++v) out[v] = v < S ? sc[(size_t)v * view_stride] : 0.0f;
#endif
}

template <int MV>
DVP_HD void strong_decide_px(const Dev& d, int px, int py, int iter) {
	const SlotCostView cv = slot_cost_view(d, px, py);
	const int W = d.width;
	const int center = py * W + px;
	const DvpParams& P = d.params;
	const DvpCamera rc = load_camera(d, 0);
	const int S = P.num_images - 1;
	const size_t L = (size_t)W * d.height;
	const size_t Lh = (size_t)d.half_w * (size_t)d.height, hi = half_index(d, px, py);
	const float good_thr = 0.8f * dvp_expf((iter) * (iter) / (-90.0f));
	const uint32_t sel_entry = d.selected_views[center];
	float ca[8][MV];
	uint32_t flag = 0;
	int positions[8];
	const uint32_t* dup = reinterpret_cast<const uint32_t*>(d.strong_rec) + hi;
	const uint32_t dw0 = dup[SR_DUP * Lh], dw1 = dup[(SR_DUP + 1) * Lh], dw2 = dup[(SR_DUP + 2) * Lh];
#pragma unroll
	for (int k = 0; k < 8; ++k) {
		positions[k] = 0;
#pragma unroll
		for (int v = 0; v < MV; ++v) ca[k][v] = 0.0f;
	}
	ca[0][0] = 2.0f;
#pragma unroll
	for (int k = 0; k < 8; ++k) {
		{
			const int pos = d.search_pos[(size_t)k * L + center];
			if (pos >= 0) {
				flag |= 1u << k;
				positions[k] = pos;
				load_slot_costs<MV>(cv.base + (size_t)slot_place(strong_slot_source(dw0, dw1, dw2, k)) * cv.slot_stride, cv.view_stride, S, ca[k]);
			}
		}
		const int pos = d.search_pos[(size_t)(8 + k) * L + center];
		if (pos >= 0) {
			const bool had = (flag >> k) & 1;
			flag |= 1u << k;
			float cb[MV];
			int good0 = 0, good1 = 0, bad0 = 0, bad1 = 0;
			load_slot_costs<MV>(cv.base + (size_t)slot_place(strong_slot_source(dw0, dw1, dw2, 8 + k)) * cv.slot_stride, cv.view_stride, S, cb);
#pragma unroll
			for (int j = 0; j < MV; ++j) {
				if (j < S) {
					const float a = ca[k][j], b = cb[j];
					if (a < good_thr) good0++;
					if (a > 1.2f) bad0++;
					if (b < good_thr) good1++;
					if (b > 1.2f) bad1++;
				}
			}
			if (!had || good1 > good0 || (good1 == good0 && bad1 < bad0)) {
				positions[k] = pos;
#pragma unroll
				for (int j = 0; j < MV; ++j)
					if (j < S) ca[k][j] = cb[j];
			}
		}
	}
	float priors[MV];
#pragma unroll
	for (int i = 0; i < MV; ++i) priors[i] = 0.0f;
	{
		const int nb[4] = { center - W, center + W, center - 1, center + 1 };
#pragma unroll
		for (int i = 0; i < 4; ++i) {
			if ((flag >> (2 * i)) & 1) {
				const uint32_t sv = d.selected_views[nb[i]];
#pragma unroll
				for (int j = 0; j < MV; ++j)
					if (j < S) priors[j] += is_set(sv, j) ? 0.9f : 0.1f;
			}
		}
	}
	float probs[MV];
	const float thr = (float)(0.8 * dvp_expf((iter) * (iter) / (-90.0f)));
#pragma unroll
	for (int i = 0; i < MV; ++i) {
		probs[i] = 0.0f;
		if (i < S) {
			float count = 0;
			int count_false = 0;
			float tmpw = 0;
#pragma unroll
			for (int j = 0; j < 8; j++) {
				const float cst = ca[j][i];
				if (cst < thr) { tmpw += dvp_expf(cst * cst / (-0.18f)); count++; }
				if (cst > 1.2f) count_false++;
			}
			float pr = 0.0f;
			if (count > 2 && count_false < 3) pr = tmpw / count;
			else if (count_false < 3) pr = dvp_expf(thr * thr / (-0.32f));
			probs[i] = pr * priors[i];
		}
	}
	float psum = 0.0f;
#pragma unroll
	for (int i = 0; i < MV; ++i)
		if (i < S) psum += probs[i];
	const float inv = 1.0f / psum;
	float cum = 0.0f;
#pragma unroll
	for (int i = 0; i < MV; ++i)
		if (i < S) { cum += probs[i] * inv; probs[i] = cum; }
	int vw[MV];
#pragma unroll
	for (int i = 0; i < MV; ++i) vw[i] = 0;
	Rng rv(d.seed, (uint32_t)center, rng_site(PH_STRONG, iter, SUB_VIEW));
	for (int s = 0; s < 15; ++s) {
		const float rp = rv.uniform() - FLT_EPSILON;
		bool done = false;
#pragma unroll
		for (int v = 0; v < MV; ++v)
			if (v < S && !done && probs[v] > rp) { vw[v] += 1; done = true; }
	}
	uint32_t sel_mask = 0;
	float weight_norm = 0;
#pragma unroll
	for (int i = 0; i < MV; ++i)
		if (i < S && vw[i] > 0) { set_bit(&sel_mask, i); weight_norm += vw[i]; }
	{
		uint8_t* gvw = d.view_weight + (size_t)center * 32;
		uint32_t words[8];
#pragma unroll
		for (int w8 = 0; w8 < 8; ++w8) {
			uint32_t x = 0;
#pragma unroll
			for (int b = 0; b < 4; ++b)
				if (w8 * 4 + b < MV) x |= ((uint32_t)vw[w8 * 4 + b] & 255u) << (8 * b);
			words[w8] = x;
		}
		uint32_t* g32 = reinterpret_cast<uint32_t*>(gvw);
#pragma unroll
		for (int w8 = 0; w8 < 8; ++w8) g32[w8] = words[w8];
	}
	float final_costs[8];
#pragma unroll
	for (int k = 0; k < 8; ++k) {
		float fc = 0.0f;
#pragma unroll
		for (int j = 0; j < MV; ++j)
			if (j < S && vw[j] > 0) fc += vw[j] * ca[k][j];
		final_costs[k] = fc / weight_norm;
	}
	int min_cost_idx = 0;
	{
		float mc = final_costs[0];
#pragma unroll
		for (int k = 1; k < 8; ++k)
			if (final_costs[k] <= mc) { mc = final_costs[k]; min_cost_idx = k; }
	}
	float cn = 0.0f;
#pragma unroll
	for (int v = 0; v < MV; ++v)
		if (v < S && vw[v] > 0) cn += vw[v] * cv.base[(size_t)slot_place((int)dw2) * cv.slot_stride + (size_t)v * cv.view_stride];
	float cost_now = cn / weight_norm;
	const float costs_center = cost_now;
	f4 plane_now = d.planes_snap[center];
	float depth_now = depth_from_plane(rc, plane_now, px, py);
	bool selected_views_written = false;
	{
		float fmin = final_costs[0];
		int pmin = positions[0];
#pragma unroll
		for (int k = 1; k < 8; ++k)
			if (k == min_cost_idx) { fmin = final_costs[k]; pmin = positions[k]; }
		if ((flag >> min_cost_idx) & 1) {
			const f4 cand = d.planes_snap[pmin];
			const float db = depth_from_plane(rc, cand, px, py);
			if (db >= P.depth_min && db <= P.depth_max && fmin < cost_now) {
				depth_now = db;
				plane_now = cand;
				cost_now = fmin;
				selected_views_written = true;
			}
		}
	}
	Rng rd(d.seed, (uint32_t)center, rng_site(PH_STRONG, iter, SUB_DEPTH_RAND));
	Rng rn(d.seed, (uint32_t)center, rng_site(PH_STRONG, iter, SUB_NORMAL));
	Rng rp(d.seed, (uint32_t)center, rng_site(PH_STRONG, iter, SUB_DEPTH_PERT));
	const float depth_rand = rd.uniform() * (P.depth_max - P.depth_min) + P.depth_min;
	if (selected_views_written) d.selected_views[center] = sel_mask;
#if defined(DVP_DECIDE_YZL_GENERIC)
	const f4 n_rand = random_normal_yzl(d, px, py, rn, depth_now);
#else
	const f4 n_rand = MV <= 16 ? random_normal_yzl_views<(MV <= 16 ? MV : 16)>(d, px, py, rn, depth_now, selected_views_written ? sel_mask : sel_entry)
	                           : random_normal_yzl(d, px, py, rn, depth_now);
#endif
	const float dmin_p = (1 - 0.02f) * depth_now, dmax_p = (1 + 0.02f) * depth_now;
	const float depth_pert = rp.uniform() * (dmax_p - dmin_p) + dmin_p;
	float* rec = d.strong_rec + hi;
	rec[(SR_PLANE + 0) * Lh] = plane_now.x; rec[(SR_PLANE + 1) * Lh] = plane_now.y; rec[(SR_PLANE + 2) * Lh] = plane_now.z; rec[(SR_PLANE + 3) * Lh] = plane_now.w;
	rec[SR_DEPTH * Lh] = depth_now; rec[SR_COST * Lh] = cost_now; rec[SR_CENTER * Lh] = costs_center;
	rec[SR_DRAND * Lh] = depth_rand; rec[SR_DPERT * Lh] = depth_pert;
	rec[(SR_NRAND + 0) * Lh] = n_rand.x; rec[(SR_NRAND + 1) * Lh] = n_rand.y; rec[(SR_NRAND + 2) * Lh] = n_rand.z;
}

template <int SMP, bool LANE_WALK = false>
DVP_HD void strong_refine_px(const Dev& d, int px, int py, PatchTab tab, unsigned long long* nevals) {
	const int W = d.width;
	const int center = py * W + px;
	const DvpParams& P = d.params;
	const DvpCamera rc = load_camera(d, 0);
	const int S = P.num_images - 1;
	const size_t Lh = (size_t)d.half_w * (size_t)d.height, hi = half_index(d, px, py);
	PatchCtx c;
	{
		int radius, inc;
		patch_geometry(d, center, &radius, &inc);
		build_patch_ctx(d, px, py, radius, inc, 0, tab, &c);
	}
	const float* rec = d.strong_rec + hi;
	f4 plane_now = mk4(rec[(SR_PLANE + 0) * Lh], rec[(SR_PLANE + 1) * Lh], rec[(SR_PLANE + 2) * Lh], rec[(SR_PLANE + 3) * Lh]);
	float depth_now = rec[SR_DEPTH * Lh], cost_now = rec[SR_COST * Lh], costs_center = rec[SR_CENTER * Lh];
	const float depth_rand = rec[SR_DRAND * Lh], depth_pert = rec[SR_DPERT * Lh];
	const f4 n_rand = mk4(rec[(SR_NRAND + 0) * Lh], rec[(SR_NRAND + 1) * Lh], rec[(SR_NRAND + 2) * Lh], 0.0f);
	f4 n_pert = plane_now;
	normalize3(&n_pert);
	const uint32_t* g32 = reinterpret_cast<const uint32_t*>(d.view_weight + (size_t)center * 32);
	uint32_t wq[8];
#pragma unroll
	for (int i = 0; i < 8; ++i) wq[i] = g32[i];
	float weight_norm = 0;
	for (int i = 0; i < S; ++i) {
		const int wv = (int)((wq[i >> 2] >> (8 * (i & 3))) & 255u);
		if (wv > 0) weight_norm += wv;
	}
	const float hyp_depth[5] = { depth_rand, depth_now, depth_rand, depth_now, depth_pert };
	const f4 hyp_normal[5] = { plane_now, n_rand, n_rand, n_pert, plane_now };
	const float depth_entry = depth_now;
	const f4 plane_entry = plane_now;
	(void)depth_entry; (void)plane_entry;
	if (LANE_WALK) {
		uint32_t sel = 0;
		for (int j = 0; j < S; ++j)
			if (((wq[j >> 2] >> (8 * (j & 3))) & 255u) > 0) sel |= 1u << j;
		int hyp = 0;
		bool busy = false;
		f4 plane = plane_now;
		float db = 0.0f, tc = 0.0f;
		uint32_t todo = 0;
		for (;;) {
			while (!busy && hyp < 5) {
				plane = hyp_normal[hyp];
				plane.w = distance_to_origin(rc, px, py, hyp_depth[hyp], plane);
				db = depth_from_plane(rc, plane, px, py);
				++hyp;
				if (!(db >= P.depth_min && db <= P.depth_max)) continue;
				if (!(weight_norm > 0.0f)) continue;
				tc = 0.0f;
				todo = sel;
				busy = true;
			}
			if (!busy) break;
			const int j = dvp_ctz(todo);
			todo &= todo - 1;
			uint32_t q = wq[0];
#pragma unroll
			for (int k = 1; k < 8; ++k) q = (j >> 2) == k ? wq[k] : q;
			const int wv = (int)((q >> (8 * (j & 3))) & 255u);
			tc += wv * ncc_old_lane<SMP>(d, c, px, py, j + 1, plane);
			if (nevals) *nevals += 1;
			const bool alive = tc / weight_norm < cost_now;
			if (!alive) busy = false;
			else if (todo == 0) {
				depth_now = db;
				plane_now = plane;
				cost_now = tc / weight_norm;
				busy = false;
			}
		}
	} else
	for (int i = 0; i < 5; ++i) {
		f4 plane = hyp_normal[i];
		plane.w = distance_to_origin(rc, px, py, hyp_depth[i], plane);
		const float db = depth_from_plane(rc, plane, px, py);
		if (!(db >= P.depth_min && db <= P.depth_max)) continue;
		float tc = 0.0f;
		bool alive = weight_norm > 0.0f;
		for (int j = 0; j < S && alive; ++j) {
			const int wv = (int)((wq[j >> 2] >> (8 * (j & 3))) & 255u);
			if (wv > 0) {
				tc += wv * ncc_old<SMP>(d, c, px, py, j + 1, plane);
				if (nevals) *nevals += 1;
				alive = tc / weight_norm < cost_now;
			}
		}
		if (alive) {
			depth_now = db;
			plane_now = plane;
			cost_now = tc / weight_norm;
		}
	}
	if (P.state == DVP_REFINE_INIT) {
		if (cost_now < costs_center - 0.1) {
			costs_center = cost_now;
			d.planes[center] = plane_now;
		}
	} else {
		costs_center = cost_now;
		d.planes[center] = plane_now;
	}
	d.costs[center] = costs_center;
}

DVP_HD void get_depth_normal_px(const Dev& d, int px, int py) {
	const int center = py * d.width + px;
	f4 pl = d.planes[center];
// ... 617 lines not shown
```

dvp-mvs_amd/host/main.cpp:

```cpp
#include <sstream>
#include "APD.h"
#include <thread>
#include "comm.h"
#include <cstdlib>
#include <map>
#include <set>
#include <memory>
#include <future>
#include <mutex>
#include <condition_variable>
#include <algorithm>

namespace {

struct Options {
	path dense_folder;
	int gpu = 0, max_src = 0, iters = 3, min_scale = 2, geom_passes = 3, rank = 0, world = 1;
	uint64_t seed = 1234;
	bool fusion = true, jacobi = false, label_files = false;
	int collective_timeout_s = 600;
	bool sync_io = false;
	bool host_rescale = false;
	bool edges_on_gpu = false;
	bool labels_on_gpu = false;
// ... 303 lines not shown
			s.h = depth.rows;
		}
		RankComm::HostToDevice(s.dev, depth.ptr<float>(0), (size_t)s.w * s.h);
		APD::SetResidentDepth(image_id, s.dev, s.w, s.h);
	}
	float* Reserve(int image_id, int w, int h) {
		Slot& s = maps_[image_id];
		if (s.w != w || s.h != h) {
			APD::UnsetResidentDepth(image_id);
			RankComm::DeviceFree(s.dev);
			s.dev = RankComm::DeviceAlloc((size_t)w * h);
			s.w = w;
			s.h = h;
		}
		return s.dev;
	}
	void Commit(int image_id) {
		const Slot& s = maps_[image_id];
		if (s.dev) APD::SetResidentDepth(image_id, s.dev, s.w, s.h);
	}
	void Release() {
		APD::ClearResidentDepths();
		for (auto& kv : maps_) RankComm::DeviceFree(kv.second.dev);
		maps_.clear();
	}
private:
	struct Slot { float* dev = nullptr; int w = 0, h = 0; };
	std::map<int, Slot> maps_;
};

class LevelImages {
public:
	~LevelImages() { Release(); }
	void Fill(const std::vector<Problem*>& owned, int scale) {
		Release();
		const char* e = std::getenv("DVP_RESIDENT_IMAGES_GB");
		const size_t budget = (size_t)(e ? std::max(0, std::atoi(e)) : 24) << 30;
		size_t used = 0;
		std::set<int> ids;
		for (const Problem* p : owned) { ids.insert(p->ref_image_id); ids.insert(p->src_image_ids.begin(), p->src_image_ids.end()); }
		if (owned.empty()) return;
		Problem q = *owned[0];
		q.scale_size = scale;
		for (int id : ids) {
			int oc = 0, orr = 0;
			const Mat img = APD::CachedImage(q, id, &oc, &orr);
			const size_t count = (size_t)img.cols * img.rows;
			if (img.empty() || used + count * 4 > budget) continue;
			float* dev = RankComm::DeviceAlloc(count);
			RankComm::HostToDevice(dev, img.ptr<float>(0), count);
			blocks_.push_back(dev);
			used += count * 4;
			APD::SetResidentImage(id, scale, dev, img.cols, img.rows, oc, orr);
		}
	}
	void Release() {
		APD::ClearResidentImages();
		for (float* b : blocks_) RankComm::DeviceFree(b);
		blocks_.clear();
	}
private:
	std::vector<float*> blocks_;
};

void ShareLevelImages(RankComm& comm, std::vector<Problem>& problems, const std::vector<int>& owner_of, int scale) {
	if (comm.world() <= 1) return;
	APD::ReserveImageCache(problems.size());
	for (Problem& p : problems) {
		p.scale_size = scale;
		const int owner = owner_of[(size_t)p.index];
		int meta[4] = { 0, 0, 0, 0 };
		Mat img;
		if (comm.rank() == owner) {
			img = APD::CachedImage(p, p.ref_image_id, &meta[2], &meta[3]);
			meta[0] = img.cols;
			meta[1] = img.rows;
		}
		comm.BroadcastHost(meta, sizeof(meta), owner);
		if (comm.rank() != owner) img = Mat(meta[1], meta[0], CV_32FC1);
		comm.BroadcastHost(img.data, (size_t)meta[0] * meta[1] * sizeof(float), owner);
		if (comm.rank() != owner) APD::InsertCachedImage(p, p.ref_image_id, img, meta[2], meta[3]);
	}
}

Options ParseOptions(int argc, char** argv) {
	Options o;
	o.dense_folder = argv[1];
	int a = 2;
	if (argc > 2 && argv[2][0] != '-') { o.gpu = std::atoi(argv[2]); a = 3; }
	for (; a < argc; ++a) {
		const std::string s = argv[a];
		auto val = [&]() { return (a + 1 < argc) ? std::atoll(argv[++a]) : 0ll; };
		if (s == "--max-src") o.max_src = (int)val();
		else if (s == "--iters") o.iters = (int)val();
		else if (s == "--min-scale") o.min_scale = (int)val();
		else if (s == "--passes") o.geom_passes = (int)val();
		else if (s == "--seed") o.seed = (uint64_t)val();
		else if (s == "--rank") o.rank = (int)val();
		else if (s == "--world") o.world = (int)val();
		else if (s == "--job") { if (a + 1 < argc) o.job = argv[++a]; }
		else if (s == "--transport") { if (a + 1 < argc) o.transport = argv[++a]; }
		else if (s == "--collective-timeout") o.collective_timeout_s = (int)val();
		else if (s == "--jacobi") o.jacobi = true;
		else if (s == "--labels") o.label_files = true;
		else if (s == "--no-fusion") o.fusion = false;
		else if (s == "--sync-io") o.sync_io = true;
		else if (s == "--views-in-flight") { if (a + 1 < argc) o.views_in_flight = std::min(APD::kMaxViewsInFlight, std::max(1, atoi(argv[++a]))); }
		else if (s == "--in-flight-pixels") { if (a + 1 < argc) o.in_flight_pixels = atoll(argv[++a]); }
		else if (s == "--previews") o.previews = true;
		else if (s == "--edges-on" && a + 1 < argc) {
			const std::string where = argv[++a];
			if (where != "host" && where != "gpu") { std::cerr << "--edges-on takes host or gpu\n"; std::exit(1); }
			o.edges_on_gpu = where == "gpu";
		}
		else if (s == "--labels-on" && a + 1 < argc) {
			const std::string where = argv[++a];
			if (where != "host" && where != "gpu") { std::cerr << "--labels-on takes host or gpu\n"; std::exit(1); }
			o.labels_on_gpu = where == "gpu";
		}
		else if (s == "--cleanup-on" && a + 1 < argc) {
			const std::string where = argv[++a];
			if (where != "host" && where != "gpu") { std::cerr << "--cleanup-on takes host or gpu\n"; std::exit(1); }
			o.cleanup_on_gpu = where == "gpu";
		}
		else if (s == "--host-rescale") o.host_rescale = true;
		else if (s == "--fusion") { if (a + 1 < argc) o.fusion_kind = argv[++a]; }
		else if (s == "--fusion-on") { if (a + 1 < argc) o.fusion_on_host = std::string(argv[++a]) == "host"; }
	}
	if (o.world > 1) o.jacobi = true;
	if (o.job.empty())
		for (const char* e : { "DVP_JOB_ID", "TORCHELASTIC_RUN_ID", "SLURM_JOB_ID" })
			if (const char* v = std::getenv(e)) { o.job = v; break; }
	return o;
}

}

int main(int argc, char** argv) {
	if (argc < 2) {
		std::cerr << "USAGE: apd dense_folder [gpu_index] [--previews] [--max-src N] [--iters N] [--min-scale S] [--passes P] [--seed X] [--rank R --world N [--job ID]] [--jacobi] [--no-fusion | --fusion KIND] [--fusion-on device|host] [--edges-on host|gpu] [--labels-on host|gpu] [--cleanup-on host|gpu] [--views-in-flight N]\n";
		return EXIT_FAILURE;
	}
	const Options opt = ParseOptions(argc, argv);
	const bool main_timing = std::getenv("DVP_HOST_TIMING") != nullptr;
	auto main_t = std::chrono::steady_clock::now();
	auto main_lap = [&](const std::string& what) {
		if (!main_timing) return;
		const auto now = std::chrono::steady_clock::now();
		std::cout << "[main] " << what << ": " << std::chrono::duration_cast<std::chrono::microseconds>(now - main_t).count() / 1000.0 << " ms" << std::endl;
		main_t = now;
	};
	std::filesystem::create_directories(opt.dense_folder / "APD");
	setenv("DVP_SWEEP_BAND_GB", "24", 0);
	SetHostThreadShare(opt.world);
	if (opt.world > 1) std::cout << "rank " << opt.rank << " of " << opt.world << ": " << HostThreads() << " host threads (of " << std::thread::hardware_concurrency() << " cores)" << std::endl;
	APD::SetDevice(opt.gpu);
	{
		const int node = RankComm::BindProcessNearDevice(opt.gpu);
		if (node >= 0) std::cout << "GPU " << opt.gpu << " hangs off NUMA node " << node << ": process confined to its CPUs" << std::endl;
	}
	APD::SetSeed(opt.seed);
	APD::SetUseLabelFiles(opt.label_files);
	APD::SetEdgesOnDevice(opt.edges_on_gpu);
	APD::SetCleanupOnDevice(opt.cleanup_on_gpu);
	APD::SetLabelsOnDevice(opt.labels_on_gpu);
	SetResultCache(!opt.sync_io);
	APD::SetDeviceRescale(!opt.sync_io && !opt.host_rescale);
	g_device_maps = !opt.sync_io && !opt.host_rescale;
	RankComm comm(opt.rank, opt.world, opt.gpu, (opt.dense_folder / "APD" / ".rccl_id").string(), opt.job, opt.collective_timeout_s, opt.transport);
	DvpSetFatalHook([](const char* msg) { if (RankComm* c = RankComm::Current()) if (c->world() > 1) c->Abort(msg); });

	std::vector<Problem> problems = ReadViewGraph(opt.dense_folder, opt.max_src);
	for (Problem& p : problems) p.show_medium_result = opt.previews;
	std::cout << "There are " << problems.size() << " problems needed to be processed!" << std::endl;
	const std::vector<int> owner_of = AssignViews(problems, opt.world);
	if (opt.world > 1) {
		std::cout << "rank " << opt.rank << " owns views";
		for (const Problem& p : problems) if (owner_of[(size_t)p.index] == opt.rank) std::cout << " " << p.index;
		std::cout << std::endl;
	}
	{
		std::vector<path> mine;
		for (const Problem& p : problems)
			if (owner_of[(size_t)p.index] == opt.rank) mine.push_back(opt.dense_folder / "images" / (ToFormatIndex(p.ref_image_id) + ".jpg"));
		if (opt.world == 1)
			for (const Problem& p : problems)
				for (int id : p.src_image_ids) mine.push_back(opt.dense_folder / "images" / (ToFormatIndex(id) + ".jpg"));
		APD::PrefetchDecoded(mine);
	}
	main_lap("start-up (options, rendezvous, view graph, decode prefetch started)");
	const int round_num = PyramidLevels(problems);
	main_lap("PyramidLevels (first image decoded)");
	std::cout << "Round nums: " << round_num << std::endl;

	std::vector<Pass> plan;
	for (int level = 0; level < round_num; ++level) {
		const int scale = 1 << (round_num - 1 - level);
		if (scale < opt.min_scale && round_num != 1) break;
		plan.push_back(Pass{ level, scale, -1 });
		for (int j = 0; j < opt.geom_passes; ++j) plan.push_back(Pass{ level, scale, j });
	}

	g_final_iteration = (int)plan.size() - 1;

	std::unique_ptr<DepthExchange> exchange;
	std::unique_ptr<InPlaceDepths> inplace;
	if (opt.jacobi) { exchange.reset(new DepthExchange(comm, problems, owner_of)); APD::SetResidentDownloader(&RankComm::DeviceToHost); }
	else if (!opt.sync_io) inplace.reset(new InPlaceDepths());
	int shared_scale = -1;
	LevelImages level_images;
	for (size_t it = 0; it < plan.size(); ++it) {
		const Pass& pass = plan[it];
		const bool new_level = pass.scale != shared_scale;
		main_t = std::chrono::steady_clock::now();
		if (new_level) {
			ShareLevelImages(comm, problems, owner_of, pass.scale);
			shared_scale = pass.scale;
			if (exchange) exchange->Release();
		}
		std::map<int, Mat> mine;
		std::vector<Problem*> owned;
		for (Problem& problem : problems) {
			ConfigurePass(problem, pass, (int)it, opt.iters, round_num);
			if (owner_of[(size_t)problem.index] == opt.rank) owned.push_back(&problem);
		}
		if (new_level && !opt.sync_io) level_images.Fill(owned, pass.scale);
		if (new_level) main_lap("level " + std::to_string(pass.level) + ": images shared + resident on the device");
		if (!opt.sync_io && it + 1 < plan.size() && plan[it + 1].scale != pass.scale && !owned.empty()) {
			int nw = 0, nh = 0;
			if (APD::LevelSize(*owned[0], plan[it + 1].scale, &nw, &nh)) APD::PrewarmContext(nw, nh, (int)owned[0]->src_image_ids.size() + 1, plan[it + 1].scale);
			std::vector<Problem> mine_next;
			for (const Problem* p : owned) mine_next.push_back(*p);
			APD::PrefetchLevelImages(mine_next, plan[it + 1].scale);
		}
		std::vector<std::future<void>> edge_jobs;
		auto start_edge_jobs = [&edge_jobs](const std::vector<Problem>& views) {
			struct Queue { std::mutex m; size_t next = 0; std::vector<std::pair<Problem, std::vector<path>>> items; };
			auto q = std::make_shared<Queue>();
			for (const Problem& p : views) {
				std::vector<path> outs = ProblemEdgeOutputs(p);
				for (const path& f : outs) ExpectResult(f);
				if (!outs.empty()) q->items.emplace_back(p, std::move(outs));
			}
			const int helpers = (int)std::min<size_t>(q->items.size(), (size_t)std::max(1, std::min(4, HostThreads() / 4)));
			for (int h = 0; h < helpers; ++h)
				edge_jobs.push_back(std::async(std::launch::async, [q]() {
					SetThisThreadHostThreads(2);
					for (;;) {
						size_t i;
						{ std::lock_guard<std::mutex> lk(q->m); i = q->next++; }
						if (i >= q->items.size()) return;
						GetProblemEdges(q->items[i].first, q->items[i].second);
					}
				}));
		};
		if (!opt.sync_io) {
			std::vector<Problem> views;
			if (pass.geom_index < 0)
				for (const Problem* p : owned) views.push_back(*p);
			if (it + 1 < plan.size() && plan[it + 1].scale != pass.scale && plan[it + 1].geom_index < 0)
				for (const Problem* p : owned) {
					Problem q = *p;
					ConfigurePass(q, plan[it + 1], (int)it + 1, opt.iters, round_num);
					views.push_back(q);
				}
			if (!views.empty()) start_edge_jobs(views);
		}
		int in_flight = 1;
		if (!opt.sync_io && (pass.geom_index < 0 || exchange) && !owned.empty()) {
			int lw = 0, lh = 0;
			if (APD::LevelSize(*owned[0], pass.scale, &lw, &lh) && (size_t)lw * lh <= (size_t)opt.in_flight_pixels) in_flight = opt.views_in_flight > 0 ? opt.views_in_flight : 2;
			in_flight = (int)std::min<size_t>((size_t)std::max(1, in_flight), owned.size());
		}
		if (it + 1 == plan.size() && opt.fusion && opt.rank == 0 && !opt.sync_io) PrefetchFusionImages(opt.dense_folder, problems);
		main_lap("pass " + std::to_string(it) + ": helpers started");
		const auto pass_t0 = std::chrono::steady_clock::now();
		if (in_flight <= 1) {
			for (size_t k = 0; k < owned.size(); ++k) {
				Problem& problem = *owned[k];
				if (pass.geom_index < 0 && opt.sync_io) GetProblemEdges(problem);
				bool on_device = false;
				ViewResult r = ProcessProblem(problem, [&](int w, int h) -> float* {
					if (!inplace || !g_device_maps) return nullptr;
					on_device = true;
					return inplace->Reserve(problem.ref_image_id, w, h);
				});
				if (exchange) mine[problem.index] = r.depth;
				if (inplace && on_device) inplace->Commit(problem.ref_image_id);
				else if (inplace) inplace->Update(problem.ref_image_id, r.depth);
			}
		} else {
			std::atomic<size_t> next{0};
			std::mutex results;
			std::vector<std::thread> workers;
			const int team = std::max(2, HostThreads() / in_flight);
			for (int wkr = 0; wkr < in_flight; ++wkr)
				workers.emplace_back([&, team]() {
					RankComm::BindThisThread(opt.gpu);
					SetThisThreadHostThreads(team);
					for (;;) {
						const size_t k = next++;
						if (k >= owned.size()) return;
						Problem& problem = *owned[k];
						std::ostringstream log;
						SetViewLog(&log);
						bool on_device = false;
// ... 54 lines not shown
```

Measured before the change: 59.76.

## Cache per-pixel candidate plane costs across iterations in the strong update

Adds a per-pixel plane-cost cache keyed by exact plane bits. A new planning kernel compares each pixel's candidate planes with the cached keys and assigns each slot a cache place. The eval stage then computes NCC costs only for planes that are not already cached, and the decide stage reads costs through the per-slot place map. The epoch is bumped on every state, parameter or image upload and on every run, so reuse happens only across iterations within one run. In exchange it adds an extra kernel launch, larger full-resolution cost buffers and key/header traffic; the host app turns it off by default.

After: 61.07, median of 6. 1.02x the previous value.

```diff
diff --git a/__graft_entry__.py b/__graft_entry__.py
--- a/__graft_entry__.py
+++ b/__graft_entry__.py
@@ -21,6 +21,7 @@
     subprocess.check_call(["make", "-s", "-C", os.path.join(ROOT, "tests", "edges_host")])
     subprocess.check_call(["make", "-s", "-C", os.path.join(ROOT, "tests", "viewclean_host")])
     subprocess.check_call(["make", "-s", "-C", os.path.join(ROOT, "tests", "labels_host")])
+    subprocess.check_call(["make", "-s", "-C", os.path.join(ROOT, "tests", "reuse_host")])
     pkg = importlib.import_module("dvp-mvs_amd")
     lib = pkg.get_capi().lib()
     missing = [s for s in pkg.get_capi().EXPORTS if not hasattr(lib, s)]
diff --git a/dvp-mvs_amd/csrc/dvp_dev.hpp b/dvp-mvs_amd/csrc/dvp_dev.hpp
--- a/dvp-mvs_amd/csrc/dvp_dev.hpp
+++ b/dvp-mvs_amd/csrc/dvp_dev.hpp
@@ -52,6 +52,13 @@
 
 struct AnchorRec;
 struct WeakRec;
+struct alignas(16) PlaneKey { uint32_t w[4]; };
+struct alignas(16) ReuseHdr {
+	uint32_t valid;
+	uint32_t radius;
+	uint32_t epoch;
+	uint32_t eval;
+};
 struct Dev {
 	int width, height, num_images;
 	int pitch;
@@ -98,6 +105,10 @@
 	int* search_pos;
 	float* slot_costs;
 	float* strong_rec;
+	float* reuse_costs;
+	PlaneKey* reuse_keys;
+	ReuseHdr* reuse_hdr;
+	uint32_t reuse_epoch;
 	f4* sweep_rec;
 	float* sweep_cost;
 	float* sweep_pc;
diff --git a/dvp-mvs_amd/csrc/dvp_engine.hip b/dvp-mvs_amd/csrc/dvp_engine.hip
--- a/dvp-mvs_amd/csrc/dvp_engine.hip
+++ b/dvp-mvs_amd/csrc/dvp_engine.hip
@@ -144,11 +144,15 @@
 		int radius, inc;
 		patch_geometry(d, center, &radius, &inc);
 		build_patch_ctx(d, px, py, radius, inc, 0, c.tab, &c);
-		uint32_t w[3];
-		uniq = strong_slot_sources(d, center, w);
-		const size_t Lh = (size_t)d.half_w * (size_t)d.height;
-		uint32_t* dup = reinterpret_cast<uint32_t*>(d.strong_rec) + half_index(d, px, py);
-		dup[SR_DUP * Lh] = w[0]; dup[(SR_DUP + 1) * Lh] = w[1]; dup[(SR_DUP + 2) * Lh] = w[2];
+		if (d.reuse_hdr) uniq = d.reuse_hdr[center].eval;
+		else {
+			uint32_t src[3], w[3];
+			uniq = strong_slot_sources(d, center, src);
+			strong_source_places(src, w);
+			const size_t Lh = (size_t)d.half_w * (size_t)d.height;
+			uint32_t* dup = reinterpret_cast<uint32_t*>(d.strong_rec) + half_index(d, px, py);
+			dup[SR_DUP * Lh] = w[0]; dup[(SR_DUP + 1) * Lh] = w[1]; dup[(SR_DUP + 2) * Lh] = w[2];
+		}
 	}
 	const int n = __popc(uniq);
 	int incl = n;
@@ -617,6 +621,13 @@
 	int px, py;
 	if (block_to_pixel(blockIdx.x, threadIdx.x & 63, threadIdx.x >> 6, a.tiles_x, a.tiles, a.rows, a.half, a.colour, d.width, d.height, &px, &py))
 		strong_search_px(d, px, py);
+}
+
+extern "C" __global__ void __launch_bounds__(256) dvp_strong_plan(const Dev d, const LaunchArgs a) {
+	int px, py;
+	if (block_to_pixel(blockIdx.x, threadIdx.x & 63, threadIdx.x >> 6, a.tiles_x, a.tiles, a.rows, a.half, a.colour, d.width, d.height, &px, &py) &&
+	    d.weak_info[px + py * d.width] != DVP_WEAK)
+		strong_plan_px(d, px, py);
 }
 
 extern "C" __global__ void __launch_bounds__(256) dvp_edge_rays(const Dev d, int what) {
@@ -997,6 +1008,9 @@
 	int* search_pos = nullptr;
 	float* slot_costs = nullptr;
 	float* strong_rec = nullptr;
+	float* reuse_costs = nullptr; PlaneKey* reuse_keys = nullptr; ReuseHdr* reuse_hdr = nullptr;
+	bool strong_reuse = true;
+	uint32_t reuse_epoch = 0;
 	bool strong_split = true;
 	bool eval_items = true;
 	bool refine_lanes = true;
@@ -1098,6 +1112,14 @@
 	*p = nullptr;
 }
 
+static void bump_reuse_epoch(dvp_ctx* c) {
+	if (++c->reuse_epoch == 0) {
+		if (c->reuse_hdr) (void)hipMemsetAsync(c->reuse_hdr, 0, c->L * sizeof(ReuseHdr), c->stream);
+		c->reuse_epoch = 1;
+	}
+	c->d.reuse_epoch = c->reuse_epoch;
+}
+
 static size_t img16_plane_bytes(int W, int H) { return (size_t)img16_tiles_x(W) * img16_tiles_y(H) * 128; }
 
 static void sync_dev_struct(dvp_ctx* c) {
@@ -1111,6 +1133,7 @@
 	d.search_pos = c->search_pos;
 	d.sweep_px0 = 0; d.sweep_row0 = 0; d.sweep_row1 = 0;
 	d.sweep_rec = c->sweep_rec; d.sweep_cost = c->sweep_cost; d.sweep_pc = c->sweep_pc; d.slot_costs = c->slot_costs; d.strong_rec = c->strong_rec; d.half_w = (c->W + 1) / 2;
+	d.reuse_costs = c->reuse_costs; d.reuse_keys = c->reuse_keys; d.reuse_hdr = c->reuse_hdr; d.reuse_epoch = c->reuse_epoch;
 	d.planes = c->planes; d.planes_snap = c->planes_snap; d.costs = c->costs; d.costs_snap = c->costs_snap;
 	d.selected_views = c->selected_views; d.view_weight = c->view_weight; d.weak_info = c->weak_info;
 	d.weak_reliable = c->weak_reliable; d.weak_nearest_strong = c->weak_nearest_strong;
@@ -1153,6 +1176,8 @@
 	c->no_images8 = getenv("DVP_NO_IMAGES8") != nullptr;
 	c->no_images16 = getenv("DVP_NO_IMAGES16") != nullptr;
 	if (const char* e = getenv("DVP_STRONG_SPLIT")) c->strong_split = atoi(e) != 0;
+	if (const char* e = getenv("DVP_STRONG_REUSE")) c->strong_reuse = atoi(e) != 0;
+	bump_reuse_epoch(c);
 	if (const char* e = getenv("DVP_REFINE_LANES")) c->refine_lanes = atoi(e) != 0;
 	if (const char* e = getenv("DVP_EVAL_ITEMS")) c->eval_items = atoi(e) != 0;
 	if (const char* e = getenv("DVP_SWEEP_SPLIT")) { c->sweep_split = atoi(e) != 0; c->sweep_force = atoi(e) == 2; }
@@ -1325,12 +1350,14 @@
 }
 int dvp_upload_images(dvp_ctx* c, const float* const* images, int pitch_floats) {
 	c->anchor_tab_valid = false;
+	bump_reuse_epoch(c);
 	if (upload_planes(c, c->image_stage, images, pitch_floats, hipMemcpyHostToDevice, c->images)) return 1;
 	c->have_images = true;
 	return 0;
 }
 int dvp_upload_images_device(dvp_ctx* c, const float* const* images, int pitch_floats) {
 	c->anchor_tab_valid = false;
+	bump_reuse_epoch(c);
 	if (upload_planes(c, c->image_stage, images, pitch_floats, hipMemcpyDeviceToDevice, c->images)) return 1;
 	c->have_images = true;
 	return 0;
@@ -1353,6 +1380,7 @@
 }
 
 int dvp_upload_cameras(dvp_ctx* c, const DvpCamera* cams, int n) {
+	bump_reuse_epoch(c);
 	if (set_device(c)) return 1;
 	if (n != c->NI) { c->error = "dvp_upload_cameras: n != num_images"; return 1; }
 	HIP_TRY(c, hipMemcpyAsync(c->cameras, cams, sizeof(DvpCamera) * n, hipMemcpyHostToDevice, c->stream));
@@ -1422,6 +1450,7 @@
 int dvp_upload_state(dvp_ctx* c, const float* planes, const uint32_t* views, const uint8_t* weak,
                      const uint8_t* edge, const int32_t* label, const int32_t* radius) {
 	c->anchor_tab_valid = false;
+	bump_reuse_epoch(c);
 	if (set_device(c)) return 1;
 	const size_t L = c->L;
 	if (planes) HIP_TRY(c, hipMemcpyAsync(c->planes, planes, L * 16, hipMemcpyHostToDevice, c->stream));
@@ -1436,6 +1465,7 @@
 int dvp_upload_state_rescaled(dvp_ctx* c, int src_w, int src_h, const float* depth, const float* normal_xyz, const uint32_t* views,
                               const uint8_t* weak, const int32_t* radius, int radius_fallback, const uint8_t* edge, const int32_t* label) {
 	c->anchor_tab_valid = false;
+	bump_reuse_epoch(c);
 	if (set_device(c)) return 1;
 	if (src_w <= 0 || src_h <= 0 || !depth || !normal_xyz || !views) { c->error = "dvp_upload_state_rescaled: depth, normal and selected_views are required"; return 1; }
 	const size_t L = c->L, n = (size_t)src_w * src_h;
@@ -1470,6 +1500,7 @@
 
 int dvp_reset_state(dvp_ctx* c) {
 	c->anchor_tab_valid = false;
+	bump_reuse_epoch(c);
 	if (set_device(c)) return 1;
 	const size_t L = c->L;
 	HIP_TRY(c, hipMemsetAsync(c->planes, 0, L * 16, c->stream));
@@ -1506,6 +1537,7 @@
 }
 int dvp_restore_state(dvp_ctx* c) {
 	c->anchor_tab_valid = false;
+	bump_reuse_epoch(c);
 	if (set_device(c)) return 1;
 	if (!c->have_saved) { c->error = "dvp_restore_state: no saved state"; return 1; }
 	const size_t L = c->L;
@@ -1523,6 +1555,7 @@
 
 int dvp_set_params(dvp_ctx* c, const DvpParams* p) {
 	c->anchor_tab_valid = false;
+	bump_reuse_epoch(c);
 	if (set_device(c)) return 1;
 	if (p->num_images != c->NI) { c->error = "dvp_set_params: params.num_images != context num_images"; return 1; }
 	if (p->use_edge == 0) { c->error = "dvp_set_params: use_edge=false is rejected: the reference's legacy ACMH branch (APD.cu:2142-2460) adopts planes through positions[], which only the use_edge branch assigns (APD.cu:2036, 2084, 2133 vs 2559-2563) - it has no defined result to reproduce"; return 1; }
@@ -1542,7 +1575,7 @@
 	return 0;
 }
 int dvp_set_seed(dvp_ctx* c, uint64_t seed) { c->d.seed = seed; return 0; }
-int dvp_set_sampler(dvp_ctx* c, int s) { c->d.sampler = s ? 1 : 0; return 0; }
+int dvp_set_sampler(dvp_ctx* c, int s) { c->d.sampler = s ? 1 : 0; bump_reuse_epoch(c); return 0; }
 int dvp_set_profiling(dvp_ctx* c, int on) { c->profiling = on != 0; sync_dev_struct(c); return 0; }
 
 static int grow_anchor_table(dvp_ctx* c, size_t wc) {
@@ -1620,8 +1653,13 @@
 	return 0;
 }
 
+static void ensure_strong_reuse_buffers(dvp_ctx* c);
 static void ensure_strong_split_buffers(dvp_ctx* c) {
 	if (c->slot_costs || !c->strong_split || c->NI - 1 > 16) return;
+	if (!getenv("DVP_TEST_SPLIT_ALLOC_FAIL")) {
+		ensure_strong_reuse_buffers(c);
+		if (c->reuse_costs) return;
+	}
 	const size_t Lh = (size_t)((c->W + 1) / 2) * c->H;
 	void *sc = nullptr, *sr = nullptr;
 	if (getenv("DVP_TEST_SPLIT_ALLOC_FAIL")  || hipMalloc(&sc, (size_t)kSlotCount * (c->NI - 1) * Lh * sizeof(*c->slot_costs) + 64 ) != hipSuccess || hipMalloc(&sr, (size_t)SR_FIELDS * Lh * sizeof(*c->strong_rec)) != hipSuccess) {
@@ -1632,6 +1670,26 @@
 	} else {
 		c->allocs.push_back(sc); c->allocs.push_back(sr);
 		c->slot_costs = (decltype(c->slot_costs))sc; c->strong_rec = (decltype(c->strong_rec))sr;
+		sync_dev_struct(c);
+	}
+}
+static void ensure_strong_reuse_buffers(dvp_ctx* c) {
+	if (c->reuse_costs || !c->strong_reuse || !c->strong_split || c->NI - 1 > 16) return;
+	const size_t L = c->L, vec = (size_t)kSlotCount * (c->NI - 1) * L * sizeof(float) + 64 ;
+	void *rc = nullptr, *rk = nullptr, *rh = nullptr, *sr = nullptr;
+	const size_t Lh = (size_t)((c->W + 1) / 2) * c->H;
+	const bool need_rec = !c->strong_rec;
+	if (getenv("DVP_TEST_REUSE_ALLOC_FAIL")  || hipMalloc(&rc, vec) != hipSuccess || hipMalloc(&rk, L * kSlotCount * sizeof(PlaneKey)) != hipSuccess ||
+	    hipMalloc(&rh, L * sizeof(ReuseHdr)) != hipSuccess || (need_rec && hipMalloc(&sr, (size_t)SR_FIELDS * Lh * sizeof(*c->strong_rec)) != hipSuccess) ||
+	    hipMemsetAsync(rh, 0, L * sizeof(ReuseHdr), c->stream) != hipSuccess) {
+		(void)hipGetLastError();
+		for (void* q : { rc, rk, rh, sr }) if (q) (void)hipFree(q);
+		c->strong_reuse = false;
+		fprintf(stderr, "dvp: no room for the strong update's plane cache (%.1f GB); every visit evaluates all its planes\n", (double)(vec + L * (kSlotCount * sizeof(PlaneKey) + sizeof(ReuseHdr))) / 1e9);
+	} else {
+		for (void* q : { rc, rk, rh }) c->allocs.push_back(q);
+		c->reuse_costs = (float*)rc; c->reuse_keys = (PlaneKey*)rk; c->reuse_hdr = (ReuseHdr*)rh;
+		if (need_rec) { c->allocs.push_back(sr); c->strong_rec = (decltype(c->strong_rec))sr; }
 		sync_dev_struct(c);
 	}
 }
@@ -1682,7 +1740,9 @@
 		HIP_TRY(c, hipEventRecord(prep.a, c->stream));
 		HIP_TRY(c, hipMemcpyAsync(c->planes_snap, c->planes, c->L * 16, hipMemcpyDeviceToDevice, c->stream));
 		HIP_TRY(c, hipMemcpyAsync(c->costs_snap, c->costs, c->L * 4, hipMemcpyDeviceToDevice, c->stream));
+		if (c->strong_split && c->NI - 1 <= 16) ensure_strong_split_buffers(c);
 		hipLaunchKernelGGL(dvp_strong_search, dim3(g.grid()), dim3(256), 0, c->stream, c->d, a);
+		if (c->strong_split && c->NI - 1 <= 16 && c->d.reuse_hdr) hipLaunchKernelGGL(dvp_strong_plan, dim3(g.grid()), dim3(256), 0, c->stream, c->d, a);
 		HIP_TRY(c, hipGetLastError());
 		HIP_TRY(c, hipEventRecord(prep.b, c->stream));
 		c->events.push_back(prep);
@@ -1913,6 +1973,7 @@
 
 int dvp_run_patchmatch(dvp_ctx* c) {
 	c->anchor_tab_valid = false;
+	bump_reuse_epoch(c);
 	if (set_device(c)) return 1;
 	EventPair tot, itl;
 	tot.stage = EV_TOTAL; itl.stage = EV_ITER_LOOP;
@@ -2267,6 +2328,7 @@
 }
 int dvp_upload_buffer(dvp_ctx* c, int id, const void* src) {
 	c->anchor_tab_valid = false;
+	bump_reuse_epoch(c);
 	if (set_device(c)) return 1;
 	size_t b; void* p = buffer_ptr(c, id, &b);
 	if (!p) { c->error = "bad or unallocated buffer id"; return 1; }
diff --git a/dvp-mvs_amd/csrc/dvp_strong.hpp b/dvp-mvs_amd/csrc/dvp_strong.hpp
--- a/dvp-mvs_amd/csrc/dvp_strong.hpp
+++ b/dvp-mvs_amd/csrc/dvp_strong.hpp
@@ -546,16 +546,19 @@
 DVP_HD bool same_plane_bits(const f4 a, const f4 b) {
 	return f32_bits(a.x) == f32_bits(b.x) && f32_bits(a.y) == f32_bits(b.y) && f32_bits(a.z) == f32_bits(b.z) && f32_bits(a.w) == f32_bits(b.w);
 }
-DVP_HD uint32_t strong_slot_sources(const Dev& d, int center, uint32_t w[3]) {
+DVP_HD uint32_t strong_slot_planes(const Dev& d, int center, f4 pl[kSlotCount]) {
 	const size_t L = (size_t)d.width * d.height;
-	f4 pl[kSlotCount];
-	uint32_t have = 0, uniq = 0;
+	uint32_t have = 0;
 #pragma unroll
 	for (int slot = 0; slot < kSlotCount; ++slot) {
 		const int pos = slot < 16 ? d.search_pos[(size_t)slot * L + center] : center;
 		pl[slot] = mk4(0.0f, 0.0f, 0.0f, 0.0f);
 		if (pos >= 0) { pl[slot] = d.planes_snap[pos]; have |= 1u << slot; }
 	}
+	return have;
+}
+DVP_HD uint32_t strong_slot_sources_of(const f4 pl[kSlotCount], uint32_t have, uint32_t w[3]) {
+	uint32_t uniq = 0;
 	w[0] = w[1] = w[2] = 0;
 #pragma unroll
 	for (int slot = 0; slot < kSlotCount; ++slot) {
@@ -571,8 +574,84 @@
 	}
 	return uniq;
 }
+DVP_HD uint32_t strong_slot_sources(const Dev& d, int center, uint32_t w[3]) {
+	f4 pl[kSlotCount];
+	const uint32_t have = strong_slot_planes(d, center, pl);
+	return strong_slot_sources_of(pl, have, w);
+}
 DVP_HD int strong_slot_source(uint32_t w0, uint32_t w1, uint32_t w2, int slot) {
 	return slot < 8 ? (int)((w0 >> (4 * slot)) & 15u) : slot < 16 ? (int)((w1 >> (4 * (slot - 8))) & 15u) : (int)w2;
+}
+constexpr uint32_t kPlaceMask = (1u << kSlotCount) - 1u;
+DVP_HD int strong_slot_place_of(uint32_t w0, uint32_t w1, uint32_t w2, int slot) {
+	return slot < 6 ? (int)((w0 >> (5 * slot)) & 31u) : slot < 12 ? (int)((w1 >> (5 * (slot - 6))) & 31u) : (int)((w2 >> (5 * (slot - 12))) & 31u);
+}
+DVP_HD void strong_source_places(const uint32_t src[3], uint32_t place_w[3]) {
+	place_w[0] = place_w[1] = place_w[2] = 0;
+#pragma unroll
+	for (int s = 0; s < kSlotCount; ++s)
+		place_w[s / 6] |= (uint32_t)slot_place(strong_slot_source(src[0], src[1], src[2], s)) << (5 * (s % 6));
+}
+DVP_HD PlaneKey plane_key(const f4 p) {
+	PlaneKey k;
+	k.w[0] = f32_bits(p.x); k.w[1] = f32_bits(p.y); k.w[2] = f32_bits(p.z); k.w[3] = f32_bits(p.w);
+	return k;
+}
+DVP_HD uint32_t strong_reuse_plan(const f4 pl[kSlotCount], uint32_t uniq, const uint32_t src[3], PlaneKey* keys, ReuseHdr* hdr,
+                                  uint32_t epoch, int radius, uint32_t place_w[3]) {
+	const ReuseHdr h = *hdr;
+	const uint32_t valid = (h.epoch == epoch && h.radius == (uint32_t)radius) ? (h.valid & kPlaceMask) : 0u;
+	int place[kSlotCount];
+#pragma unroll
+	for (int s = 0; s < kSlotCount; ++s) place[s] = -1;
+	uint32_t held = 0;
+	if (valid) {
+#pragma unroll
+		for (int p = 0; p < kSlotCount; ++p) {
+			if (!((valid >> p) & 1u)) continue;
+			const PlaneKey k = keys[p];
+#pragma unroll
+			for (int s = 0; s < kSlotCount; ++s) {
+				if (!((uniq >> s) & 1u) || place[s] >= 0) continue;
+				if (k.w[0] == f32_bits(pl[s].x) && k.w[1] == f32_bits(pl[s].y) && k.w[2] == f32_bits(pl[s].z) && k.w[3] == f32_bits(pl[s].w)) { place[s] = p; held |= 1u << p; }
+			}
+		}
+	}
+	uint32_t free_places = kPlaceMask & ~held, eval = 0;
+#pragma unroll
+	for (int s = 0; s < kSlotCount; ++s) {
+		if (!((uniq >> s) & 1u) || place[s] >= 0) continue;
+		const int p = dvp_ctz(free_places);
+		free_places &= free_places - 1;
+		place[s] = p;
+		eval |= 1u << s;
+		keys[p] = plane_key(pl[s]);
+	}
+	place_w[0] = place_w[1] = place_w[2] = 0;
+#pragma unroll
+	for (int s = 0; s < kSlotCount; ++s) {
+		const int from = strong_slot_source(src[0], src[1], src[2], s);
+		int p = 0;
+#pragma unroll
+		for (int u = 0; u <= s; ++u)
+			if (u == from && place[u] >= 0) p = place[u];
+		place_w[s / 6] |= (uint32_t)p << (5 * (s % 6));
+	}
+	ReuseHdr o;
+	o.valid = kPlaceMask & ~free_places; o.radius = (uint32_t)radius; o.epoch = epoch; o.eval = eval;
+	*hdr = o;
+	return eval;
+}
+DVP_HD void strong_plan_px(const Dev& d, int px, int py) {
+	const int center = py * d.width + px;
+	f4 pl[kSlotCount];
+	const uint32_t have = strong_slot_planes(d, center, pl);
+	uint32_t src[3], pw[3];
+	const uint32_t uniq = strong_slot_sources_of(pl, have, src);
+	strong_reuse_plan(pl, uniq, src, d.reuse_keys + (size_t)center * kSlotCount, d.reuse_hdr + center, d.reuse_epoch, d.radius[center], pw);
+	const size_t Lh = (size_t)d.half_w * (size_t)d.height;
+	uint32_t* dup = reinterpret_cast<uint32_t*>(d.strong_rec) + half_index(d, px, py);
+	dup[SR_DUP * Lh] = pw[0]; dup[(SR_DUP + 1) * Lh] = pw[1]; dup[(SR_DUP + 2) * Lh] = pw[2];
 }
 template <int SMP>
 DVP_HD void strong_eval_item(const Dev& d, const PatchCtx& c, int px, int py, int slot, bool store, unsigned long long* nevals) {
@@ -582,9 +661,23 @@
 	const size_t L = (size_t)W * d.height;
 	const int pos = slot < 16 ? d.search_pos[(size_t)slot * L + center] : center;
 	const f4 plane = d.planes_snap[pos];
+	const bool reuse = d.reuse_costs != nullptr;
+	float* const buf = reuse ? d.reuse_costs : d.slot_costs;
+	int at = slot_place(slot);
+	if (reuse) {
+		const size_t Lh = (size_t)d.half_w * (size_t)d.height;
+		const int word = (slot >= 6) + (slot >= 12);
+		const uint32_t pw = reinterpret_cast<const uint32_t*>(d.strong_rec)[(size_t)(SR_DUP + word) * Lh + half_index(d, px, py)];
+		at = (int)((pw >> (5 * (slot - 6 * word))) & 31u);
+	}
 	for (int v = 0; v < S; ++v) {
 		const float cost = ncc_old<SMP>(d, c, px, py, v + 1, plane);
-		if (store) DVP_NT_STORE(4, &d.slot_costs[slot_cost_index(d, slot, v, px, py)], cost);
+#if DVP_SLOT_LAYOUT
+		const size_t rec = reuse ? (size_t)center : half_index(d, px, py);
+		if (store) DVP_NT_STORE(4, &buf[(rec * kSlotCount + (size_t)at) * (size_t)S + (size_t)v], cost);
+#else
+		if (store) DVP_NT_STORE(4, &buf[reuse ? ((size_t)center * kSlotCount + (size_t)at) * (size_t)S + (size_t)v : slot_cost_index(d, slot, v, px, py)], cost);
+#endif
 	}
 	if (nevals && store) *nevals += (unsigned long long)S;
 }
@@ -598,11 +691,16 @@
 		patch_geometry(d, center, &radius, &inc);
 		build_patch_ctx(d, px, py, radius, inc, 0, tab, &c);
 	}
-	uint32_t w[3];
-	const uint32_t uniq = strong_slot_sources(d, center, w);
-	const size_t Lh = (size_t)d.half_w * (size_t)d.height, hi = half_index(d, px, py);
-	uint32_t* dup = reinterpret_cast<uint32_t*>(d.strong_rec) + hi;
-	dup[SR_DUP * Lh] = w[0]; dup[(SR_DUP + 1) * Lh] = w[1]; dup[(SR_DUP + 2) * Lh] = w[2];
+	uint32_t uniq;
+	if (d.reuse_hdr) uniq = d.reuse_hdr[center].eval;
+	else {
+		uint32_t src[3], w[3];
+		uniq = strong_slot_sources(d, center, src);
+		strong_source_places(src, w);
+		const size_t Lh = (size_t)d.half_w * (size_t)d.height, hi = half_index(d, px, py);
+		uint32_t* dup = reinterpret_cast<uint32_t*>(d.strong_rec) + hi;
+		dup[SR_DUP * Lh] = w[0]; dup[(SR_DUP + 1) * Lh] = w[1]; dup[(SR_DUP + 2) * Lh] = w[2];
+	}
 	for (uint32_t m = uniq; m; m &= m - 1) strong_eval_item<SMP>(d, c, px, py, dvp_ctz(m), true, nevals);
 }
 
@@ -624,12 +722,15 @@
 
 template <int MV>
 DVP_HD void strong_decide_px(const Dev& d, int px, int py, int iter) {
-	const SlotCostView cv = slot_cost_view(d, px, py);
 	const int W = d.width;
 	const int center = py * W + px;
 	const DvpParams& P = d.params;
 	const DvpCamera rc = load_camera(d, 0);
 	const int S = P.num_images - 1;
+	const bool reuse = d.reuse_costs != nullptr;
+	SlotCostView cv;
+	if (reuse) { cv.base = d.reuse_costs + (size_t)center * kSlotCount * (size_t)S; cv.slot_stride = (size_t)S; cv.view_stride = 1; }
+	else cv = slot_cost_view(d, px, py);
 	const size_t L = (size_t)W * d.height;
 	const size_t Lh = (size_t)d.half_w * (size_t)d.height, hi = half_index(d, px, py);
 	const float good_thr = 0.8f * dvp_expf((iter) * (iter) / (-90.0f));
@@ -653,7 +754,7 @@
 			if (pos >= 0) {
 				flag |= 1u << k;
 				positions[k] = pos;
-				load_slot_costs<MV>(cv.base + (size_t)slot_place(strong_slot_source(dw0, dw1, dw2, k)) * cv.slot_stride, cv.view_stride, S, ca[k]);
+				load_slot_costs<MV>(cv.base + (size_t)strong_slot_place_of(dw0, dw1, dw2, k) * cv.slot_stride, cv.view_stride, S, ca[k]);
 			}
 		}
 		const int pos = d.search_pos[(size_t)(8 + k) * L + center];
@@ -662,7 +763,7 @@
 			flag |= 1u << k;
 			float cb[MV];
 			int good0 = 0, good1 = 0, bad0 = 0, bad1 = 0;
-			load_slot_costs<MV>(cv.base + (size_t)slot_place(strong_slot_source(dw0, dw1, dw2, 8 + k)) * cv.slot_stride, cv.view_stride, S, cb);
+			load_slot_costs<MV>(cv.base + (size_t)strong_slot_place_of(dw0, dw1, dw2, 8 + k) * cv.slot_stride, cv.view_stride, S, cb);
 #pragma unroll
 			for (int j = 0; j < MV; ++j) {
 				if (j < S) {
@@ -776,7 +877,7 @@
 	float cn = 0.0f;
 #pragma unroll
 	for (int v = 0; v < MV; ++v)
-		if (v < S && vw[v] > 0) cn += vw[v] * cv.base[(size_t)slot_place((int)dw2) * cv.slot_stride + (size_t)v * cv.view_stride];
+		if (v < S && vw[v] > 0) cn += vw[v] * cv.base[(size_t)strong_slot_place_of(dw0, dw1, dw2, kSlotCur) * cv.slot_stride + (size_t)v * cv.view_stride];
 	float cost_now = cn / weight_norm;
 	const float costs_center = cost_now;
 	f4 plane_now = d.planes_snap[center];
diff --git a/dvp-mvs_amd/host/main.cpp b/dvp-mvs_amd/host/main.cpp
--- a/dvp-mvs_amd/host/main.cpp
+++ b/dvp-mvs_amd/host/main.cpp
@@ -479,6 +479,7 @@
 	};
 	std::filesystem::create_directories(opt.dense_folder / "APD");
 	setenv("DVP_SWEEP_BAND_GB", "24", 0);
+	setenv("DVP_STRONG_REUSE", "0", 0);
 	SetHostThreadShare(opt.world);
 	if (opt.world > 1) std::cout << "rank " << opt.rank << " of " << opt.world << ": " << HostThreads() << " host threads (of " << std::thread::hardware_concurrency() << " cores)" << std::endl;
 	APD::SetDevice(opt.gpu);
```
